# terran-project/terran

Measured on AMD Instinct MI355X. Metric: frames/sec 1080p detect+embed+pose, higher is better.
Workload: dtype f16x3: operands x = hi + lo (two IEEE halfs, 22 bits), 3 f16 MFMAs per product, f32 accumulate; float32-grade results; 1 GPU; BASELINE configs[4]: 1080p detect+embed+pose; Detection(short_side=416) + Recognition(top-2) + Estimation(short_side=184); 32 frames per GPU per step resident in HBM; random-init weights; precision=f16x3, frames_per_gpu_step=32, faces_per_frame=2, resident_batch_reused=True, batches_in_flight_per_gpu=2

## Files before the change

include/terran_amd.h:

```cpp
#ifndef TERRAN_AMD_H
#define TERRAN_AMD_H

#include <stddef.h>
#include <stdint.h>

#ifdef __cplusplus
extern "C" {
#endif

#define TA_OK 0
#define TA_E_INVALID (-1)
#define TA_E_DEVICE (-2)
#define TA_E_CAPACITY (-3)
#define TA_E_OVERFLOW (-4)
#define TA_E_RANGE (-5)

#define TA_MODEL_RETINAFACE 1
#define TA_MODEL_ARCFACE 2
#define TA_MODEL_OPENPOSE 3

typedef struct ta_ctx ta_ctx;
typedef struct ta_model ta_model;
typedef struct ta_frames ta_frames;

const char* ta_version(void);
int ta_device_count(void);
int ta_device_pci_bus_id(int device_id, char* out, int capacity);
int ta_ctx_create(int device_id, ta_ctx** out);
void ta_ctx_destroy(ta_ctx* ctx);
const char* ta_last_error(const ta_ctx* ctx);
int ta_ctx_sync(ta_ctx* ctx);
int ta_profile_enable(ta_ctx* ctx, int on);
int ta_profile_reset(ta_ctx* ctx);
int ta_profile_read(ta_ctx* ctx, int klass, double* ms, int64_t* launches, double* work);
int ta_timer_start(ta_ctx* ctx);
int ta_timer_stop(ta_ctx* ctx, double* ms);

int ta_host_alloc(ta_ctx* ctx, size_t bytes, void** out);
void ta_host_free(ta_ctx* ctx, void* ptr);

int ta_frames_upload(ta_ctx* ctx, const uint8_t* nhwc_rgb, int n, int h, int w, ta_frames** out);
int ta_frames_alloc(ta_ctx* ctx, int n, int h, int w, ta_frames** out);
int ta_frames_shape(const ta_frames* f, int* n, int* h, int* w);
int ta_frames_download(const ta_frames* f, uint8_t* nhwc_rgb);
void ta_frames_free(ta_frames* f);
int ta_frames_resize(ta_ctx* ctx, const ta_frames* src, int dst_h, int dst_w, ta_frames** out);
int ta_frames_resize_bicubic(ta_ctx* ctx, const ta_frames* src, int dst_h, int dst_w, ta_frames** out);
int ta_frames_paste(ta_ctx* ctx, const ta_frames* src, int src_index, ta_frames* dst, int dst_index,
                    int top, int left);

#define TA_DRAW_BAR 0
#define TA_DRAW_LINE 1
#define TA_DRAW_DISC 2
typedef struct ta_draw_prim {
  int32_t frame;
  int32_t kind;
  int32_t x0, y0, x1, y1;
  int32_t width;
  uint8_t rgba[4];
} ta_draw_prim;
int ta_frames_draw(ta_ctx* ctx, ta_frames* frames, const ta_draw_prim* prims, int n);

#define TA_JPEG_DEVICE 0
#define TA_JPEG_FALLBACK_PROCESS 1
#define TA_JPEG_FALLBACK_ARITHMETIC 2
#define TA_JPEG_FALLBACK_PRECISION 3
#define TA_JPEG_FALLBACK_COMPONENTS 4
#define TA_JPEG_FALLBACK_COLOR 5
#define TA_JPEG_FALLBACK_SCANS 6
#define TA_JPEG_FALLBACK_SAMPLING 7
#define TA_JPEG_INVALID (-1)
typedef struct ta_jpeg_header {
  int32_t width, height, components;
  int32_t path;
  int32_t h_samp[3], v_samp[3];
  int32_t quant_index[3];
  int32_t blocks_w[3], blocks_h[3];
  int32_t restart_interval;
  int32_t reserved[2];
  int64_t block_offset[3];
  int64_t blocks_total;
  uint16_t quant[4][64];
} ta_jpeg_header;
int ta_jpeg_coefficients(const uint8_t* data, size_t size, ta_jpeg_header* header, int16_t* coefs, int64_t capacity_blocks,
                         char* err, int err_capacity);
int ta_jpeg_decode(ta_ctx* ctx, const uint8_t* const* data, const size_t* sizes, int n, int threads, int capacity,
                   ta_frames** out, int32_t* paths, int32_t* required);
int ta_jpeg_last_stats(const ta_ctx* ctx, double* ms, int64_t* counts);

int ta_jpeg_encode_header(int h, int w, int quality, int subsampling, uint8_t* out, size_t capacity, size_t* size);
int ta_jpeg_encode(ta_ctx* ctx, const ta_frames* frames, int quality, int subsampling, const uint8_t** out,
                   size_t* sizes);
int ta_jpeg_encode_last_stats(const ta_ctx* ctx, double* ms, int64_t* counts);

int ta_model_load(ta_ctx* ctx, int kind, const void* blob, size_t bytes, ta_model** out);
void ta_model_free(ta_model* m);
int ta_model_kind(const ta_model* m);

int ta_model_forward_frames(ta_model* m, const ta_frames* frames);
int ta_model_forward_crops(ta_model* m, const uint8_t* crops_nchw_bgr, int n);
int ta_model_tensor_shape(ta_model* m, int tensor, int* n, int* c, int* h, int* w);
int ta_model_read_tensor(ta_model* m, int tensor, int ch_off, int ch, float* dst_nchw);

int ta_model_tensor_unscale(const ta_model* m, int tensor, float* out, int capacity);
int ta_model_debug_amax(ta_model* m, int enable, float* out, int capacity);
int ta_model_graph_probe(ta_model* m, int reps, double* out_ms);

int ta_retinaface_run(ta_model* m, const ta_frames* frames, float score_thr, float nms_thr,
                      int capacity, int32_t* counts, float* boxes, float* landmarks, float* scores,
                      int32_t* required);
int ta_retinaface_postprocess(ta_ctx* ctx, const float* const heads[9], int n, int h, int w,
                              float score_thr, float nms_thr, int capacity, int32_t* counts,
                              float* boxes, float* landmarks, float* scores, int32_t* required);

int ta_arcface_embed_crops(ta_model* m, const uint8_t* crops_nchw_bgr, int n, int normalize, float* out);
int ta_arcface_embed_faces(ta_model* m, const ta_frames* frames, const int32_t* frame_index,
                           const double* inv_affine, int n, int normalize, float* out,
                           uint8_t* crops_out);
int ta_arcface_embed_faces_multi(ta_model* m, const ta_frames* const* frames, int n_sources, const int32_t* source_index,
                                 const int32_t* frame_index, const double* inv_affine, int n, int normalize,
                                 float* out, uint8_t* crops_out);
int ta_cosine_distance(ta_ctx* ctx, const float* a, int na, const float* b, int nb, int dim, float* out);

int ta_openpose_run(ta_model* m, const ta_frames* frames, double scale, int capacity,
                    int32_t* counts, int32_t* keypoints, double* scores, int32_t* required);
int ta_openpose_group(ta_ctx* ctx, const float* pafs, const float* heatmaps, int n, int h, int w,
                      double scale, int capacity, int32_t* counts, int32_t* keypoints,
                      double* scores, int32_t* required);
int ta_openpose_last_stats(const ta_ctx* ctx, int64_t* peaks, int64_t* connections);

int ta_openpose_debug_read(ta_ctx* ctx, int n, int cap_peaks, int32_t* peak_counts, int32_t* peaks_yx,
                           float* peak_scores, int cap_conn, int32_t* conn_counts, int32_t* conn_ij,
                           float* conn_scores);

int ta_bicubic_x8(ta_ctx* ctx, const float* maps, int n, int c, int h, int w, float* out);

#define TA_CONV_AUTO 0
#define TA_CONV_GENERIC 1
#define TA_CONV_PIPE64 2
#define TA_CONV_PIPE128 3
#define TA_CONV_SPLIT_2x2 4
#define TA_CONV_SPLIT_2x2_P8 5
#define TA_CONV_SPLIT_2x4 6
#define TA_CONV_SPLIT_1x4 7
#define TA_CONV_WIN_2x2 8
#define TA_CONV_WIN_2x4 9
#define TA_CONV_WIN_1x4 10
#define TA_CONV_SPLIT_1x4_W2 11
#define TA_CONV_SPLIT_2x2_W2 12
int ta_debug_conv_variant(ta_ctx* ctx, int variant);
int ta_debug_range_check(ta_ctx* ctx);
int ta_debug_conv_counts(ta_ctx* ctx, int64_t* counts16, int reset);
int ta_debug_kernel_work(ta_ctx* ctx, char* csv, size_t capacity, int reset);

#ifdef __cplusplus
}
#endif
#endif
```

terran_amd/csrc/conv_split.hip:

```cpp
#include "conv_split_kernels.h"

TA_TRACE_READER(ta_debug_trace_read_split)

__global__ __launch_bounds__(256) void splitk_reduce_kernel(const ta_conv_launch p) {
  const int c4 = p.cout >> 2;
  const int total = p.M * c4;
  const int HoWo = p.Ho * p.Wo;
  for (int i = blockIdx.x * blockDim.x + threadIdx.x; i < total; i += gridDim.x * blockDim.x) {
    const int pix = i / c4, co = (i - pix * c4) * 4;
    const int img = pix / HoWo;
    const int rem = pix - img * HoWo;
    const int y = rem / p.Wo, x = rem - y * p.Wo;
    f32x4 v = *(const f32x4*)(p.bias + co);
    const f32x4 us = *(const f32x4*)((p.bias + p.coutp) + co);
    if (p.bias9) {
      const int cls = ta_border_class(y, x, p.Ho, p.Wo);
      if (cls != TA_INTERIOR) v = *(const f32x4*)(p.bias9 + (size_t)cls * p.coutp + co);
    }
    for (int k = 0; k < p.k_split; ++k) {
      const f32x4 t = *(const f32x4*)(p.partial + ((size_t)k * p.M + pix) * p.coutp + co);
#pragma unroll
      for (int e = 0; e < 4; ++e) v[e] = __builtin_fmaf(t[e], us[e], v[e]);
    }
    if (p.act == TA_ACT_RELU) {
#pragma unroll
      for (int e = 0; e < 4; ++e) v[e] = ta_relu(v[e]);
    } else if (p.act == TA_ACT_PRELU) {
      const f32x4 sl = *(const f32x4*)(p.prelu + co);
#pragma unroll
      for (int e = 0; e < 4; ++e) v[e] = v[e] > 0.f ? v[e] : v[e] * sl[e];
    }
    if (p.res) {
      const int ry = p.res_up2 ? (y >> 1) : y, rx = p.res_up2 ? (x >> 1) : x;
      const f32x4 r = ta_ld4(p.res + (size_t)img * p.res_img + (size_t)ry * p.res_row + (size_t)rx * p.res_pix + p.res_off0, p.res_ch + co, p.res_fmt);
#pragma unroll
      for (int e = 0; e < 4; ++e) v[e] += r[e];
    }
    ta_st4(p.out + (size_t)img * p.out_img + (size_t)y * p.out_row + (size_t)x * p.out_pix + p.out_off0, p.out_ch + co,
           p.out_fmt, v);
    unsigned amax = ta_amax4(0u, v);
    if (p.out2) {
      const f32x4 sc = *(const f32x4*)(p.scale2 + co), sh = *(const f32x4*)(p.shift2 + co);
      f32x4 z;
#pragma unroll
      for (int e = 0; e < 4; ++e) z[e] = v[e] * sc[e] + sh[e];
      ta_st4(p.out2 + (size_t)img * p.o2_img + (size_t)y * p.o2_row + (size_t)x * p.o2_pix + p.o2_off0, p.o2_ch + co, p.o2_fmt, z);
      amax = ta_amax4(amax, z);
    }
    if (p.range_check) ta_range_report(p, amax);
  }
}


int ta_win_patch_rows(const ta_conv_launch& p, int BM) {
  if (p.Wo <= 0 || p.Ho <= 0 || p.win_wp <= 0) return 1 << 30;
  const long long n = BM - 1, hp = p.win_img / p.win_wp;
  const long long rows = n + ((n + p.Wo - 1) / p.Wo) * (p.win_wp - p.Wo) + ((n + (long long)p.Ho * p.Wo - 1) / ((long long)p.Ho * p.Wo)) * (hp - p.Ho) * p.win_wp +
                         (long long)(p.k_h - 1) * p.win_wp + p.k_w;
  return rows > (1 << 30) ? (1 << 30) : (int)rows;
}


int ta_launch_conv_split(ta_ctx* ctx, int v, const ta_conv_launch& p) {
  int rc;
  switch (p.prec) {
    case PREC_F16X3: rc = launch_split_variant<PREC_F16X3>(ctx, v, p); break;
    case PREC_F16X2: rc = launch_split_variant<PREC_F16X2>(ctx, v, p); break;
    default: rc = ta_launch_conv_split_modes(ctx, v, p); break;
  }
  if (rc != TA_OK || p.k_split <= 1) return rc;
  const int total = p.M * (p.cout >> 2);
  hipLaunchKernelGGL(splitk_reduce_kernel, dim3((total + 255) / 256), dim3(256), 0, ctx->stream, p);
  TA_HIP(ctx, hipGetLastError());
  return TA_OK;
}
```

terran_amd/csrc/conv_split_kernels.h:

```cpp
#pragma once
#include "conv_common.h"

__device__ __forceinline__ void split_acc_clear(f32x16 (&acc)[2][2]) {
#pragma unroll
  for (int a = 0; a < 2; ++a)
#pragma unroll
    for (int b = 0; b < 2; ++b)
#pragma unroll
      for (int r = 0; r < 16; ++r) acc[a][b][r] = 0.f;
}

template <int PREC>
__device__ __forceinline__ void split_mma16(f32x16 (&acc)[2][2], const bf16x8 (&ah)[2], const bf16x8 (&al)[2], const bf16x8 (&bh)[2],
                                            const bf16x8 (&bl)[2]) {
  if constexpr (prec_x3(PREC) || prec_x2(PREC)) {
#pragma unroll
    for (int a = 0; a < 2; ++a)
#pragma unroll
      for (int b = 0; b < 2; ++b) acc[a][b] = ta_mfma16<PREC>(al[a], bh[b], acc[a][b]);
  }
  if constexpr (prec_x3(PREC)) {
#pragma unroll
    for (int a = 0; a < 2; ++a)
#pragma unroll
      for (int b = 0; b < 2; ++b) acc[a][b] = ta_mfma16<PREC>(ah[a], bl[b], acc[a][b]);
  }
  if constexpr (PREC == PREC_F16) {
#pragma unroll
    for (int a = 0; a < 2; ++a)
#pragma unroll
      for (int b = 0; b < 2; ++b) acc[a][b] = ta_mfma16<PREC>(al[a], bl[b], acc[a][b]);
  }
#pragma unroll
  for (int a = 0; a < 2; ++a)
#pragma unroll
    for (int b = 0; b < 2; ++b) acc[a][b] = ta_mfma16<PREC>(ah[a], bh[b], acc[a][b]);
}

template <int NREAD, int NMMA>
__device__ __forceinline__ void split_pin() {
#pragma unroll
  for (int i = 0; i < NREAD; ++i) {
    __builtin_amdgcn_sched_group_barrier(0x100, 1, 0);
    __builtin_amdgcn_sched_group_barrier(0x008, 1, 0);
  }
  __builtin_amdgcn_sched_group_barrier(0x008, NMMA - NREAD, 0);
}


template <int CM, int CN, int NP, int PREC, int STAGES>
__global__ __launch_bounds__(64 * (CM * CN + NP), STAGES == 2 ? 4 : (CM * CN + NP) / 4) void conv_igemm_split(const ta_conv_launch p) {
  static_assert(NP == 4 || NP == 8, "4 or 8 producer waves");
  static_assert(STAGES == 3 || (STAGES == 2 && CM * CN == 4 && NP == 4), "3-stage ring, or the 2-stage two-workgroups-per-CU variant of the 8-wave tiles");
  static_assert(CM * CN == 4 || CM * CN == 8, "consumer grid: 1x4 (64 cout x 256 px), 2x2 (128 x 128) or 2x4 (128 x 256)");
  constexpr int NC = CM * CN;
  constexpr int BN = CM * 64, BM = CN * 64;
  constexpr int NI = (BN + BM) / 8 / NP;
  constexpr int QA = BN / 8 / NP;
  constexpr int STAGE = (BN + BM) * 32;
  extern __shared__ __attribute__((aligned(16))) float lds[];

  const int tid = threadIdx.x;
  const int lane = tid & 63;
  const int wave = __builtin_amdgcn_readfirstlane(tid >> 6);
  if (wave == 0) TA_STAMP(0);
  if (wave == NC) TA_STAMP(8);

  const int n_ct = p.coutp / BN;
  const int n_pt = (p.M + BM - 1) / BM;
  const int tile_blocks = (((n_pt + 7) >> 3) * n_ct) << 3;
  const int ks = p.k_split > 1 ? ta_div_r(blockIdx.x, tile_blocks, p.r_tile_blocks, p.fast_div) : 0;
  const int bid = blockIdx.x - ks * tile_blocks;
  const int grp = bid >> 3, xcd = bid & 7;
  const int gq = ta_div_r(grp, n_ct, p.r_nct, p.fast_div);
  const int pt = ta_xcd_tile(n_pt, xcd, gq);
  if (pt < 0) return;
  const int ct0 = (grp - gq * n_ct) * BN;
  const int pt0 = pt * BM;
  const int HoWo = p.Ho * p.Wo;
  int s_begin = 0, S = p.n_slabs;
  if (p.k_split > 1) {
    s_begin = (int)(((long long)ks * p.n_slabs) / p.k_split);
    S = (int)(((long long)(ks + 1) * p.n_slabs) / p.k_split) - s_begin;
  }

  if (wave >= NC) {
    const int pw = wave - NC;
    const int pchunk = lane & 7;
    const int lchunk = pchunk ^ ((4 * (pw & 1) + (lane >> 4)) & 7);
    const char* a_base = (const char*)p.w;
    const size_t a_slab_bytes = (size_t)p.coutp * 128;
    unsigned a_off[QA];
    unsigned b_off[NI - QA];
#pragma unroll
    for (int q = 0; q < QA; ++q) a_off[q] = (unsigned)(((ct0 + (q * NP + pw) * 8 + (lane >> 3)) * 32 + lchunk * 4) * 4);
    ta_k_walk wa(p, s_begin);
    auto issue_a = [&](int, int stage) {
#pragma unroll
      for (int q = 0; q < QA; ++q) ta_dma16(a_base + (size_t)wa.a_slab * a_slab_bytes, a_off[q], lds + stage * STAGE + (q * NP + pw) * 256);
      wa.advance();
    };
    issue_a(0, 0);
    if (S > 1) issue_a(1, 1);
    const int pl = p.pool;
    const ta_pixel_walk walk(p, pl ? pt0 >> 2 : pt0, HoWo);
    const int in_ch = p.in_ch_off + (p.group_cout ? (ct0 / p.group_cout) * p.group_cin : 0);
    const size_t off0 = (size_t)walk.img0 * p.in_img + (size_t)((walk.y0 << pl) * p.stride) * p.in_row +
                        (size_t)((walk.x0 << pl) * p.stride) * p.in_pix + p.in_off0 + in_ch;
    const char* b_base = (const char*)(p.in + off0);
    ta_k_walk wb(p, s_begin);
#pragma unroll
    for (int q = QA; q < NI; ++q) {
      const int d = (q * NP + pw) * 8 + (lane >> 3) - BN;
      int img, y, x;
      const int dd = pt0 + d < p.M ? d : 0;
      walk.at(pl ? dd >> 2 : dd, img, y, x);
      if (pl) {
        y = 2 * y + ((dd >> 1) & 1);
        x = 2 * x + (dd & 1);
      }
      const size_t off = (size_t)img * p.in_img + (size_t)(y * p.stride) * p.in_row + (size_t)(x * p.stride) * p.in_pix +
                         p.in_off0 + in_ch;
      b_off[q - QA] = (unsigned)((off - off0) * 4 + lchunk * 16);
      ta_dma16(b_base + wb.b_off, b_off[q - QA], lds + (q * NP + pw) * 256);
    }
    wb.advance();
    auto issue_b = [&](int stage) {
#pragma unroll
      for (int q = QA; q < NI; ++q) ta_dma16(b_base + wb.b_off, b_off[q - QA], lds + stage * STAGE + (q * NP + pw) * 256);
      wb.advance();
    };
    if (wave == NC) TA_STAMP(9);
    if (S > 1) issue_b(1);
    if (wave == NC) TA_STAMP(10);
    int stage = STAGES == 2 ? 0 : 2;
    if constexpr (STAGES == 2) {
      for (int s = 0; s < S; ++s) {
        if (s == 0 && S > 1) asm volatile("s_waitcnt vmcnt(%0)" ::"n"(NI - QA) : "memory");
        else asm volatile("s_waitcnt vmcnt(0)" ::: "memory");
        __builtin_amdgcn_s_barrier();
        asm volatile("" ::: "memory");
        if (s >= 1 && s + 1 < S) {
          issue_a(s + 1, stage);
          issue_b(stage);
          stage ^= 1;
        }
      }
    } else
    for (int s = 0; s < S; ++s) {
      if (s == 0 && S > 1) asm volatile("s_waitcnt vmcnt(%0)" ::"n"(NI - QA) : "memory");
      else if (s + 1 < S) asm volatile("s_waitcnt vmcnt(%0)" ::"n"(NI) : "memory");
      else asm volatile("s_waitcnt vmcnt(0)" ::: "memory");
      __builtin_amdgcn_s_barrier();
      asm volatile("" ::: "memory");
      if (s + 2 < S) {
        issue_a(s + 2, stage);
        issue_b(stage);
        stage = stage == 2 ? 0 : stage + 1;
      }
    }
    {
      __builtin_amdgcn_s_barrier();
      __builtin_amdgcn_s_barrier();
      asm volatile("" ::: "memory");
      bool done = false;
      if constexpr (PREC != PREC_F32) done = conv_drain_dispatch<BN, BM, 64 * (NC + NP), (PREC == PREC_F16 ? 2 : (prec_half(PREC) ? 1 : 0))>(p, lds, ct0, pt0, tid, HoWo);
      if (!done) conv_epilogue_drain<BN, BM, 64 * (NC + NP)>(p, lds, ct0, pt0, tid, HoWo, ks);
    }
    return;
  }

  const int cm = wave / CN, cn = wave % CN;
  int stage = 0;
  f32x16 acc[2][2];
  split_acc_clear(acc);
  const int frow = lane & 31;
  const int fsw = (frow >> 1) & 7;
  const int kg = lane >> 5;
  const int a_row0 = cm * 64 + frow;
  const int b_row0 = BN + cn * 64 + frow;
  struct Frag {
    bf16x8 ah[2], al[2], bh[2], bl[2];
    f32x4 a32[2][2], b32[2][2];
  };
  const int fcb = kg * 4;
  auto load = [&](Frag& f, const float* st, int t) {
    if constexpr (PREC == PREC_F32) {
#pragma unroll
      for (int g = 0; g < 2; ++g) {
        const int pc = ((fcb + 2 * t + g) ^ fsw) * 4;
#pragma unroll
        for (int a = 0; a < 2; ++a) f.a32[a][g] = *(const f32x4*)(st + (a_row0 + a * 32) * 32 + pc);
#pragma unroll
        for (int b = 0; b < 2; ++b) f.b32[b][g] = *(const f32x4*)(st + (b_row0 + b * 32) * 32 + pc);
      }
      return;
    }
#pragma unroll
    for (int a = 0; a < 2; ++a) {
      f.ah[a] = *(const bf16x8*)(st + (a_row0 + a * 32) * 32 + ((2 * kg + t) ^ fsw) * 4);
      if constexpr (prec_x3(PREC) || prec_x2(PREC) || PREC == PREC_F16) f.al[a] = *(const bf16x8*)(st + (a_row0 + a * 32) * 32 + ((4 + 2 * kg + t) ^ fsw) * 4);
    }
#pragma unroll
    for (int b = 0; b < 2; ++b) {
      f.bh[b] = *(const bf16x8*)(st + (b_row0 + b * 32) * 32 + ((2 * kg + t) ^ fsw) * 4);
      if constexpr (prec_x3(PREC) || PREC == PREC_F16) f.bl[b] = *(const bf16x8*)(st + (b_row0 + b * 32) * 32 + ((4 + 2 * kg + t) ^ fsw) * 4);
    }
  };
  auto mma = [&](const Frag& f) {
    if constexpr (PREC == PREC_F32) {
#pragma unroll
      for (int g = 0; g < 2; ++g)
#pragma unroll
        for (int e = 0; e < 4; ++e)
#pragma unroll
          for (int a = 0; a < 2; ++a)
#pragma unroll
            for (int b = 0; b < 2; ++b)
              acc[a][b] = __builtin_amdgcn_mfma_f32_32x32x2f32(f.a32[a][g][e], f.b32[b][g][e], acc[a][b], 0, 0, 0);
      return;
    }
    split_mma16<PREC>(acc, f.ah, f.al, f.bh, f.bl);
  };
  constexpr int NREAD = PREC == PREC_BF16 ? 4 : (prec_x2(PREC) ? 6 : 8);
  constexpr int NMMA = PREC == PREC_F32 ? 32 : (prec_x3(PREC) ? 12 : ((PREC == PREC_F16 || prec_x2(PREC)) ? 8 : 4));
  Frag F0, F1;
  if (wave == 0) TA_STAMP(1);
  __builtin_amdgcn_s_barrier();
  asm volatile("" ::: "memory");
  if (wave == 0) TA_STAMP(2);
  if constexpr (STAGES == 2) {
    for (int s = 0; s < S; ++s) {
      const float* st = lds + (s & 1) * STAGE;
      load(F0, st, 0);
      mma(F0);
      load(F0, st, 1);
      mma(F0);
      if (s + 1 < S) {
        asm volatile("s_waitcnt lgkmcnt(0)" ::: "memory");
        __builtin_amdgcn_s_barrier();
        asm volatile("" ::: "memory");
      }
    }
  } else {
  load(F0, lds + stage * STAGE, 0);
  for (int s = 0; s + 1 < S; ++s) {
    const float* st = lds + stage * STAGE;
    stage = stage + 1 == STAGES ? 0 : stage + 1;
    __builtin_amdgcn_sched_barrier(0);
    load(F1, st, 1);
    mma(F0);
    split_pin<NREAD, NMMA>();
    __builtin_amdgcn_sched_barrier(0);
    asm volatile("s_waitcnt lgkmcnt(0)" ::: "memory");
    __builtin_amdgcn_s_barrier();
    asm volatile("" ::: "memory");
    load(F0, lds + stage * STAGE, 0);
    mma(F1);
    split_pin<NREAD, NMMA>();
    __builtin_amdgcn_sched_barrier(0);
  }
  load(F1, lds + stage * STAGE, 1);
  stage = stage + 1 == STAGES ? 0 : stage + 1;
  mma(F0);
  mma(F1);
  }
  if (wave == 0) TA_STAMP(3);
  {
    __builtin_amdgcn_s_barrier();
    asm volatile("" ::: "memory");
    if (wave == 0) TA_STAMP(5);
    conv_epilogue_park<BN>(acc, lds, cm, cn, lane);
    if (wave == 0) TA_STAMP(6);
    asm volatile("s_waitcnt lgkmcnt(0)" ::: "memory");
    __builtin_amdgcn_s_barrier();
    asm volatile("" ::: "memory");
    if (wave == 0) TA_STAMP(7);
    bool done = false;
    if constexpr (PREC != PREC_F32) done = conv_drain_dispatch<BN, BM, 64 * (NC + NP), (PREC == PREC_F16 ? 2 : (prec_half(PREC) ? 1 : 0))>(p, lds, ct0, pt0, tid, HoWo);
    if (!done) conv_epilogue_drain<BN, BM, 64 * (NC + NP)>(p, lds, ct0, pt0, tid, HoWo, ks);
  }
  if (wave == 0) TA_STAMP(4);
}

template <int CM, int CN, int PREC, int PR>
__global__ __launch_bounds__(64 * (CM * CN + 4), (CM * CN + 4) / 4) void conv_igemm_win(const ta_conv_launch p) {
  static_assert(prec_half(PREC) && PREC != PREC_F16, "pre-split half-float tensors (f16x3 / f16x2)");
  static_assert(CM * CN == 4 || CM * CN == 8, "consumer grid: 1x4 (64 cout x 256 px), 2x2 (128 x 128) or 2x4 (128 x 256)");
  static_assert(PR % 32 == 0, "whole DMA instructions per producer wave");
  constexpr int NC = CM * CN, NP = 4;
  constexpr int BN = CM * 64, BM = CN * 64;
  constexpr int QA = BN / 8 / NP;
  constexpr int NPW = PR / 8 / NP;
  constexpr int A_STAGE = BN * 32;
  constexpr int PATCH = PR * 32;
  static_assert(QA + NPW < 64, "s_waitcnt vmcnt is a 6-bit count");
  extern __shared__ __attribute__((aligned(16))) float lds[];
  float* const patch0 = lds + 3 * A_STAGE;

  const int tid = threadIdx.x;
  const int lane = tid & 63;
  const int wave = __builtin_amdgcn_readfirstlane(tid >> 6);
  const int n_ct = p.coutp / BN;
  const int n_pt = (p.M + BM - 1) / BM;
  const int bid = blockIdx.x;
  const int grp = bid >> 3, xcd = bid & 7;
  const int gq = ta_div_r(grp, n_ct, p.r_nct, p.fast_div);
  const int pt = ta_xcd_tile(n_pt, xcd, gq);
  if (pt < 0) return;
  const int ct0 = (grp - gq * n_ct) * BN;
  const int pt0 = pt * BM;
  const int HoWo = p.Ho * p.Wo;
  const int S = p.n_slabs;
  const int T = p.k_w * p.k_h;
  if (wave == 0) TA_STAMP(0);
  if (wave == NC) TA_STAMP(8);
  const ta_pixel_walk walk(p, pt0, HoWo);
  const int wp = p.win_wp, wimg = p.win_img;

  if (wave >= NC) {
    const int pw = wave - NC;
    const int pchunk = lane & 7;
    const int lchunk = pchunk ^ ((4 * (pw & 1) + (lane >> 4)) & 7);
    const char* a_base = (const char*)p.w;
    const size_t a_slab_bytes = (size_t)p.coutp * 128;
    unsigned a_off[QA];
#pragma unroll
    for (int q = 0; q < QA; ++q) a_off[q] = (unsigned)(((ct0 + (q * NP + pw) * 8 + (lane >> 3)) * 32 + lchunk * 4) * 4);
    ta_k_walk wa(p, 0);
    auto issue_a = [&](int stage) {
#pragma unroll
      for (int q = 0; q < QA; ++q) ta_dma16(a_base + (size_t)wa.a_slab * a_slab_bytes, a_off[q], lds + stage * A_STAGE + (q * NP + pw) * 256);
      wa.advance();
    };
    issue_a(0);
    const int last = (p.M - pt0 < BM ? p.M - pt0 : BM) - 1;
    int img1, y1, x1;
    walk.at(last, img1, y1, x1);
    const int n_patch = (img1 - walk.img0) * wimg + (y1 - walk.y0) * wp + (x1 - walk.x0) + (p.k_h - 1) * wp + p.k_w;
    const int in_ch = p.in_ch_off + (p.group_cout ? (ct0 / p.group_cout) * p.group_cin : 0);
    const size_t off0 = (size_t)walk.img0 * p.in_img + (size_t)walk.y0 * p.in_row + (size_t)walk.x0 * p.in_pix + p.in_off0 + in_ch;
    const char* b_base = (const char*)(p.in + off0);
    unsigned p_off[NPW];
#pragma unroll
    for (int i = 0; i < NPW; ++i) {
      const int r = (i * NP + pw) * 8 + (lane >> 3);
      const int rr = r < n_patch ? r : n_patch - 1;
      p_off[i] = (unsigned)rr * (unsigned)(p.in_pix * 4) + (unsigned)(lchunk * 16);
    }
    auto issue_patch = [&](int cb) {
      float* dst = patch0 + (cb & 1) * PATCH;
#pragma unroll
      for (int i = 0; i < NPW; ++i) ta_dma16(b_base + (size_t)cb * 128, p_off[i], dst + (i * NP + pw) * 256);
    };
    if (wave == NC) TA_STAMP(9);
    issue_patch(0);
    if (S > 1) issue_a(1);
    if (wave == NC) TA_STAMP(10);
    int stage = 2, t = 0, cb = 0;
    bool patch_behind = false;
    for (int g = 0; g < S; ++g) {
      const bool more = g + 1 < S;
      if (patch_behind) {
        if (more) asm volatile("s_waitcnt vmcnt(%0)" ::"n"(QA + NPW) : "memory");
        else asm volatile("s_waitcnt vmcnt(%0)" ::"n"(NPW) : "memory");
      } else {
        if (more) asm volatile("s_waitcnt vmcnt(%0)" ::"n"(QA) : "memory");
        else asm volatile("s_waitcnt vmcnt(0)" ::: "memory");
      }
      __builtin_amdgcn_s_barrier();
      asm volatile("" ::: "memory");
      patch_behind = false;
      if (t == 0 && cb + 1 < p.k_cblocks) {
        issue_patch(cb + 1);
        patch_behind = true;
      }
      if (g + 2 < S) {
        issue_a(stage);
        stage = stage == 2 ? 0 : stage + 1;
      }
      if (++t == T) {
        t = 0;
        ++cb;
      }
    }
    {
      __builtin_amdgcn_s_barrier();
      __builtin_amdgcn_s_barrier();
      asm volatile("" ::: "memory");
      if (!conv_drain_dispatch<BN, BM, 64 * (NC + NP), 1>(p, lds, ct0, pt0, tid, HoWo))
        conv_epilogue_drain<BN, BM, 64 * (NC + NP)>(p, lds, ct0, pt0, tid, HoWo, 0);
    }
    return;
  }

  const int cm = wave / CN, cn = wave % CN;
  f32x16 acc[2][2];
  split_acc_clear(acc);
  const int frow = lane & 31;
  const int fsw = (frow >> 1) & 7;
  const int kg = lane >> 5;
  const int a_row0 = cm * 64 + frow;
  int rB[2];
#pragma unroll
  for (int b = 0; b < 2; ++b) {
    const int d = cn * 64 + b * 32 + frow;
    int img, y, x;
    walk.at(pt0 + d < p.M ? d : 0, img, y, x);
    rB[b] = (img - walk.img0) * wimg + (y - walk.y0) * wp + (x - walk.x0);
  }
  struct Frag {
    bf16x8 ah[2], al[2], bh[2], bl[2];
  };
  unsigned pb[2];
  auto baddr = [&](int tap_off, int buf) {
#pragma unroll
    for (int b = 0; b < 2; ++b) {
      const unsigned row = (unsigned)(rB[b] + tap_off);
      pb[b] = (unsigned)buf * (unsigned)(PATCH * 4) + row * 128u + ((((unsigned)(2 * kg)) ^ ((row >> 1) & 7u)) << 4);
    }
  };
  auto load = [&](Frag& f, const float* st, int t) {
#pragma unroll
    for (int a = 0; a < 2; ++a) {
      f.ah[a] = *(const bf16x8*)(st + (a_row0 + a * 32) * 32 + ((2 * kg + t) ^ fsw) * 4);
      f.al[a] = *(const bf16x8*)(st + (a_row0 + a * 32) * 32 + ((4 + 2 * kg + t) ^ fsw) * 4);
    }
#pragma unroll
    for (int b = 0; b < 2; ++b) {
      const char* q = (const char*)patch0 + (pb[b] ^ (unsigned)(t << 4));
      f.bh[b] = *(const bf16x8*)q;
      if constexpr (prec_x3(PREC)) f.bl[b] = *(const bf16x8*)((const char*)patch0 + ((pb[b] ^ (unsigned)(t << 4)) ^ 64u));
    }
  };
  auto mma = [&](const Frag& f) { split_mma16<PREC>(acc, f.ah, f.al, f.bh, f.bl); };
  constexpr int NREAD = prec_x3(PREC) ? 8 : 6;
  constexpr int NMMA = prec_x3(PREC) ? 12 : 8;
  int kx = 0, ky = 0, cb = 0, tap_off = 0, stage = 0;
  Frag F0, F1;
  baddr(0, 0);
  if (wave == 0) TA_STAMP(1);
  __builtin_amdgcn_s_barrier();
  asm volatile("" ::: "memory");
  if (wave == 0) TA_STAMP(2);
  load(F0, lds, 0);
  for (int g = 0; g + 1 < S; ++g) {
    const float* st = lds + stage * A_STAGE;
    stage = stage == 2 ? 0 : stage + 1;
    __builtin_amdgcn_sched_barrier(0);
    load(F1, st, 1);
    mma(F0);
    split_pin<NREAD, NMMA>();
    __builtin_amdgcn_sched_barrier(0);
    if (++kx == p.k_w) {
      kx = 0;
      tap_off += wp - p.k_w;
      if (++ky == p.k_h) {
        ky = 0;
        ++cb;
        tap_off = -1;
      }
    }
    ++tap_off;
    asm volatile("s_waitcnt lgkmcnt(0)" ::: "memory");
    baddr(tap_off, cb & 1);
    __builtin_amdgcn_s_barrier();
    asm volatile("" ::: "memory");
    load(F0, lds + stage * A_STAGE, 0);
    mma(F1);
    split_pin<NREAD, NMMA>();
    __builtin_amdgcn_sched_barrier(0);
  }
  load(F1, lds + stage * A_STAGE, 1);
  mma(F0);
  mma(F1);
  if (wave == 0) TA_STAMP(3);
  {
    __builtin_amdgcn_s_barrier();
    asm volatile("" ::: "memory");
    if (wave == 0) TA_STAMP(5);
    conv_epilogue_park<BN>(acc, lds, cm, cn, lane);
    if (wave == 0) TA_STAMP(6);
    asm volatile("s_waitcnt lgkmcnt(0)" ::: "memory");
    __builtin_amdgcn_s_barrier();
    asm volatile("" ::: "memory");
    if (wave == 0) TA_STAMP(7);
    if (!conv_drain_dispatch<BN, BM, 64 * (NC + NP), 1>(p, lds, ct0, pt0, tid, HoWo))
      conv_epilogue_drain<BN, BM, 64 * (NC + NP)>(p, lds, ct0, pt0, tid, HoWo, 0);
  }
  if (wave == 0) TA_STAMP(4);
}

static void split_launch_facts(ta_ctx* ctx, ta_conv_launch& q, const ta_tile_grid& g, int BM, int split_fmt, bool lean_ok) {
  q.r_nct = 1.0f / (float)g.n_ct;
  q.r_tile_blocks = 1.0f / (float)(g.groups * 8);
  q.r_Wo = 1.0f / (float)q.Wo;
  q.r_Ho = 1.0f / (float)q.Ho;
  q.r_HoWo = 1.0f / (float)(q.Ho * q.Wo);
  const long long grid = (long long)g.groups * 8 * q.k_split;
  q.fast_div = (grid < (1 << 24) && (long long)q.M + BM < (1 << 24)) ? 1 : 0;
  const long long n_img = q.Ho * q.Wo > 0 ? ((long long)q.M + q.Ho * q.Wo - 1) / (q.Ho * q.Wo) : 0;
  auto fits = [&](long long img_stride, int off0) { return ((n_img + 1) * img_stride + off0) * 4 < (1LL << 32); };
  bool ok = lean_ok && q.out_fmt == split_fmt && (q.cout & 7) == 0 && ((q.out_ch | q.res_ch | q.o2_ch) & 7) == 0 && fits(q.out_img, q.out_off0);
  if (q.res) ok = ok && q.res_fmt == split_fmt && fits(q.res_img, q.res_off0);
  if (q.out2) ok = ok && q.o2_fmt == split_fmt && fits(q.o2_img, q.o2_off0);
  q.fast_drain = ok ? 1 : 0;
  if (ok) ctx->conv_counts[TA_CV_COUNT - 1] += 1;
}

template <int CM, int CN, int NP, int PREC, int STAGES>
static int launch_split(ta_ctx* ctx, const ta_conv_launch& p) {
  constexpr int BN = CM * 64, BM = CN * 64;
  const ta_tile_grid g(p, BN, BM);
  const size_t lds_bytes = (size_t)STAGES * (BN + BM) * 32 * sizeof(float);
  auto kern = conv_igemm_split<CM, CN, NP, PREC, STAGES>;
  TA_SET_LDS_ATTR(ctx, kern, lds_bytes);
  ta_conv_launch q = p;
  constexpr int SPLIT_FMT = PREC == PREC_F16 ? TA_FMT_F16 : (prec_half(PREC) ? TA_FMT_SPLIT16 : TA_FMT_SPLIT);
  split_launch_facts(ctx, q, g, BM, SPLIT_FMT, PREC != PREC_F32 && p.k_split == 1);
  TA_NOTE_KERNEL(ctx, "conv_igemm_split<%d,%d,%d,%d,%d>", CM, CN, NP, PREC, STAGES);
  hipLaunchKernelGGL(kern, dim3(g.groups * 8 * p.k_split), dim3(64 * (CM * CN + NP)), lds_bytes, ctx->stream, q);
  TA_HIP(ctx, hipGetLastError());
  return TA_OK;
}

template <int CM, int CN, int PREC, int PR>
static int launch_win(ta_ctx* ctx, const ta_conv_launch& p) {
  constexpr int BN = CM * 64, BM = CN * 64;
  const ta_tile_grid g(p, BN, BM);
  constexpr size_t ring = (size_t)(3 * BN + 2 * PR) * 128, park = (size_t)BM * BN * 4;
  constexpr size_t lds_bytes = ring > park ? ring : park;
  static_assert(lds_bytes <= 160 * 1024, "one workgroup's LDS");
  auto kern = conv_igemm_win<CM, CN, PREC, PR>;
  TA_SET_LDS_ATTR(ctx, kern, lds_bytes);
  ta_conv_launch q = p;
  q.k_split = 1;
  split_launch_facts(ctx, q, g, BM, TA_FMT_SPLIT16, true);
  TA_NOTE_KERNEL(ctx, "conv_igemm_win<%d,%d,%d,%d>", CM, CN, PREC, PR);
  hipLaunchKernelGGL(kern, dim3(g.groups * 8), dim3(64 * (CM * CN + 4)), lds_bytes, ctx->stream, q);
  TA_HIP(ctx, hipGetLastError());
  return TA_OK;
}

template <int PREC>
static int launch_split_variant(ta_ctx* ctx, int v, const ta_conv_launch& p) {
  switch (v) {
    case TA_CV_SPLIT_2x2: return launch_split<2, 2, 4, PREC, 3>(ctx, p);
    case TA_CV_SPLIT_2x2_P8: return launch_split<2, 2, 8, PREC, 3>(ctx, p);
    case TA_CV_SPLIT_2x4: return launch_split<2, 4, 4, PREC, 3>(ctx, p);
    case TA_CV_SPLIT_1x4: return launch_split<1, 4, 4, PREC, 3>(ctx, p);
    case TA_CV_SPLIT_1x4_W2: return launch_split<1, 4, 4, PREC, 2>(ctx, p);
    case TA_CV_SPLIT_2x2_W2: return launch_split<2, 2, 4, PREC, 2>(ctx, p);
    case TA_CV_WIN_2x2:
    case TA_CV_WIN_2x4:
    case TA_CV_WIN_1x4:
      if constexpr (PREC == PREC_F16X3 || PREC == PREC_F16X2) {
        if (v == TA_CV_WIN_2x2) return launch_win<2, 2, PREC, TA_WIN_PR_2x2>(ctx, p);
        if (v == TA_CV_WIN_2x4) return launch_win<2, 4, PREC, TA_WIN_PR_2x4>(ctx, p);
        return launch_win<1, 4, PREC, TA_WIN_PR_1x4>(ctx, p);
      }
      break;
  }
  return ta_fail(ctx, TA_E_INVALID, "conv: unknown kernel variant %d", v);
}
```

terran_amd/csrc/conv_split_modes.hip:

```cpp
#include "conv_split_kernels.h"

TA_TRACE_READER(ta_debug_trace_read_split_modes)

int ta_launch_conv_split_modes(ta_ctx* ctx, int v, const ta_conv_launch& p) {
  switch (p.prec) {
    case PREC_F32: return launch_split_variant<PREC_F32>(ctx, v, p);
    case PREC_BF16X3: return launch_split_variant<PREC_BF16X3>(ctx, v, p);
    case PREC_F16: return launch_split_variant<PREC_F16>(ctx, v, p);
    default: return launch_split_variant<PREC_BF16>(ctx, v, p);
  }
}
```

terran_amd/csrc/net.hip:

```cpp
#include <stdlib.h>
#include <string.h>

#include <algorithm>
#include <chrono>

#include "act_format.h"
#include "ta_internal.h"

static int conv_out(int in, int k, int stride, int pad) { return (in + 2 * pad - k) / stride + 1; }

static bool conv_ksplit_eligible(const ta_op_desc& op, int in_fmt) {
  const int kblk = in_fmt == TA_FMT_F16 ? 64 : 32;
  const bool uniform = (op.cin % kblk == 0) && (op.n_slabs == op.kh * op.kw * (op.cin / kblk));
  const bool kernel_ok = in_fmt == ta_split_fmt_of(op.prec);
  return uniform && kernel_ok && op.groups <= 1 && !op.pool;
}

#define TA_MAX_PLANS 4
#define TA_MAX_PLAN_BYTES ((size_t)96 << 30)

static void destroy_plan(ta_plan* pl) {
  if (!pl) return;
  if (pl->arena) (void)hipFree(pl->arena);
  if (pl->ktab_dev) (void)hipFree(pl->ktab_dev);
  delete pl;
}

static void activate(ta_model* m, ta_plan* pl) {
  m->active = pl;
  pl->last_use = ++m->use_counter;
  m->plan_n = pl->n;
  m->plan_h = pl->h;
  m->plan_w = pl->w;
  m->tensors = pl->tensors;
  m->ktab_dev = pl->ktab_dev;
  m->ktab_off = pl->ktab_off;
  m->splitk_ws = pl->splitk_ws;
}

static void free_plans(ta_model* m) {
  for (ta_plan* pl : m->plans) destroy_plan(pl);
  m->plans.clear();
  m->active = nullptr;
  m->plan_n = m->plan_h = m->plan_w = 0;
  m->tensors.clear();
  m->ktab_dev = nullptr;
}

static int plan_capacity(int kind, int n) {
  if (kind != TA_MODEL_ARCFACE) return n;
  if (n <= 8) return 8;
  if (n <= 32) return 32;
  return (n + 63) / 64 * 64;
}

int ta_model_plan(ta_model* m, int n_run, int h, int w) {
  ta_ctx* ctx = m->ctx;
  if (n_run <= 0 || h <= 0 || w <= 0) return ta_fail(ctx, TA_E_INVALID, "plan: bad input shape %dx%dx%d", n_run, h, w);
  const int n = plan_capacity(m->kind, n_run);
  m->run_n = n_run;
  if (m->active && m->plan_n == n && m->plan_h == h && m->plan_w == w) {
    m->active->last_use = ++m->use_counter;
    return TA_OK;
  }
  for (ta_plan* pl : m->plans)
    if (pl->n == n && pl->h == h && pl->w == w) {
      activate(m, pl);
      return TA_OK;
    }
  TA_HIP(ctx, hipStreamSynchronize(ctx->stream));
  for (;;) {
    size_t bytes = 0;
    for (ta_plan* pl : m->plans) bytes += pl->arena_bytes;
    if (m->plans.size() < TA_MAX_PLANS && bytes <= TA_MAX_PLAN_BYTES) break;
    if (m->plans.empty()) break;
    size_t lru = 0;
    for (size_t i = 1; i < m->plans.size(); ++i)
      if (m->plans[i]->last_use < m->plans[lru]->last_use) lru = i;
    if (m->plans[lru] == m->active) m->active = nullptr;
    destroy_plan(m->plans[lru]);
    m->plans.erase(m->plans.begin() + lru);
  }
  ta_plan* np = new ta_plan();
  np->n = n;
  np->h = h;
  np->w = w;
  struct guard_t {
    ta_plan*& p;
    ~guard_t() { if (p) destroy_plan(p); }
  } guard{np};

  const int T = m->hdr.n_tensors;
  std::vector<ta_tensor> ts(T);
  std::vector<bool> set(T, false);
  for (int i = 0; i < T; ++i) {
    ts[i].c = m->tdesc[i].channels;
    ts[i].halo = m->tdesc[i].halo;
    ts[i].fmt = m->tdesc[i].fmt;
    if (m->tdesc[i].unscale_off >= 0) {
      ts[i].unscale_dev = (const float*)(m->weights_dev + m->tdesc[i].unscale_off);
      ts[i].unscale_host = m->unscale_host[i].data();
    }
    ts[i].n = n;
  }
  const int in_id = m->hdr.input_tensor;
  ts[in_id].h = h;
  ts[in_id].w = w;
  set[in_id] = true;

  auto resolve_alias = [&](int id) -> int {
    const int src = m->tdesc[id].alias_of;
    if (src == -2) ts[id].owns = false;
    if (src < 0 || set[id]) return TA_OK;
    if (!set[src]) return ta_fail(ctx, TA_E_INVALID, "plan: alias tensor %d used before its source %d", id, src);
    if (ts[src].halo != 0 || (size_t)ts[src].h * ts[src].w * ts[src].c != (size_t)ts[id].c)
      return ta_fail(ctx, TA_E_INVALID, "plan: alias tensor %d does not match source %d", id, src);
    ts[id].h = ts[id].w = 1;
    ts[id].owns = false;
    set[id] = true;
    return TA_OK;
  };

  auto set_out = [&](int id, int oh, int ow) -> int {
    if (oh <= 0 || ow <= 0) return ta_fail(ctx, TA_E_INVALID, "plan: input %dx%d too small for the network", h, w);
    if (set[id]) {
      if (ts[id].h != oh || ts[id].w != ow)
        return ta_fail(ctx, TA_E_INVALID, "plan: tensor %d written with %dx%d and %dx%d", id, ts[id].h, ts[id].w, oh, ow);
      return TA_OK;
    }
    ts[id].h = oh;
    ts[id].w = ow;
    set[id] = true;
    return TA_OK;
  };

  for (size_t oi = 0; oi < m->ops.size(); ++oi) {
    const ta_op_desc& op = m->ops[oi];
    TA_TRY(resolve_alias(op.in));
    if (!set[op.in]) return ta_fail(ctx, TA_E_INVALID, "plan: op %zu reads unset tensor %d", oi, op.in);
    const ta_tensor& ti = ts[op.in];
    if (op.type != TA_OP_CONV && (ti.fmt == TA_FMT_F16 || ts[op.out].fmt == TA_FMT_F16))
      return ta_fail(ctx, TA_E_INVALID, "plan: op %zu: only convs read and write half-float tensors", oi);
    switch (op.type) {
      case TA_OP_CONV:
        if (op.groups > 1) {
          const bool ok = op.cin % 32 == 0 && op.n_slabs == op.kh * op.kw * (op.cin / 32) && op.n_slabs >= 2 &&
                          op.cout % op.groups == 0 && (op.cout / op.groups) % 128 == 0 && op.cout == op.coutp &&
                          op.in_ch_off % 32 == 0 && op.in_ch_off + op.groups * op.cin <= ti.c &&
                          ti.fmt == ta_split_fmt_of(op.prec);
          if (!ok) return ta_fail(ctx, TA_E_INVALID, "plan: op %zu: unsupported grouped convolution", oi);
        }
        [[fallthrough]];
      case TA_OP_DWCONV:
        if (ti.halo < op.pad) return ta_fail(ctx, TA_E_INVALID, "plan: op %zu needs halo %d, tensor has %d", oi, op.pad, ti.halo);
        if (op.type == TA_OP_CONV && op.pool) {
          if (op.out2 >= 0 || op.res >= 0 || op.groups > 1 || op.cin % 32 || op.coutp % 64)
            return ta_fail(ctx, TA_E_INVALID, "plan: op %zu: unsupported conv + max-pool fusion", oi);
          TA_TRY(set_out(op.out, conv_out(ti.h, op.kh, op.stride, op.pad) / 2, conv_out(ti.w, op.kw, op.stride, op.pad) / 2));
          break;
        }
        TA_TRY(set_out(op.out, conv_out(ti.h, op.kh, op.stride, op.pad), conv_out(ti.w, op.kw, op.stride, op.pad)));
        if (op.out2 >= 0) TA_TRY(set_out(op.out2, ts[op.out].h, ts[op.out].w));
        break;
      case TA_OP_MAXPOOL:
        TA_TRY(set_out(op.out, ti.h / 2, ti.w / 2));
        break;
      case TA_OP_RFSTEM:
        if (oi != 0 || op.in != in_id || m->tdesc[op.in].alias_of != -2 || op.w_off < 0)
          return ta_fail(ctx, TA_E_INVALID, "plan: the RetinaFace front op must be op 0 on a shape-only input tensor");
        if (op.cout == 32)
          TA_TRY(set_out(op.out, ((ti.h + 1) / 2 + 1) / 2, ((ti.w + 1) / 2 + 1) / 2));
        else
          TA_TRY(set_out(op.out, (ti.h + 1) / 2, (ti.w + 1) / 2));
        break;
      case TA_OP_DWPW:
        if (ti.halo < 1) return ta_fail(ctx, TA_E_INVALID, "plan: op %zu (dw+pw) needs an input halo", oi);
        if (ti.fmt != TA_FMT_F32 || op.in_ch_off || op.scale2_off < 0 || op.shift2_off < 0 || op.cin > ti.c)
          return ta_fail(ctx, TA_E_INVALID, "plan: op %zu: unsupported dw+pw block", oi);
        TA_TRY(set_out(op.out, conv_out(ti.h, 3, op.stride, 1), conv_out(ti.w, 3, op.stride, 1)));
        break;

      case TA_OP_COPYCH:
        TA_TRY(set_out(op.out, ti.h, ti.w));
        break;
      default:
        return ta_fail(ctx, TA_E_INVALID, "plan: unknown op type %d", op.type);
    }
  }
  for (int i = 0; i < T; ++i) TA_TRY(resolve_alias(i));
  for (int i = 0; i < T; ++i)
    if ((ts[i].fmt != TA_FMT_F32 && ts[i].c % 32) || (ts[i].fmt == TA_FMT_F16 && ts[i].c % 64) || ts[i].fmt < 0 || ts[i].fmt > TA_FMT_F16)
      return ta_fail(ctx, TA_E_INVALID, "plan: tensor %d: format %d with %d channels", i, ts[i].fmt, ts[i].c);

  size_t total = 0;
  std::vector<size_t> offs(T, 0);
  for (int i = 0; i < T; ++i) {
    if (!set[i] || !ts[i].owns) continue;
    const size_t bytes = ts[i].elems() * sizeof(float);
    if (bytes >= ((size_t)1 << 32)) return ta_fail(ctx, TA_E_INVALID, "plan: tensor %d exceeds 4 GiB; split the batch", i);
    offs[i] = total;
    total += (bytes + 255) & ~(size_t)255;
  }
  size_t ws_bytes = 0;
  for (size_t oi = 0; oi < m->ops.size(); ++oi) {
    const ta_op_desc& op = m->ops[oi];
    if (op.type != TA_OP_CONV) continue;
    const int M = ts[op.out].n * ts[op.out].h * ts[op.out].w;
    const int ks = ta_conv_ksplit(op.coutp, op.n_slabs, conv_ksplit_eligible(op, ts[op.in].fmt), (op.variant >> 8) & 255);
    if (ks > 1) ws_bytes = std::max(ws_bytes, (size_t)ks * M * op.coutp * sizeof(float));
  }
  const size_t ws_off = total;
  total += (ws_bytes + 255) & ~(size_t)255;
  hipError_t e = hipMalloc((void**)&np->arena, total ? total : 256);
  if (e != hipSuccess) return ta_fail(ctx, TA_E_DEVICE, "plan: hipMalloc(%zu) failed: %s", total, hipGetErrorString(e));
  np->arena_bytes = total;
  TA_HIP(ctx, hipMemsetAsync(np->arena, 0, total ? total : 256, ctx->stream));
  for (int i = 0; i < T; ++i)
    if (set[i] && ts[i].owns) ts[i].dev = (float*)(np->arena + offs[i]);
  for (int i = 0; i < T; ++i)
    if (set[i] && !ts[i].owns) ts[i].dev = m->tdesc[i].alias_of >= 0 ? ts[m->tdesc[i].alias_of].dev : nullptr;
  np->splitk_ws = ws_bytes ? (float*)(np->arena + ws_off) : nullptr;

  std::vector<int32_t> ktab;
  np->ktab_off.assign(m->ops.size(), 0);
  for (size_t oi = 0; oi < m->ops.size(); ++oi) {
    const ta_op_desc& op = m->ops[oi];
    if (op.type != TA_OP_CONV) continue;
    const ta_tensor& ti = ts[op.in];
    np->ktab_off[oi] = ktab.size();
    if (ti.fmt == TA_FMT_F16) continue;
    const int cpt = op.cin / 4;
    const int nq = op.kh * op.kw * cpt;
    if (nq > op.n_slabs * 8) return ta_fail(ctx, TA_E_INVALID, "plan: op %zu has too few K slabs", oi);
    for (int q = 0; q < op.n_slabs * 8; ++q) {
      int32_t off = 0;
      if (q < nq) {
        const int tap = q / cpt, ch = (q % cpt) * 4;
        const int ky = tap / op.kw, kx = tap % op.kw;
        off = (int32_t)((((size_t)ky * ti.wp() + kx) * ti.c + op.in_ch_off + ch) * sizeof(float));
      }
      ktab.push_back(off);
    }
  }
  if (!ktab.empty()) {
    TA_HIP(ctx, hipMalloc((void**)&np->ktab_dev, ktab.size() * sizeof(int32_t)));
    TA_HIP(ctx, hipMemcpy(np->ktab_dev, ktab.data(), ktab.size() * sizeof(int32_t), hipMemcpyHostToDevice));
  }
  TA_HIP(ctx, hipStreamSynchronize(ctx->stream));
  np->tensors.swap(ts);
  ta_plan* done = np;
  np = nullptr;
  m->plans.push_back(done);
  activate(m, done);
  return TA_OK;
}

static const float* wptr(const ta_model* m, int64_t off) { return off < 0 ? nullptr : (const float*)(m->weights_dev + off); }

static void print_op_profile(ta_model* m, std::vector<hipEvent_t>& ev) {
  (void)hipStreamSynchronize(m->ctx->stream);
  double tot_ms = 0, tot_fl = 0;
  for (size_t oi = 0; oi < m->ops.size(); ++oi) {
    const ta_op_desc& op = m->ops[oi];
    const ta_tensor& to = m->tensors[op.out];
    float ms = 0.f;
    (void)hipEventElapsedTime(&ms, ev[2 * oi], ev[2 * oi + 1]);
    const ta_tensor& ti = m->tensors[op.in];
    const double M = op.type == TA_OP_CONV && op.pool
                         ? (double)m->run_n * conv_out(ti.h, op.kh, op.stride, op.pad) * conv_out(ti.w, op.kw, op.stride, op.pad)
                         : (double)m->run_n * to.h * to.w;
    const double fl = (op.type == TA_OP_CONV || op.type == TA_OP_DWPW) ? 2.0 * op.macs_per_pixel * M : 0.0;
    tot_ms += ms;
    tot_fl += fl;
    fprintf(stderr, "op %3zu type %d k%dx%d s%d g%d cin %4d cout %4d  %3dx%-3d M %8.0f slabs %4d  %8.1f us %7.1f TF\n", oi, op.type, op.kh,
            op.kw, op.stride, op.groups, op.cin, op.cout, to.h, to.w, M, op.n_slabs, ms * 1e3, ms > 0 ? fl / (ms * 1e-3) / 1e12 : 0.0);
  }
  fprintf(stderr, "model kind %d n %d: %.3f ms in ops, %.1f GFLOP, %.1f TF\n", m->kind, m->run_n, tot_ms, tot_fl / 1e9, tot_fl / (tot_ms * 1e-3) / 1e12);
  for (auto e : ev) (void)hipEventDestroy(e);
}

int ta_model_run_ops(ta_model* m) {
  ta_ctx* ctx = m->ctx;
  static const bool prof_ops = getenv("TA_PROFILE_OPS") != nullptr;
  std::vector<hipEvent_t> ev;
  if (prof_ops) {
    ev.resize(2 * m->ops.size());
    for (auto& e : ev) (void)hipEventCreate(&e);
  }
  struct fin_t {
    ta_model* m;
    std::vector<hipEvent_t>& ev;
    bool on;
    ~fin_t() { if (on) print_op_profile(m, ev); }
  } fin{m, ev, prof_ops};
  static const bool no_lanes = getenv("TA_NO_LANES") != nullptr;
  const bool lanes_on = !prof_ops && !ctx->profiling && !no_lanes;
  struct lanes_t {
    ta_ctx* ctx;
    hipStream_t main;
    bool started[2] = {false, false};
    ~lanes_t() {
      ctx->stream = main;
      for (int i = 0; i < 2; ++i)
        if (started[i]) {
          (void)hipEventRecord(ctx->side_join[i], ctx->side_stream[i]);
          (void)hipStreamWaitEvent(main, ctx->side_join[i], 0);
        }
    }
  } lanes{ctx, ctx->stream};
  for (size_t oi = 0; oi < m->ops.size(); ++oi) {
    const ta_op_desc& op = m->ops[oi];
    const ta_tensor& ti = m->tensors[op.in];
    const ta_tensor& to = m->tensors[op.out];
    const int lane = lanes_on ? (op.variant >> 17) & 3 : 0;
    ctx->stream = lanes.main;
    if (lane) {
      const int li = lane - 1;
      if (!ctx->side_stream[li]) {
        TA_HIP(ctx, hipStreamCreateWithFlags(&ctx->side_stream[li], hipStreamNonBlocking));
        TA_HIP(ctx, hipEventCreateWithFlags(&ctx->side_fork[li], hipEventDisableTiming));
        TA_HIP(ctx, hipEventCreateWithFlags(&ctx->side_join[li], hipEventDisableTiming));
      }
      if (!lanes.started[li]) {
        TA_HIP(ctx, hipEventRecord(ctx->side_fork[li], lanes.main));
        TA_HIP(ctx, hipStreamWaitEvent(ctx->side_stream[li], ctx->side_fork[li], 0));
        lanes.started[li] = true;
      }
      ctx->stream = ctx->side_stream[li];
    }
    struct evp_t {
      hipEvent_t e;
      hipStream_t s;
      bool on;
      ~evp_t() { if (on) (void)hipEventRecord(e, s); }
    } evp{prof_ops ? ev[2 * oi + 1] : nullptr, ctx->stream, prof_ops};
    if (prof_ops) (void)hipEventRecord(ev[2 * oi], ctx->stream);
    switch (op.type) {
      case TA_OP_CONV: {
        ta_conv_launch p;
        memset(&p, 0, sizeof(p));
        p.in = ti.dev;
        p.w = wptr(m, op.w_off);
        p.ktab = m->ktab_dev + m->ktab_off[oi];
        p.bias = wptr(m, op.bias_off);
        p.prelu = wptr(m, op.prelu_off);
        p.out = to.dev;
        p.M = m->run_n * to.h * to.w;
        p.Ho = to.h;
        p.Wo = to.w;
        p.n_slabs = op.n_slabs;
        p.coutp = op.coutp;
        p.cout = op.cout;
        p.act = op.act;
        p.stride = op.stride;
        p.prec = op.prec;
        const int kblk = ti.fmt == TA_FMT_F16 ? 64 : 32;
        p.uniform_k = (op.cin % kblk == 0) && (op.n_slabs == op.kh * op.kw * (op.cin / kblk));
        p.k_cblocks = op.cin / kblk;
        if (ti.fmt == TA_FMT_F16 && (!p.uniform_k || op.in_ch_off || op.groups > 1 || op.prec != 4))
          return ta_fail(ctx, TA_E_INVALID, "op %zu: a half-float tensor feeds whole-tensor convs of the f16 mode only", oi);
        p.k_w = op.kw;
        p.k_h = op.kh;
        p.in_ch_off = op.in_ch_off;
        p.in_img = (int)((size_t)ti.hp() * ti.wp() * ti.cf());
        p.in_row = ti.wp() * ti.cf();
        p.in_pix = ti.cf();
        p.win_wp = ti.wp();
        p.win_img = ti.hp() * ti.wp();
        p.in_off0 = (int)(((size_t)(ti.halo - op.pad) * ti.wp() + (ti.halo - op.pad)) * ti.cf());
        p.out_img = (int)((size_t)to.hp() * to.wp() * to.cf());
        p.out_row = to.wp() * to.cf();
        p.out_pix = to.cf();
        p.out_off0 = (int)to.off(0, 0, 0);
        p.out_ch = op.out_ch_off;
        p.out_fmt = to.fmt;
        p.in_fmt = ti.fmt;
        if (op.res >= 0) {
          const ta_tensor& tr = m->tensors[op.res];
          p.res = tr.dev;
          p.res_img = (int)((size_t)tr.hp() * tr.wp() * tr.cf());
          p.res_row = tr.wp() * tr.cf();
          p.res_pix = tr.cf();
          p.res_off0 = (int)tr.off(0, 0, 0);
          p.res_ch = op.res_ch_off;
          p.res_fmt = tr.fmt;
          p.res_up2 = op.res_up2;
        }
        if (op.out2 >= 0) {
          const ta_tensor& t2 = m->tensors[op.out2];
          p.out2 = t2.dev;
          p.scale2 = wptr(m, op.scale2_off);
          p.shift2 = wptr(m, op.shift2_off);
          p.o2_img = (int)((size_t)t2.hp() * t2.wp() * t2.cf());
          p.o2_row = t2.wp() * t2.cf();
          p.o2_pix = t2.cf();
          p.o2_off0 = (int)t2.off(0, 0, 0);
          p.o2_ch = op.out2_ch_off;
          p.o2_fmt = t2.fmt;
        }
        if (op.groups > 1) {
          p.group_cout = op.cout / op.groups;
          p.group_cin = op.cin;
        }
        p.variant = op.variant & 255;
        if ((op.variant >> 16) & 1) p.bias9 = wptr(m, op.scale2_off);
        p.range_check = (m->has_half_ops && (m->tensor_read[op.out] || (op.out2 >= 0 && m->tensor_read[op.out2]))) ? 1 : 0;
        p.amax_index = (m->amax_on && oi < TA_AMAX_OPS) ? (int)oi : -1;
        double flops = 2.0 * op.macs_per_pixel * (double)p.M;
        if (op.pool) {
          p.pool = 1;
          p.M = m->run_n * to.h * to.w * 4;
          flops = 2.0 * op.macs_per_pixel * (double)m->run_n * conv_out(ti.h, op.kh, op.stride, op.pad) *
                  conv_out(ti.w, op.kw, op.stride, op.pad);
        }
        p.k_split = m->splitk_ws ? ta_conv_ksplit(p.coutp, p.n_slabs, conv_ksplit_eligible(op, ti.fmt), (op.variant >> 8) & 255) : 1;
        p.partial = m->splitk_ws;
        if (lane) p.k_split = 1;
        TA_TRY(ta_launch_conv(ctx, p, flops));
        break;
      }
      case TA_OP_RFSTEM:
        TA_TRY(ta_launch_rfstem(ctx, m->input_u8, m->run_n, ti.h, ti.w, (const float*)m->weights_host_small.data(),
                                op.cout == 32 ? wptr(m, op.w_off) + 448 : nullptr, to));
        break;
      case TA_OP_DWPW: {
        ta_conv_launch p;
        memset(&p, 0, sizeof(p));
        p.in = ti.dev;
        p.w = wptr(m, op.w_off);
        p.bias = wptr(m, op.bias_off);
        p.dw_w = wptr(m, op.scale2_off);
        p.dw_bias = wptr(m, op.shift2_off);
        p.dw_c = op.cin;
        p.dw_stride = op.stride;
        p.out = to.dev;
        p.M = m->run_n * to.h * to.w;
        p.Ho = to.h;
        p.Wo = to.w;
        p.n_slabs = op.n_slabs;
        p.coutp = op.coutp;
        p.cout = op.cout;
        p.act = op.act;
        p.stride = 1;
        p.prec = op.prec;
        p.range_check = (m->has_half_ops && m->tensor_read[op.out]) ? 1 : 0;
        p.amax_index = (m->amax_on && oi < TA_AMAX_OPS) ? (int)oi : -1;
        p.in_img = (int)((size_t)ti.hp() * ti.wp() * ti.c);
        p.in_row = ti.wp() * ti.c;
        p.in_pix = ti.c;
        p.in_off0 = (int)(((size_t)(ti.halo - 1) * ti.wp() + (ti.halo - 1)) * ti.c);
        p.in_fmt = ti.fmt;
        p.out_img = (int)((size_t)to.hp() * to.wp() * to.c);
        p.out_row = to.wp() * to.c;
        p.out_pix = to.c;
        p.out_off0 = (int)to.off(0, 0, 0);
        p.out_ch = op.out_ch_off;
        p.out_fmt = to.fmt;
        TA_TRY(ta_launch_dwpw(ctx, p, 2.0 * op.macs_per_pixel * (double)p.M));
        break;
      }
      case TA_OP_DWCONV: {
        ta_dw_launch p;
        memset(&p, 0, sizeof(p));
        p.in = ti.dev;
        p.w = wptr(m, op.w_off);
        p.bias = wptr(m, op.bias_off);
        p.out = to.dev;
        p.N = m->run_n;
        p.Ho = to.h;
        p.Wo = to.w;
        p.C = op.cin;
        p.stride = op.stride;
        p.relu = op.act == TA_ACT_RELU;
        p.in_img = (int)((size_t)ti.hp() * ti.wp() * ti.c);
        p.in_row = ti.wp() * ti.c;
        p.in_pix = ti.c;
        if (op.in_ch_off || op.out_ch_off) return ta_fail(ctx, TA_E_INVALID, "depthwise conv on a channel slice is not supported");
        p.in_off0 = (int)(((size_t)(ti.halo - op.pad) * ti.wp() + (ti.halo - op.pad)) * ti.c);
        p.in_fmt = ti.fmt;
        p.out_img = (int)((size_t)to.hp() * to.wp() * to.c);
        p.out_row = to.wp() * to.c;
        p.out_pix = to.c;
        p.out_off0 = (int)to.off(0, 0, 0);
        p.out_fmt = to.fmt;
        TA_TRY(ta_launch_dwconv(ctx, p));
        break;
      }
      case TA_OP_MAXPOOL:
        TA_TRY(ta_launch_maxpool(ctx, ti, to, m->run_n));
        break;
      case TA_OP_COPYCH:
        TA_TRY(ta_launch_copych(ctx, ti, op.in_ch_off, to, op.out_ch_off, op.cin, m->run_n));
        break;
    }
  }
  return TA_OK;
}

extern "C" {

int ta_model_load(ta_ctx* ctx, int kind, const void* blob, size_t bytes, ta_model** out) {
  ta_enter(ctx);
  if (!ctx || !blob || !out) return TA_E_INVALID;
  *out = nullptr;
  if (bytes < sizeof(ta_blob_header)) return ta_fail(ctx, TA_E_INVALID, "model blob too small");
  ta_blob_header h;
  memcpy(&h, blob, sizeof(h));
  if (h.magic != TA_BLOB_MAGIC || h.version != 9) return ta_fail(ctx, TA_E_INVALID, "model blob: bad magic/version (this library reads version 9)");
  if (h.kind != kind) return ta_fail(ctx, TA_E_INVALID, "model blob is kind %d, expected %d", h.kind, kind);
  if (h.n_tensors <= 0 || h.n_ops <= 0 || h.n_outputs < 0 || h.n_outputs > 16 || h.input_tensor < 0 ||
      h.input_tensor >= h.n_tensors)
    return ta_fail(ctx, TA_E_INVALID, "model blob: bad counts");
  const size_t t_end = (size_t)h.tensors_off + (size_t)h.n_tensors * sizeof(ta_tensor_desc);
  const size_t o_end = (size_t)h.ops_off + (size_t)h.n_ops * sizeof(ta_op_desc);
  const size_t w_end = (size_t)h.weights_off + (size_t)h.weights_bytes;
  if (t_end > bytes || o_end > bytes || w_end > bytes) return ta_fail(ctx, TA_E_INVALID, "model blob: truncated");
  ta_model* m = new ta_model();
  m->ctx = ctx;
  m->kind = kind;
  m->hdr = h;
  m->tdesc.resize(h.n_tensors);
  m->ops.resize(h.n_ops);
  memcpy(m->tdesc.data(), (const char*)blob + h.tensors_off, h.n_tensors * sizeof(ta_tensor_desc));
  memcpy(m->ops.data(), (const char*)blob + h.ops_off, h.n_ops * sizeof(ta_op_desc));
  for (auto& op : m->ops) {
    auto bad_t = [&](int t) { return t < 0 || t >= h.n_tensors; };
    auto bad_w = [&](int64_t off, size_t need) { return off >= 0 && (size_t)off + need > (size_t)h.weights_bytes; };
    bool bad = bad_t(op.in) || bad_t(op.out) || (op.res >= 0 && bad_t(op.res)) || (op.out2 >= 0 && bad_t(op.out2));
    if (op.type == TA_OP_CONV) {
      bad = bad || op.w_off < 0 || op.bias_off < 0 || op.cin % 4 || op.cout % 4 || op.coutp % 32 || op.n_slabs <= 0 ||
            op.stride <= 0 || op.wus_off != op.bias_off + 4 * (int64_t)op.coutp || bad_w(op.wus_off, (size_t)op.coutp * 4) || op.prec < 0 || op.prec > 5 || bad_w(op.w_off, (size_t)op.n_slabs * op.coutp * 128) ||
            bad_w(op.bias_off, (size_t)op.coutp * 4) || bad_w(op.prelu_off, (size_t)op.coutp * 4) ||
            bad_w(op.scale2_off, (size_t)op.coutp * 4) || bad_w(op.shift2_off, (size_t)op.coutp * 4) ||
            (op.act == TA_ACT_PRELU && op.prelu_off < 0) || (op.out2 >= 0 && (op.scale2_off < 0 || op.shift2_off < 0)) ||
            (((op.variant >> 16) & 1) && (op.out2 >= 0 || op.scale2_off < 0 || op.kh != 3 || op.kw != 3 || op.stride != 1 || op.pad != 1 ||
                                          op.pool || bad_w(op.scale2_off, (size_t)16 * op.coutp * 4)));
    } else if (op.type == TA_OP_RFSTEM) {
      bad = bad || op.w_off < 0 || (op.cout != 16 && op.cout != 32) || bad_w(op.w_off, (op.cout == 32 ? 448 + 704 : 448) * 4);
    } else if (op.type == TA_OP_DWPW) {
      bad = bad || op.w_off < 0 || op.bias_off < 0 || op.scale2_off < 0 || op.shift2_off < 0 || op.cin % 4 || op.cout % 4 ||
            (op.prec != 0 && op.prec != 3) || op.wus_off != op.bias_off + 4 * (int64_t)op.coutp || bad_w(op.wus_off, (size_t)op.coutp * 4) ||
            op.coutp % 32 || op.n_slabs <= 0 || op.n_slabs * 32 < op.cin || (op.stride != 1 && op.stride != 2) ||
            bad_w(op.w_off, (size_t)op.n_slabs * op.coutp * 128) || bad_w(op.bias_off, (size_t)op.coutp * 4) ||
            bad_w(op.scale2_off, (size_t)op.cin * 36) || bad_w(op.shift2_off, (size_t)op.cin * 4);
    } else if (op.type == TA_OP_DWCONV) {
      bad = bad || op.w_off < 0 || op.bias_off < 0 || op.cin % 4 || op.kh != 3 || op.kw != 3 ||
            bad_w(op.w_off, (size_t)op.cin * 36) || bad_w(op.bias_off, (size_t)op.cin * 4);
    }
    if (bad) {
      delete m;
      return ta_fail(ctx, TA_E_INVALID, "model blob: malformed op");
    }
  }
  {
    bool bad = m->tdesc[h.input_tensor].unscale_off >= 0;
    m->unscale_host.resize(h.n_tensors);
    for (int t = 0; t < h.n_tensors && !bad; ++t) {
      const int64_t off = m->tdesc[t].unscale_off;
      if (off < 0) continue;
      const size_t need = (size_t)m->tdesc[t].channels * sizeof(float);
      if ((off & 3) || (size_t)off + need > (size_t)h.weights_bytes) {
        bad = true;
        break;
      }
      m->unscale_host[t].resize(m->tdesc[t].channels);
      memcpy(m->unscale_host[t].data(), (const char*)blob + h.weights_off + off, need);
    }
    for (int i = 0; i < h.n_outputs; ++i)
      if (h.outputs[i] < 0 || h.outputs[i] >= h.n_tensors) bad = true;
    m->tensor_read.assign(h.n_tensors, 0);
    for (auto& op : m->ops) {
      m->tensor_read[op.in] = 1;
      if (op.res >= 0) m->tensor_read[op.res] = 1;
    }
    for (int t = 0; t < h.n_tensors; ++t)
      if (m->tdesc[t].alias_of >= 0 && m->tdesc[t].alias_of < h.n_tensors && (m->tensor_read[t] || m->tensor_read[m->tdesc[t].alias_of]))
        m->tensor_read[t] = m->tensor_read[m->tdesc[t].alias_of] = 1;
    for (auto& op : m->ops) {
      if (op.type == TA_OP_DWCONV && (m->tdesc[op.in].unscale_off >= 0 || m->tdesc[op.out].unscale_off >= 0)) bad = true;
      if ((op.type == TA_OP_CONV || op.type == TA_OP_DWPW) && (op.prec == 3 || op.prec == 4 || op.prec == 5)) m->has_half_ops = true;
    }
    if (bad) {
      delete m;
      return ta_fail(ctx, TA_E_INVALID, "model blob: inconsistent activation scales");
    }
  }
  {
    std::vector<int> writer_lane(h.n_tensors, 0), reader_lanes(h.n_tensors, 0);
    bool bad = false;
    for (auto& op : m->ops) {
      const int lane = (op.variant >> 17) & 3;
      if (lane == 3 || (lane && (op.type != TA_OP_CONV || ((op.variant >> 8) & 255) > 1 || op.pool))) bad = true;
      const int reads[3] = {op.in, op.res, -1};
      for (int t : reads) {
        if (t < 0) continue;
        if (writer_lane[t] && writer_lane[t] != lane) bad = true;
        reader_lanes[t] |= 1 << lane;
      }
      const int writes[2] = {op.out, op.out2};
      for (int t : writes) {
        if (t < 0) continue;
        if (reader_lanes[t] & ~(1 << lane)) bad = true;
        if (writer_lane[t] && writer_lane[t] != lane) bad = true;
        if (lane) writer_lane[t] = lane;
        else if (reader_lanes[t] >> 1) bad = true;
      }
    }
    if (bad) {
      delete m;
      return ta_fail(ctx, TA_E_INVALID, "model blob: an op lane (side stream) shares tensors with ops outside it");
    }
  }
  hipError_t e = hipMalloc((void**)&m->weights_dev, h.weights_bytes ? h.weights_bytes : 16);
  if (e != hipSuccess) {
    delete m;
    return ta_fail(ctx, TA_E_DEVICE, "hipMalloc(weights %lld) failed: %s", (long long)h.weights_bytes, hipGetErrorString(e));
  }
  e = hipMemcpy(m->weights_dev, (const char*)blob + h.weights_off, h.weights_bytes, hipMemcpyHostToDevice);
  if (e != hipSuccess) {
    (void)hipFree(m->weights_dev);
    delete m;
    return ta_fail(ctx, TA_E_DEVICE, "weights upload failed: %s", hipGetErrorString(e));
  }
  if (m->ops[0].type == TA_OP_RFSTEM)
    m->weights_host_small.assign((const char*)blob + h.weights_off + m->ops[0].w_off, (const char*)blob + h.weights_off + m->ops[0].w_off + 448 * 4);
  *out = m;
  return TA_OK;
}

int ta_model_graph_probe(ta_model* m, int reps, double* out_ms) {
  ta_enter(m ? m->ctx : nullptr);
  if (!m || !out_ms || reps < 1) return TA_E_INVALID;
  ta_ctx* ctx = m->ctx;
  if (m->run_n <= 0) return ta_fail(ctx, TA_E_INVALID, "graph_probe: run a forward first (it replays that plan)");
  struct res_t {
    hipEvent_t e0 = nullptr, e1 = nullptr;
    hipGraph_t graph = nullptr;
    hipGraphExec_t exec = nullptr;
    ~res_t() {
      if (exec) (void)hipGraphExecDestroy(exec);
      if (graph) (void)hipGraphDestroy(graph);
      if (e0) (void)hipEventDestroy(e0);
      if (e1) (void)hipEventDestroy(e1);
    }
  } r;
  hipEvent_t& e0 = r.e0;
  hipEvent_t& e1 = r.e1;
  hipGraph_t& graph = r.graph;
  hipGraphExec_t& exec = r.exec;
  TA_HIP(ctx, hipEventCreate(&e0));
  TA_HIP(ctx, hipEventCreate(&e1));
  auto now = [] { return std::chrono::duration<double, std::milli>(std::chrono::steady_clock::now().time_since_epoch()).count(); };
  for (int i = 0; i < 2; ++i) TA_TRY(ta_model_run_ops(m));
  TA_HIP(ctx, hipStreamSynchronize(ctx->stream));
  float ms = 0.f;
  double t0 = now();
  TA_HIP(ctx, hipEventRecord(e0, ctx->stream));
  for (int i = 0; i < reps; ++i) TA_TRY(ta_model_run_ops(m));
  TA_HIP(ctx, hipEventRecord(e1, ctx->stream));
  out_ms[2] = (now() - t0) / reps;
  TA_HIP(ctx, hipStreamSynchronize(ctx->stream));
  TA_HIP(ctx, hipEventElapsedTime(&ms, e0, e1));
  out_ms[0] = ms / reps;
  t0 = now();
  TA_HIP(ctx, hipStreamBeginCapture(ctx->stream, hipStreamCaptureModeRelaxed));
  const int rc = ta_model_run_ops(m);
  const hipError_t ce = hipStreamEndCapture(ctx->stream, &graph);
  if (rc != TA_OK) return rc;
  TA_HIP(ctx, ce);
  TA_HIP(ctx, hipGraphInstantiate(&exec, graph, nullptr, nullptr, 0));
  out_ms[4] = now() - t0;
  for (int i = 0; i < 2; ++i) TA_HIP(ctx, hipGraphLaunch(exec, ctx->stream));
  TA_HIP(ctx, hipStreamSynchronize(ctx->stream));
  t0 = now();
  TA_HIP(ctx, hipEventRecord(e0, ctx->stream));
  for (int i = 0; i < reps; ++i) TA_HIP(ctx, hipGraphLaunch(exec, ctx->stream));
  TA_HIP(ctx, hipEventRecord(e1, ctx->stream));
  out_ms[3] = (now() - t0) / reps;
  TA_HIP(ctx, hipStreamSynchronize(ctx->stream));
  TA_HIP(ctx, hipEventElapsedTime(&ms, e0, e1));
  out_ms[1] = ms / reps;
  return TA_OK;
}

int ta_model_debug_amax(ta_model* m, int enable, float* out, int capacity) {
  ta_enter(m ? m->ctx : nullptr);
  if (!m) return TA_E_INVALID;
  ta_ctx* ctx = m->ctx;
  const size_t n = 2 * std::min(m->ops.size(), (size_t)TA_AMAX_OPS);
  unsigned* slots = (unsigned*)ctx->range_flag + TA_AMAX_SLOT0;
  TA_HIP(ctx, hipStreamSynchronize(ctx->stream));
  if (out) {
    if (!m->amax_on) return ta_fail(ctx, TA_E_INVALID, "debug_amax: not enabled");
    if ((size_t)capacity < 2 * m->ops.size()) return ta_fail(ctx, TA_E_CAPACITY, "debug_amax: %zu floats needed", 2 * m->ops.size());
    memset(out, 0, 2 * m->ops.size() * sizeof(float));
    TA_HIP(ctx, hipMemcpy(out, slots, n * sizeof(float), hipMemcpyDeviceToHost));
  }
  if (enable == 2) return TA_OK;
  if (enable) {
    if (ctx->amax_owner && ctx->amax_owner != m)
      return ta_fail(ctx, TA_E_INVALID, "debug_amax: another model of this context is collecting (disable it first)");
    TA_HIP(ctx, hipMemset(slots, 0, 2 * TA_AMAX_OPS * sizeof(unsigned)));
    ctx->amax_owner = m;
  } else if (ctx->amax_owner == m) {
    ctx->amax_owner = nullptr;
  }
  m->amax_on = enable != 0;
  return TA_OK;
}

int ta_model_tensor_unscale(const ta_model* m, int tensor, float* out, int capacity) {
  if (!m || !out || tensor < 0 || tensor >= (int)m->tdesc.size()) return TA_E_INVALID;
  const int c = m->tdesc[tensor].channels;
  if (capacity < c) return TA_E_CAPACITY;
  for (int i = 0; i < c; ++i) out[i] = m->unscale_host[tensor].empty() ? 1.0f : m->unscale_host[tensor][i];
  return TA_OK;
}

void ta_model_free(ta_model* m) {
  ta_enter(m ? m->ctx : nullptr);
  if (!m) return;
  (void)hipStreamSynchronize(m->ctx->stream);
  if (m->ctx->amax_owner == m) m->ctx->amax_owner = nullptr;
  free_plans(m);
  if (m->weights_dev) (void)hipFree(m->weights_dev);
  delete m;
}

int ta_model_kind(const ta_model* m) { return m ? m->kind : TA_E_INVALID; }

int ta_model_forward_frames(ta_model* m, const ta_frames* f) {
  ta_enter(m ? m->ctx : nullptr);
  if (!m || !f) return TA_E_INVALID;
  ta_ctx* ctx = m->ctx;
  if (m->kind != TA_MODEL_RETINAFACE && m->kind != TA_MODEL_OPENPOSE)
    return ta_fail(ctx, TA_E_INVALID, "forward_frames: model kind %d takes crops", m->kind);
  if (f->n == 0) return TA_OK;
  TA_TRY(ta_model_plan(m, f->n, f->h, f->w));
  m->input_u8 = f->dev;
  if (m->ops[0].type != TA_OP_RFSTEM)
    TA_TRY(ta_launch_preprocess(ctx, m->kind == TA_MODEL_RETINAFACE ? TA_PRE_RETINAFACE : TA_PRE_OPENPOSE, f->dev, f->n,
                                f->h, f->w, m->tensors[m->hdr.input_tensor]));
  return ta_model_run_ops(m);
}

int ta_model_forward_crops(ta_model* m, const uint8_t* crops, int n) {
  ta_enter(m ? m->ctx : nullptr);
  if (!m || (!crops && n > 0)) return TA_E_INVALID;
  ta_ctx* ctx = m->ctx;
  if (m->kind != TA_MODEL_ARCFACE) return ta_fail(ctx, TA_E_INVALID, "forward_crops: not an ArcFace model");
  if (n == 0) return TA_OK;
  TA_TRY(ta_model_plan(m, n, 112, 112));
  void* scr = nullptr;
  const size_t bytes = (size_t)n * 3 * 112 * 112;
  TA_TRY(ta_scratch(ctx, bytes, &scr));
  TA_HIP(ctx, hipMemcpyAsync(scr, crops, bytes, hipMemcpyHostToDevice, ctx->stream));
  TA_HIP(ctx, hipStreamSynchronize(ctx->stream));
  TA_TRY(ta_launch_preprocess(ctx, TA_PRE_ARCFACE_CROPS, (const uint8_t*)scr, n, 112, 112,
                              m->tensors[m->hdr.input_tensor]));
  return ta_model_run_ops(m);
}

int ta_model_tensor_shape(ta_model* m, int tensor, int* n, int* c, int* h, int* w) {
  if (!m || tensor < 0 || tensor >= (int)m->tensors.size()) return TA_E_INVALID;
  const ta_tensor& t = m->tensors[tensor];
  if (n) *n = m->run_n;
  if (c) *c = t.c;
  if (h) *h = t.h;
  if (w) *w = t.w;
  return TA_OK;
}

int ta_model_read_tensor(ta_model* m, int tensor, int ch_off, int ch, float* dst) {
  ta_enter(m ? m->ctx : nullptr);
  if (!m || !dst || tensor < 0 || tensor >= (int)m->tensors.size()) return TA_E_INVALID;
  ta_ctx* ctx = m->ctx;
  const ta_tensor& t = m->tensors[tensor];
  if (!t.dev || ch_off < 0 || ch <= 0 || ch_off + ch > t.c) return ta_fail(ctx, TA_E_INVALID, "read_tensor: bad slice");
  std::vector<float> host((size_t)m->run_n * t.hp() * t.wp() * t.c);
  TA_HIP(ctx, hipStreamSynchronize(ctx->stream));
  TA_HIP(ctx, hipMemcpy(host.data(), t.dev, host.size() * sizeof(float), hipMemcpyDeviceToHost));
  for (int i = 0; i < m->run_n; ++i)
    for (int c = 0; c < ch; ++c)
      for (int y = 0; y < t.h; ++y)
        for (int x = 0; x < t.w; ++x)
        {
          const int cc = ch_off + c;
          float v;
          if (t.fmt == TA_FMT_F16) {
            _Float16 hh;
            memcpy(&hh, (const char*)&host[t.off(i, y, x)] + 2 * cc, 2);
            v = (float)hh;
          } else if (t.fmt != TA_FMT_F32) {
            const char* b = (const char*)&host[t.off(i, y, x)] + ((cc >> 5) << 7) + ((cc & 31) << 1);
            uint16_t h16, l16;
            memcpy(&h16, b, 2);
            memcpy(&l16, b + 64, 2);
            if (t.fmt == TA_FMT_SPLIT16) {
              _Float16 hh, ll;
              memcpy(&hh, &h16, 2);
              memcpy(&ll, &l16, 2);
              v = (float)hh + (float)ll;
            } else {
              const uint32_t hb = (uint32_t)h16 << 16, lb = (uint32_t)l16 << 16;
              float hf, lf;
              memcpy(&hf, &hb, 4);
              memcpy(&lf, &lb, 4);
              v = hf + lf;
            }
          } else {
            v = host[t.off(i, y, x) + cc];
          }
          dst[(((size_t)i * ch + c) * t.h + y) * t.w + x] = t.unscale_host ? v * t.unscale_host[cc] : v;
        }
  return TA_OK;
}

}
```

terran_amd/csrc/ta_internal.h:

```cpp
#pragma once
#include <hip/hip_runtime.h>
#include <stdint.h>
#include <stdio.h>
#include <atomic>
#include <map>
#include <mutex>
#include <string>
#include <vector>

#include "../../include/terran_amd.h"

#define TA_BLOB_MAGIC 0x314D4154u

enum {
  TA_OP_CONV = 1,
  TA_OP_DWCONV = 2,
  TA_OP_MAXPOOL = 3,
  TA_OP_COPYCH = 4,
  TA_OP_RFSTEM = 5,
  TA_OP_DWPW = 6
};
enum { TA_ACT_NONE = 0, TA_ACT_RELU = 1, TA_ACT_PRELU = 2 };

struct ta_blob_header {
  uint32_t magic;
  uint32_t version;
  int32_t kind;
  int32_t n_tensors;
  int32_t n_ops;
  int32_t input_tensor;
  int32_t n_outputs;
  int32_t outputs[16];
  int64_t tensors_off, ops_off, weights_off, weights_bytes;
};

struct ta_tensor_desc {
  int32_t channels;
  int32_t halo;
  int32_t alias_of;
  int32_t fmt;
  int32_t unscale_off;
};

struct ta_op_desc {
  int32_t type;
  int32_t in, out;
  int32_t in_ch_off, cin;
  int32_t out_ch_off, cout;
  int32_t coutp;
  int32_t kh, kw, stride, pad;
  int32_t act;
  int32_t res, res_ch_off, res_up2;
  int32_t out2, out2_ch_off;
  int32_t n_slabs;
  int32_t prec;
  int32_t groups;
  int32_t variant;
  int32_t pool;
  int32_t wscale_log2;
  int64_t w_off, bias_off, prelu_off, scale2_off, shift2_off;
  int64_t wus_off;
  double macs_per_pixel;
};

static_assert(sizeof(ta_blob_header) == 128 && sizeof(ta_tensor_desc) == 20 && sizeof(ta_op_desc) == 152,
              "blob layout is shared with terran_amd/pack.py (HEADER_DT / TENSOR_DT / OP_DT)");

struct ta_prof_class {
  double ms = 0;
  int64_t launches = 0;
  double work = 0;
};

struct ta_pending_event {
  hipEvent_t a, b;
  int klass;
  const std::string* kernel;
};

struct ta_ctx {
  int device = -1;
  hipStream_t stream = nullptr;
  std::string err;
  bool profiling = false;
  ta_prof_class prof[4];
  std::vector<ta_pending_event> pending;
  std::vector<hipEvent_t> event_pool;
  hipEvent_t t0 = nullptr, t1 = nullptr;
  void* scratch = nullptr;
  size_t scratch_bytes = 0;
  void* pinned = nullptr;
  size_t pinned_bytes = 0;
  std::mutex frame_cache_mu;
  std::vector<std::pair<size_t, void*>> frame_cache;
  size_t frame_cache_bytes = 0;
  int64_t pose_peaks = 0, pose_connections = 0;
  double jpeg_ms[4] = {0, 0, 0, 0};
  int64_t jpeg_counts[4] = {0, 0, 0, 0};
  double jpeg_enc_ms[8] = {0, 0, 0, 0, 0, 0, 0, 0};
  int64_t jpeg_enc_counts[4] = {0, 0, 0, 0};
  void* jpeg_enc_dev = nullptr;
  size_t jpeg_enc_dev_bytes = 0;
  uint8_t* jpeg_enc_out = nullptr;
  size_t jpeg_enc_out_bytes = 0;
  float* pose_wphase = nullptr;
  struct {
    int n = 0, maxp = 0;
    const int *peak_cnt = nullptr, *peak_yx = nullptr, *conn_cnt = nullptr, *conn_ij = nullptr;
    const float *peak_sc = nullptr, *conn_sc = nullptr;
    struct over_t {
      int img, maxp;
      void* mem;
      const int *peak_cnt, *peak_yx, *conn_cnt, *conn_ij;
      const float *peak_sc, *conn_sc;
    };
    std::vector<over_t> over;
  } pose_dbg;
  hipStream_t side_stream[2] = {nullptr, nullptr};
  hipEvent_t side_fork[2] = {nullptr, nullptr}, side_join[2] = {nullptr, nullptr};
  int conv_force = 0;
#ifdef TA_CONV_TRACE
  int conv_trace_block = 0;
#endif
  int64_t conv_counts[16] = {0};
  int* range_flag = nullptr;
  int* range_flag_host = nullptr;
  const void* amax_owner = nullptr;
  double cur_flops = 0;
  std::map<std::string, std::pair<int64_t, double>> kernel_work;
  std::map<std::string, double> kernel_ms;
  const std::string* cur_kernel = nullptr;
  void note_kernel(const char* name) {
    auto it = kernel_work.try_emplace(name, 0, 0.0).first;
    it->second.first += 1;
    it->second.second += cur_flops;
    cur_kernel = &it->first;
  }
};
void ta_pose_free_big(ta_ctx* ctx);
#define TA_AMAX_SLOT0 16
#define TA_AMAX_OPS 4096
int ta_range_enqueue(ta_ctx* ctx);
int ta_range_check(ta_ctx* ctx);
int ta_range_finish(ta_ctx* ctx, int rc);

enum {
  TA_CV_AUTO = 0,
  TA_CV_GENERIC = 1,
  TA_CV_PIPE64 = 2,
  TA_CV_PIPE128 = 3,
  TA_CV_SPLIT_2x2 = 4,
  TA_CV_SPLIT_2x2_P8 = 5,
  TA_CV_SPLIT_2x4 = 6,
  TA_CV_SPLIT_1x4 = 7,
  TA_CV_WIN_2x2 = 8,
  TA_CV_WIN_2x4 = 9,
  TA_CV_WIN_1x4 = 10,
  TA_CV_SPLIT_1x4_W2 = 11,
  TA_CV_SPLIT_2x2_W2 = 12,
  TA_CV_COUNT = 16
};

#define TA_SET_LDS_ATTR(ctx, kern, bytes)                                                                         \
  do {                                                                                                            \
    static std::atomic<unsigned long long> _done{0};                                                              \
    const unsigned long long _bit = 1ull << ((ctx)->device & 63);                                                 \
    if (!(_done.load(std::memory_order_acquire) & _bit)) {                                                        \
      TA_HIP(ctx, hipFuncSetAttribute((const void*)(kern), hipFuncAttributeMaxDynamicSharedMemorySize, (int)(bytes))); \
      _done.fetch_or(_bit, std::memory_order_release);                                                            \
    }                                                                                                             \
  } while (0)

int ta_fail(ta_ctx* ctx, int code, const char* fmt, ...);
static inline void ta_enter(const ta_ctx* ctx) {
  if (ctx) (void)hipSetDevice(ctx->device);
}
int ta_scratch(ta_ctx* ctx, size_t bytes, void** out);
int ta_pinned(ta_ctx* ctx, size_t bytes, void** out);

#define TA_HIP(ctx, expr)                                                                      \
  do {                                                                                         \
    hipError_t _e = (expr);                                                                    \
    if (_e != hipSuccess)                                                                      \
      return ta_fail((ctx), TA_E_DEVICE, "%s failed: %s (%s:%d)", #expr, hipGetErrorString(_e), \
                     __FILE__, __LINE__);                                                      \
  } while (0)

#define TA_TRY(expr)            \
  do {                          \
    int _r = (expr);            \
    if (_r != TA_OK) return _r; \
  } while (0)

struct ta_prof_scope {
  ta_ctx* ctx;
  int klass;
  double work;
  hipEvent_t a = nullptr, b = nullptr;
  ta_prof_scope(ta_ctx* c, int k, double w);
  ~ta_prof_scope();
};

void ta_drain_profile(ta_ctx* ctx);

struct ta_frames {
  ta_ctx* ctx;
  int n, h, w;
  uint8_t* dev;
  size_t cap = 0;
};
int ta_frames_alloc_uninit(ta_ctx* ctx, int n, int h, int w, ta_frames** out);

struct ta_tensor {
  float* dev = nullptr;
  int n = 0, h = 0, w = 0, c = 0, halo = 0, fmt = 0;
  const float* unscale_dev = nullptr;
  const float* unscale_host = nullptr;
  bool owns = true;
  int hp() const { return h + 2 * halo; }
  int wp() const { return w + 2 * halo; }
  size_t elems() const { return (size_t)n * hp() * wp() * c; }
  int cf() const { return fmt == 3  ? c / 2 : c; }
  size_t off(int img, int y, int x) const { return (((size_t)img * hp() + y + halo) * wp() + x + halo) * cf(); }
};

struct ta_conv_launch {
  const float* in;
  const float* w;
  const int32_t* ktab;
  const float* bias;
  const float* prelu;
  float* out;
  const float* res;
  float* out2;
  const float* scale2;
  const float* shift2;
  int M, Ho, Wo, n_slabs, coutp, cout, act, stride, prec;
  int uniform_k, k_cblocks, k_w, k_h, in_ch_off;
  int in_img, in_row, in_pix, in_off0;
  int out_img, out_row, out_pix, out_off0, out_ch, out_fmt;
  int res_img, res_row, res_pix, res_off0, res_up2, res_ch, res_fmt;
  int o2_img, o2_row, o2_pix, o2_off0, o2_ch, o2_fmt;
  int in_fmt;
  int win_wp, win_img;
  int group_cout, group_cin;
  int k_split;
  float* partial;
  int variant;
  const float* dw_w;
  const float* dw_bias;
  int dw_c, dw_stride;
  int pool;
  float r_nct, r_tile_blocks, r_Wo, r_Ho, r_HoWo;
  int fast_div;
  int fast_drain;
#ifdef TA_CONV_TRACE
  int trace_block;
#endif
  const float* bias9;
  int range_check;
  int amax_index;
  int* range_flag;
};

static inline int ta_split_fmt_of(int prec) { return prec == 0 ? 0  : (prec == 4 ? 3  : ((prec == 3 || prec == 5) ? 2  : 1 )); }

static inline int ta_conv_ksplit(int coutp, int n_slabs, bool eligible, int packed = 0) {
  if (!eligible || coutp % 128) return 1;
  if (packed > 1) return packed <= n_slabs ? packed : 1;
  if (n_slabs < 512) return 1;
  return 32;
}

int ta_launch_conv(ta_ctx* ctx, const ta_conv_launch& p, double flops);
int ta_launch_conv_sym(ta_ctx* ctx, int variant, const ta_conv_launch& p);
int ta_launch_conv_split(ta_ctx* ctx, int variant, const ta_conv_launch& p);
int ta_launch_conv_split_modes(ta_ctx* ctx, int variant, const ta_conv_launch& p);
int ta_launch_dwpw(ta_ctx* ctx, const ta_conv_launch& p, double flops);
int ta_win_patch_rows(const ta_conv_launch& p, int BM);
#define TA_WIN_PR_2x2 384
#define TA_WIN_PR_2x4 448
#define TA_WIN_PR_1x4 512
struct ta_frames;
int ta_launch_rfstem(ta_ctx* ctx, const uint8_t* frames_dev, int n, int h, int w, const float* weights_host, const float* w2_dev, const struct ta_tensor& out);

struct ta_dw_launch {
  const float* in;
  const float* w;
  const float* bias;
  float* out;
  int N, Ho, Wo, C, stride, relu;
  int in_img, in_row, in_pix, in_off0, in_fmt;
  int out_img, out_row, out_pix, out_off0, out_fmt;
};
int ta_launch_dwconv(ta_ctx* ctx, const ta_dw_launch& p);
int ta_launch_maxpool(ta_ctx* ctx, const ta_tensor& in, const ta_tensor& out, int n);
int ta_launch_copych(ta_ctx* ctx, const ta_tensor& in, int in_ch, const ta_tensor& out, int out_ch, int ch, int n);

enum { TA_PRE_RETINAFACE = 1, TA_PRE_OPENPOSE = 2, TA_PRE_ARCFACE_CROPS = 3 };
int ta_launch_preprocess(ta_ctx* ctx, int mode, const uint8_t* src_dev, int n, int h, int w, const ta_tensor& dst);

struct ta_plan {
  int n = 0, h = 0, w = 0;
  std::vector<ta_tensor> tensors;
  char* arena = nullptr;
  size_t arena_bytes = 0;
  int32_t* ktab_dev = nullptr;
  std::vector<size_t> ktab_off;
  float* splitk_ws = nullptr;
  uint64_t last_use = 0;
};

struct ta_model {
  ta_ctx* ctx = nullptr;
  int kind = 0;
  ta_blob_header hdr;
  std::vector<ta_tensor_desc> tdesc;
  std::vector<ta_op_desc> ops;
  char* weights_dev = nullptr;
  bool has_half_ops = false;
  bool amax_on = false;
  std::vector<char> tensor_read;
  std::vector<std::vector<float>> unscale_host;
  std::vector<char> weights_host_small;
  std::vector<ta_plan*> plans;
  ta_plan* active = nullptr;
  uint64_t use_counter = 0;
  int plan_n = 0, plan_h = 0, plan_w = 0;
  int run_n = 0;
  const uint8_t* input_u8 = nullptr;
  std::vector<ta_tensor> tensors;
  int32_t* ktab_dev = nullptr;
  std::vector<size_t> ktab_off;
  float* splitk_ws = nullptr;
};

int ta_model_plan(ta_model* m, int n, int h, int w);
int ta_model_run_ops(ta_model* m);
```

terran_amd/lib.py:

```python
import ctypes as C
import os

import numpy as np

HERE = os.path.dirname(os.path.abspath(__file__))
LIB_PATH = os.path.join(HERE, 'libterran_amd.so')

OK, E_INVALID, E_DEVICE, E_CAPACITY, E_OVERFLOW, E_RANGE = 0, -1, -2, -3, -4, -5
_CODES = {E_INVALID: 'TA_E_INVALID', E_DEVICE: 'TA_E_DEVICE', E_CAPACITY: 'TA_E_CAPACITY', E_OVERFLOW: 'TA_E_OVERFLOW',
          E_RANGE: 'TA_E_RANGE'}


class TerranAmdError(RuntimeError):
    def __init__(self, code, msg):
        super().__init__('%s: %s' % (_CODES.get(code, code), msg))
        self.code = code


c_int, c_float, c_double, c_void_p, c_size_t = C.c_int, C.c_float, C.c_double, C.c_void_p, C.c_size_t
P = C.POINTER
u8p, i32p, f32p, f64p = P(C.c_uint8), P(C.c_int32), P(C.c_float), P(C.c_double)

SIGNATURES = {
    'ta_version': (C.c_char_p, []),
    'ta_device_count': (c_int, []),
    'ta_device_pci_bus_id': (c_int, [c_int, C.c_char_p, c_int]),
    'ta_ctx_create': (c_int, [c_int, P(c_void_p)]),
    'ta_ctx_destroy': (None, [c_void_p]),
    'ta_last_error': (C.c_char_p, [c_void_p]),
    'ta_ctx_sync': (c_int, [c_void_p]),
    'ta_profile_enable': (c_int, [c_void_p, c_int]),
    'ta_profile_reset': (c_int, [c_void_p]),
    'ta_profile_read': (c_int, [c_void_p, c_int, f64p, P(C.c_int64), f64p]),
    'ta_timer_start': (c_int, [c_void_p]),
    'ta_timer_stop': (c_int, [c_void_p, f64p]),
    'ta_host_alloc': (c_int, [c_void_p, c_size_t, P(c_void_p)]),
    'ta_host_free': (None, [c_void_p, c_void_p]),
    'ta_frames_upload': (c_int, [c_void_p, c_void_p, c_int, c_int, c_int, P(c_void_p)]),
    'ta_frames_alloc': (c_int, [c_void_p, c_int, c_int, c_int, P(c_void_p)]),
    'ta_frames_shape': (c_int, [c_void_p, P(c_int), P(c_int), P(c_int)]),
    'ta_frames_download': (c_int, [c_void_p, c_void_p]),
    'ta_frames_free': (None, [c_void_p]),
    'ta_frames_resize': (c_int, [c_void_p, c_void_p, c_int, c_int, P(c_void_p)]),
    'ta_frames_resize_bicubic': (c_int, [c_void_p, c_void_p, c_int, c_int, P(c_void_p)]),
    'ta_frames_paste': (c_int, [c_void_p, c_void_p, c_int, c_void_p, c_int, c_int, c_int]),
    'ta_frames_draw': (c_int, [c_void_p, c_void_p, c_void_p, c_int]),
    'ta_jpeg_coefficients': (c_int, [c_void_p, c_size_t, c_void_p, c_void_p, C.c_int64, C.c_char_p, c_int]),
    'ta_jpeg_decode': (c_int, [c_void_p, P(c_void_p), P(c_size_t), c_int, c_int, c_int, P(c_void_p), P(C.c_int32),
                               P(C.c_int32)]),
    'ta_jpeg_last_stats': (c_int, [c_void_p, c_void_p, c_void_p]),
    'ta_jpeg_encode_header': (c_int, [c_int, c_int, c_int, c_int, c_void_p, c_size_t, P(c_size_t)]),
    'ta_jpeg_encode': (c_int, [c_void_p, c_void_p, c_int, c_int, P(c_void_p), P(c_size_t)]),
    'ta_jpeg_encode_last_stats': (c_int, [c_void_p, c_void_p, c_void_p]),
    'ta_model_load': (c_int, [c_void_p, c_int, c_void_p, c_size_t, P(c_void_p)]),
    'ta_model_free': (None, [c_void_p]),
    'ta_model_kind': (c_int, [c_void_p]),
    'ta_model_forward_frames': (c_int, [c_void_p, c_void_p]),
    'ta_model_forward_crops': (c_int, [c_void_p, c_void_p, c_int]),
    'ta_model_tensor_shape': (c_int, [c_void_p, c_int, P(c_int), P(c_int), P(c_int), P(c_int)]),
    'ta_model_tensor_unscale': (c_int, [c_void_p, c_int, c_void_p, c_int]),
    'ta_model_debug_amax': (c_int, [c_void_p, c_int, c_void_p, c_int]),
    'ta_model_graph_probe': (c_int, [c_void_p, c_int, c_void_p]),
    'ta_model_read_tensor': (c_int, [c_void_p, c_int, c_int, c_int, c_void_p]),
    'ta_retinaface_run': (c_int, [c_void_p, c_void_p, c_float, c_float, c_int, c_void_p, c_void_p, c_void_p,
                                  c_void_p, P(C.c_int32)]),
    'ta_retinaface_postprocess': (c_int, [c_void_p, P(c_void_p), c_int, c_int, c_int, c_float, c_float, c_int,
                                          c_void_p, c_void_p, c_void_p, c_void_p, P(C.c_int32)]),
    'ta_arcface_embed_crops': (c_int, [c_void_p, c_void_p, c_int, c_int, c_void_p]),
    'ta_arcface_embed_faces': (c_int, [c_void_p, c_void_p, c_void_p, c_void_p, c_int, c_int, c_void_p, c_void_p]),
    'ta_arcface_embed_faces_multi': (c_int, [c_void_p, P(c_void_p), c_int, c_void_p, c_void_p, c_void_p, c_int, c_int, c_void_p,
                                             c_void_p]),
    'ta_cosine_distance': (c_int, [c_void_p, c_void_p, c_int, c_void_p, c_int, c_int, c_void_p]),
    'ta_openpose_run': (c_int, [c_void_p, c_void_p, c_double, c_int, c_void_p, c_void_p, c_void_p, P(C.c_int32)]),
    'ta_openpose_group': (c_int, [c_void_p, c_void_p, c_void_p, c_int, c_int, c_int, c_double, c_int, c_void_p,
                                  c_void_p, c_void_p, P(C.c_int32)]),
    'ta_bicubic_x8': (c_int, [c_void_p, c_void_p, c_int, c_int, c_int, c_int, c_void_p]),
    'ta_openpose_last_stats': (c_int, [c_void_p, c_void_p, c_void_p]),
    'ta_openpose_debug_read': (c_int, [c_void_p, c_int, c_int, c_void_p, c_void_p, c_void_p, c_int, c_void_p, c_void_p,
                                       c_void_p]),
    'ta_debug_conv_variant': (c_int, [c_void_p, c_int]),
    'ta_debug_range_check': (c_int, [c_void_p]),
    'ta_debug_conv_counts': (c_int, [c_void_p, c_void_p, c_int]),
    'ta_debug_kernel_work': (c_int, [c_void_p, C.c_char_p, c_size_t, c_int]),
}

DRAW_BAR, DRAW_LINE, DRAW_DISC = 0, 1, 2
PRIM_DT = np.dtype([('frame', '<i4'), ('kind', '<i4'), ('x0', '<i4'), ('y0', '<i4'), ('x1', '<i4'), ('y1', '<i4'),
                    ('width', '<i4'), ('rgba', 'u1', (4,))])
assert PRIM_DT.itemsize == 32

JPEG_DEVICE = 0
JPEG_INVALID = -1
JPEG_PATHS = {-1: 'invalid', 0: 'device', 1: 'progressive/lossless/hierarchical', 2: 'arithmetic', 3: 'precision',
              4: 'components', 5: 'rgb', 6: 'scans', 7: 'sampling'}
JPEG_HEADER_DT = np.dtype([('width', '<i4'), ('height', '<i4'), ('components', '<i4'), ('path', '<i4'),
                           ('h_samp', '<i4', (3,)), ('v_samp', '<i4', (3,)), ('quant_index', '<i4', (3,)),
                           ('blocks_w', '<i4', (3,)), ('blocks_h', '<i4', (3,)), ('restart_interval', '<i4'),
                           ('reserved', '<i4', (2,)), ('block_offset', '<i8', (3,)), ('blocks_total', '<i8'),
                           ('quant', '<u2', (4, 64))])
assert JPEG_HEADER_DT.itemsize == 632


def jpeg_coefficients(data, header_only=False):
    lib = load()
    buf = np.frombuffer(bytes(data), np.uint8)
    hdr = np.zeros(1, JPEG_HEADER_DT)
    err = C.create_string_buffer(256)
    rc = lib.ta_jpeg_coefficients(ptr(buf), buf.size, ptr(hdr), None, 0, err, len(err))
    if rc != OK:
        raise TerranAmdError(rc, err.value.decode(errors='replace'))
    if header_only or hdr['path'][0] != JPEG_DEVICE:
        return hdr[0], None
    coefs = np.empty((int(hdr['blocks_total'][0]), 64), np.int16)
    rc = lib.ta_jpeg_coefficients(ptr(buf), buf.size, ptr(hdr), ptr(coefs), coefs.shape[0], err, len(err))
    if rc != OK:
        raise TerranAmdError(rc, err.value.decode(errors='replace'))
    return hdr[0], coefs


def jpeg_encode_header(h, w, quality=75, subsampling=2):
    lib = load()
    size = c_size_t()
    buf = np.zeros(1024, np.uint8)
    rc = lib.ta_jpeg_encode_header(int(h), int(w), int(quality), int(subsampling), ptr(buf), buf.size, C.byref(size))
    if rc != OK:
        raise TerranAmdError(rc, 'jpeg_encode_header(%r, %r, %r, %r)' % (h, w, quality, subsampling))
    return buf[:size.value].tobytes()


def check_jpeg_options(quality, subsampling):
    if isinstance(quality, bool) or not isinstance(quality, (int, np.integer)) or not 1 <= quality <= 100:
        raise ValueError('JPEG quality must be an int in 1..100, got %r' % (quality,))
    if isinstance(subsampling, bool) or not isinstance(subsampling, (int, np.integer)) or subsampling not in (0, 1, 2):
        raise ValueError('JPEG subsampling must be 0 (4:4:4), 1 (4:2:2) or 2 (4:2:0), got %r' % (subsampling,))
    return int(quality), int(subsampling)


CONV_VARIANTS = {'auto': 0, 'generic': 1, 'pipe64': 2, 'pipe128': 3, 'split_2x2': 4, 'split_2x2_p8': 5, 'split_2x4': 6,
                 'split_1x4': 7, 'win_2x2': 8, 'win_2x4': 9, 'win_1x4': 10, 'split_1x4_w2': 11, 'split_2x2_w2': 12}

_lib = None


def load():
    global _lib
    if _lib is None:
        if not os.path.exists(LIB_PATH):
            raise TerranAmdError(E_DEVICE, 'libterran_amd.so not built (run `python -m terran_amd.build`); '
                                           'there is no CPU fallback')
        from . import build as _build
        try:
            with open(_build.STAMP) as fh:
                stamp = fh.read().strip()
        except OSError:
            stamp = None
        try:
            current = _build.source_hash()
        except OSError:
            current = stamp
        if (stamp is None or stamp != current) and not os.environ.get('TA_ALLOW_STALE_LIB'):
            raise TerranAmdError(E_DEVICE, 'libterran_amd.so was not built from the sources in terran_amd/csrc '
                                           '(run `python -m terran_amd.build`)')
        os.environ.setdefault('GPU_MAX_HW_QUEUES', '12')
        os.environ.setdefault('HIP_FORCE_DEV_KERNARG', '1')
        lib = C.CDLL(LIB_PATH)
        missing = []
        for name, (res, args) in SIGNATURES.items():
            try:
                fn = getattr(lib, name)
            except AttributeError:
                missing.append(name)
                continue
            fn.restype = res
            fn.argtypes = args
        if missing and not os.environ.get('TA_BRINGUP_ALLOW_MISSING'):
            raise TerranAmdError(E_INVALID, 'libterran_amd.so lacks ABI symbols: %s' % ', '.join(missing))
        _lib = lib
    return _lib


def ptr(a):
    return a.ctypes.data_as(c_void_p) if a is not None else None


class Context:

    def __init__(self, device_id=0):
        self.lib = load()
        h = c_void_p()
        rc = self.lib.ta_ctx_create(int(device_id), C.byref(h))
        if rc != OK:
            raise TerranAmdError(rc, 'ta_ctx_create(%d) failed: no usable gfx950 device '
                                     '(ta_device_count=%d)' % (device_id, self.lib.ta_device_count()))
        self.h = h
        self.device_id = device_id

    def check(self, rc):
        if rc != OK:
            raise TerranAmdError(rc, self.lib.ta_last_error(self.h).decode(errors='replace'))

    def last_error(self):
        return self.lib.ta_last_error(self.h).decode(errors='replace')

    def sync(self):
        self.check(self.lib.ta_ctx_sync(self.h))

    def close(self):
        if getattr(self, 'h', None):
            self.lib.ta_ctx_destroy(self.h)
            self.h = None

    def __del__(self):
        try:
            self.close()
        except Exception:
            pass

    def profile(self, on):
        self.check(self.lib.ta_profile_enable(self.h, int(on)))

    def profile_reset(self):
        self.check(self.lib.ta_profile_reset(self.h))

    def profile_read(self, klass):
        ms, n, w = c_double(), C.c_int64(), c_double()
        self.check(self.lib.ta_profile_read(self.h, klass, C.byref(ms), C.byref(n), C.byref(w)))
        return ms.value, n.value, w.value

    def timer_start(self):
        self.check(self.lib.ta_timer_start(self.h))

    def timer_stop(self):
        ms = c_double()
        self.check(self.lib.ta_timer_stop(self.h, C.byref(ms)))
        return ms.value

    def upload(self, images):
        images = np.ascontiguousarray(images, dtype=np.uint8)
        assert images.ndim == 4 and images.shape[3] == 3
        return Frames(self, images)

    def pinned_array(self, shape):
        n = int(np.prod(shape))
        p = c_void_p()
        self.check(self.lib.ta_host_alloc(self.h, n, C.byref(p)))
        arr = np.ctypeslib.as_array((C.c_uint8 * n).from_address(p.value)).reshape(shape)
        arr_ptr = p.value
        return arr, arr_ptr

    def free_pinned(self, ptr):
        if getattr(self, 'h', None):
            self.lib.ta_host_free(self.h, c_void_p(ptr))

    def cosine_distance(self, a, b):
        a = np.ascontiguousarray(a, dtype=np.float32)
        b = np.ascontiguousarray(b, dtype=np.float32)
        out = np.empty((a.shape[0], b.shape[0]), np.float32)
        self.check(self.lib.ta_cosine_distance(self.h, ptr(a), a.shape[0], ptr(b), b.shape[0], a.shape[1], ptr(out)))
        return out

    def jpeg_decode(self, buffers, threads=0):
        bufs = [bytes(b) for b in buffers]
        n = len(bufs)
        arrs = [np.frombuffer(b, np.uint8) for b in bufs]
        data = (c_void_p * n)(*[a.ctypes.data for a in arrs])
        sizes = (c_size_t * n)(*[a.size for a in arrs])
        out = (c_void_p * n)()
        paths = np.zeros(n, np.int32)
        req = C.c_int32()
        rc = self.lib.ta_jpeg_decode(self.h, data, sizes, n, int(threads), n, out, paths.ctypes.data_as(P(C.c_int32)),
                                     C.byref(req))
        if rc != OK:
            e = TerranAmdError(rc, self.last_error())
            e.paths = paths
            raise e
        return [Frames(self, handle=c_void_p(out[k])) for k in range(req.value)], paths

    def jpeg_stats(self):
        ms, cnt = np.zeros(4, np.float64), np.zeros(4, np.int64)
        self.check(self.lib.ta_jpeg_last_stats(self.h, ptr(ms), ptr(cnt)))
        return (dict(zip(('host', 'h2d', 'idct', 'color'), ms.tolist())),
                dict(zip(('images', 'blocks', 'bytes', 'fallbacks'), cnt.tolist())))

    def jpeg_encode(self, frames, quality=75, subsampling=2):
        quality, subsampling = check_jpeg_options(quality, subsampling)
        n = frames.shape[0]
        out = c_void_p()
        sizes = (c_size_t * n)()
        self.check(self.lib.ta_jpeg_encode(self.h, frames.h, quality, subsampling, C.byref(out), sizes))
        files, at = [], out.value
        for k in range(n):
            files.append(C.string_at(at, sizes[k]))
            at += sizes[k]
        return files

    def jpeg_encode_stats(self):
        ms, cnt = np.zeros(8, np.float64), np.zeros(4, np.int64)
        self.check(self.lib.ta_jpeg_encode_last_stats(self.h, ptr(ms), ptr(cnt)))
        return (dict(zip(('h2d', 'coef', 'length', 'emit', 'ffcount', 'pack', 'd2h', 'host'), ms.tolist())),
                dict(zip(('images', 'blocks', 'bytes', 'entropy_bytes'), cnt.tolist())))

    def conv_variant(self, name):
        self.check(self.lib.ta_debug_conv_variant(self.h, CONV_VARIANTS[name]))

    def conv_counts(self, reset=False):
        c = np.zeros(16, np.int64)
        self.check(self.lib.ta_debug_conv_counts(self.h, ptr(c), int(reset)))
        out = {k: int(c[v]) for k, v in CONV_VARIANTS.items() if v and c[v]}
        if c[15]:
            out['lean_epilogue'] = int(c[15])
        return out

    def kernel_work(self, reset=False):
        buf = C.create_string_buffer(1 << 16)
        self.check(self.lib.ta_debug_kernel_work(self.h, buf, len(buf), int(reset)))
        out = {}
        for line in buf.value.decode().splitlines():
            f = line.split(';')
            out[f[0]] = (int(f[1]), float(f[2]), float(f[3]) if len(f) > 3 else 0.0)
        return out

    def pose_debug(self, n, cap_peaks=1024, cap_conn=1024):
        pc = np.zeros((n, 18), np.int32)
        pyx = np.zeros((n, 18, cap_peaks, 2), np.int32)
        psc = np.zeros((n, 18, cap_peaks), np.float32)
        cc = np.zeros((n, 19), np.int32)
        cij = np.zeros((n, 19, cap_conn, 2), np.int32)
        csc = np.zeros((n, 19, cap_conn), np.float32)
        self.check(self.lib.ta_openpose_debug_read(self.h, n, cap_peaks, ptr(pc), ptr(pyx), ptr(psc), cap_conn,
                                                   ptr(cc), ptr(cij), ptr(csc)))
        assert pc.max(initial=0) <= cap_peaks and cc.max(initial=0) <= cap_conn
        peaks = [[(pyx[i, p, :pc[i, p]].copy(), psc[i, p, :pc[i, p]].copy()) for p in range(18)] for i in range(n)]
        conns = [[None if cc[i, l] < 0 else (cij[i, l, :cc[i, l]].copy(), csc[i, l, :cc[i, l]].copy())
                  for l in range(19)] for i in range(n)]
        return peaks, conns

    def pose_stats(self):
        a, b = C.c_int64(), C.c_int64()
        self.check(self.lib.ta_openpose_last_stats(self.h, C.byref(a), C.byref(b)))
        return a.value, b.value

    def bicubic_x8(self, maps):
        maps = np.ascontiguousarray(maps, dtype=np.float32)
        n, c, h, w = maps.shape
        out = np.empty((n, c, 8 * h, 8 * w), np.float32)
        self.check(self.lib.ta_bicubic_x8(self.h, ptr(maps), n, c, h, w, ptr(out)))
        return out


class Frames:

    def __init__(self, ctx, images=None, handle=None):
        self.ctx = ctx
        if handle is not None:
            self.h = handle
        else:
            h = c_void_p()
            n, hh, ww = images.shape[:3]
            ctx.check(ctx.lib.ta_frames_upload(ctx.h, ptr(images), n, hh, ww, C.byref(h)))
            self.h = h
        n, hh, ww = c_int(), c_int(), c_int()
        ctx.lib.ta_frames_shape(self.h, C.byref(n), C.byref(hh), C.byref(ww))
        self.shape = (n.value, hh.value, ww.value, 3)

    def __len__(self):
        return self.shape[0]

    @classmethod
    def zeros(cls, ctx, n, h, w):
        hd = c_void_p()
        ctx.check(ctx.lib.ta_frames_alloc(ctx.h, n, h, w, C.byref(hd)))
        return cls(ctx, handle=hd)

    def resize(self, h, w, ctx=None):
        ctx = ctx or self.ctx
        hd = c_void_p()
        ctx.check(ctx.lib.ta_frames_resize(ctx.h, self.h, int(h), int(w), C.byref(hd)))
        return Frames(ctx, handle=hd)

    def resize_bicubic(self, h, w, ctx=None):
        ctx = ctx or self.ctx
        hd = c_void_p()
        ctx.check(ctx.lib.ta_frames_resize_bicubic(ctx.h, self.h, int(h), int(w), C.byref(hd)))
        return Frames(ctx, handle=hd)

    def paste(self, src, src_index, dst_index, top, left):
        self.ctx.check(self.ctx.lib.ta_frames_paste(self.ctx.h, src.h, src_index, self.h, dst_index, top, left))

    def draw(self, prims, ctx=None):
        ctx = ctx or self.ctx
        prims = np.ascontiguousarray(prims, dtype=PRIM_DT)
        ctx.check(ctx.lib.ta_frames_draw(ctx.h, self.h, ptr(prims) if len(prims) else None, len(prims)))

    def encode_jpeg(self, quality=75, subsampling=2, ctx=None):
        return (ctx or self.ctx).jpeg_encode(self, quality, subsampling)

    def download(self):
        out = np.empty(self.shape, np.uint8)
        self.ctx.check(self.ctx.lib.ta_frames_download(self.h, ptr(out)))
        return out

    def free(self):
        if getattr(self, 'h', None) and getattr(self.ctx, 'h', None):
            self.ctx.lib.ta_frames_free(self.h)
        self.h = None

    def __del__(self):
        try:
            self.free()
        except Exception:
            pass


class Model:

    def __init__(self, ctx, program):
        self.ctx = ctx
        self.kind = program.kind
        self.names = dict(program.names)
        blob = program.blob()
        buf = np.frombuffer(blob, dtype=np.uint8)
        h = c_void_p()
        ctx.check(ctx.lib.ta_model_load(ctx.h, program.kind, ptr(buf), len(blob), C.byref(h)))
        self.h = h

    def forward_frames(self, frames):
        self.ctx.check(self.ctx.lib.ta_model_forward_frames(self.h, frames.h))

    def forward_crops(self, crops):
        crops = np.ascontiguousarray(crops, dtype=np.uint8)
        self.ctx.check(self.ctx.lib.ta_model_forward_crops(self.h, ptr(crops), crops.shape[0]))

    def read(self, name):
        tid, off, ch = self.names[name]
        n, c, h, w = c_int(), c_int(), c_int(), c_int()
        self.ctx.check(self.ctx.lib.ta_model_tensor_shape(self.h, tid, C.byref(n), C.byref(c), C.byref(h), C.byref(w)))
        out = np.empty((n.value, ch, h.value, w.value), np.float32)
        self.ctx.check(self.ctx.lib.ta_model_read_tensor(self.h, tid, off, ch, ptr(out)))
        return out

    def read_tensor(self, tid, ch_off=0, ch=None):
        n, c, h, w = c_int(), c_int(), c_int(), c_int()
        self.ctx.check(self.ctx.lib.ta_model_tensor_shape(self.h, tid, C.byref(n), C.byref(c), C.byref(h), C.byref(w)))
        ch = c.value - ch_off if ch is None else ch
        out = np.empty((n.value, ch, h.value, w.value), np.float32)
        self.ctx.check(self.ctx.lib.ta_model_read_tensor(self.h, tid, ch_off, ch, ptr(out)))
        return out

    def tensor_unscale(self, tid, channels):
        out = np.empty(channels, np.float32)
        self.ctx.check(self.ctx.lib.ta_model_tensor_unscale(self.h, tid, ptr(out), channels))
        return out

    def amax_collect(self, on=True):
        self.ctx.check(self.ctx.lib.ta_model_debug_amax(self.h, int(bool(on)), None, 0))

    def graph_probe(self, reps=20):
        out = np.zeros(5, np.float64)
        self.ctx.check(self.ctx.lib.ta_model_graph_probe(self.h, int(reps), ptr(out)))
        return tuple(float(x) for x in out)

    def amax_read(self, n_ops):
        out = np.zeros(2 * n_ops, np.float32)
        n = c_int()
        self.ctx.check(self.ctx.lib.ta_model_debug_amax(self.h, 2, ptr(out), out.size))
        return out.reshape(n_ops, 2)

    def free(self):
        if getattr(self, 'h', None) and getattr(self.ctx, 'h', None):
            self.ctx.lib.ta_model_free(self.h)
        self.h = None

    def __del__(self):
        try:
            self.free()
        except Exception:
            pass
```

terran_amd/pack.py:

```python
import os

import numpy as np

from . import arch

MODEL_RETINAFACE, MODEL_ARCFACE, MODEL_OPENPOSE = 1, 2, 3
OP_CONV, OP_DWCONV, OP_MAXPOOL, OP_COPYCH, OP_RFSTEM, OP_DWPW = 1, 2, 3, 4, 5, 6
ACT_NONE, ACT_RELU, ACT_PRELU = 0, 1, 2
MAGIC = 0x314D4154

HEADER_DT = np.dtype({
    'names': ['magic', 'version', 'kind', 'n_tensors', 'n_ops', 'input_tensor', 'n_outputs', 'outputs',
              'tensors_off', 'ops_off', 'weights_off', 'weights_bytes'],
    'formats': ['<u4', '<u4', '<i4', '<i4', '<i4', '<i4', '<i4', ('<i4', 16), '<i8', '<i8', '<i8', '<i8'],
    'offsets': [0, 4, 8, 12, 16, 20, 24, 28, 96, 104, 112, 120],
    'itemsize': 128,
})
TENSOR_DT = np.dtype([('channels', '<i4'), ('halo', '<i4'), ('alias_of', '<i4'), ('fmt', '<i4'), ('unscale_off', '<i4')])
FMT_F32, FMT_SPLIT, FMT_SPLIT16, FMT_F16 = 0, 1, 2, 3
_OP_I32 = ['type', 'in', 'out', 'in_ch_off', 'cin', 'out_ch_off', 'cout', 'coutp', 'kh', 'kw', 'stride', 'pad',
           'act', 'res', 'res_ch_off', 'res_up2', 'out2', 'out2_ch_off', 'n_slabs', 'prec', 'groups', 'variant', 'pool', 'wscale_log2']
_OP_I64 = ['w_off', 'bias_off', 'prelu_off', 'scale2_off', 'shift2_off', 'wus_off']
OP_DT = np.dtype([(n, '<i4') for n in _OP_I32] + [(n, '<i8') for n in _OP_I64] + [('macs_per_pixel', '<f8')])
assert OP_DT.itemsize == 152 and TENSOR_DT.itemsize == 20
BLOB_VERSION = 9


PACK_SWITCHES = ('TERRAN_AMD_NO_FUSED_POOL', 'TERRAN_AMD_NO_GROUPED', 'TERRAN_AMD_NO_MERGED_OUTPUTS', 'TERRAN_AMD_ARCFACE_SECOND_OUTPUT',
                 'TERRAN_AMD_NO_STAGE4_KSPLIT', 'TERRAN_AMD_DETECTOR_F32', 'TERRAN_AMD_DETECTOR_BASE_F32', 'TERRAN_AMD_NO_FUSED_DETECTOR', 'TERRAN_AMD_NO_FUSED_FRONT',
                 'TERRAN_AMD_NO_DETECTOR_LANES', 'TERRAN_AMD_NO_ACT_SCALES')


def active_switches():
    return tuple((k, os.environ[k]) for k in PACK_SWITCHES if os.environ.get(k))


_SOURCE_TAG = []


def source_tag():
    if not _SOURCE_TAG:
        import hashlib
        h = hashlib.sha256()
        here = os.path.dirname(os.path.abspath(__file__))
        try:
            for f in ('pack.py', 'arch.py'):
                with open(os.path.join(here, f), 'rb') as fh:
                    h.update(fh.read())
            _SOURCE_TAG.append(h.hexdigest()[:10])
        except OSError:
            _SOURCE_TAG.append(None)
    return _SOURCE_TAG[0]


PRECISIONS = {'f32': 0, 'bf16x3': 1, 'bf16': 2, 'f16x3': 3, 'f16': 4, 'f16x2': 5}
SPLIT_FMT = {0: FMT_F32, 1: FMT_SPLIT, 2: FMT_SPLIT, 3: FMT_SPLIT16, 4: FMT_F16, 5: FMT_SPLIT16}


def _rup(x, m):
    return (x + m - 1) // m * m


def _bf16_bits(x):
    u = np.ascontiguousarray(x, dtype=np.float32).view(np.uint32)
    return ((u + np.uint32(0x7FFF) + ((u >> np.uint32(16)) & np.uint32(1))) >> np.uint32(16)).astype(np.uint16)


def _bf16_to_f32(b):
    return (b.astype(np.uint32) << np.uint32(16)).view(np.float32)


def split_bf16_rows(packed):
    hi = _bf16_bits(packed)
    lo = _bf16_bits(packed - _bf16_to_f32(hi))
    rows = np.concatenate([hi, lo], axis=-1)
    return np.ascontiguousarray(rows).view(np.float32)


def row_exponents(packed):
    m = np.abs(np.asarray(packed, np.float32)).max(axis=(0, 2)).astype(np.float64)
    ok = np.isfinite(m) & (m > 0)
    s = np.zeros(m.shape, np.int64)
    s[ok] = np.clip(13 - np.floor(np.log2(m[ok])), -60, 60).astype(np.int64)
    return s


def split_f16_rows(packed, exps=None):
    packed = np.ascontiguousarray(packed, dtype=np.float32)
    s = row_exponents(packed) if exps is None else np.asarray(exps, np.int64)
    scaled = np.ldexp(packed, s[None, :, None].astype(np.int32)).astype(np.float32)
    hi = scaled.astype(np.float16)
    lo = (scaled - hi.astype(np.float32)).astype(np.float16)
    rows = np.concatenate([hi.view(np.uint16), lo.view(np.uint16)], axis=-1)
    return np.ascontiguousarray(rows).view(np.float32), s


_SQRT2, _SQRT2PI = np.sqrt(2.0), np.sqrt(2.0 * np.pi)
_TAP_CORR = 0.5
_ACT_TARGET_LOG2 = 10
_ACT_SIGMAS = 6.0
_CH_SPREAD = 8


def _erf(x):
    from math import erf
    return np.vectorize(erf, otypes=[np.float64])(x)


def act_moments(mu, var, act, slope=None):
    if act == ACT_NONE:
        return mu, var
    mu, var = np.asarray(mu, np.float64), np.maximum(np.asarray(var, np.float64), 1e-60)
    sd = np.sqrt(var)
    t = mu / sd
    Phi = 0.5 * (1.0 + _erf(t / _SQRT2))
    phi = np.exp(-0.5 * t * t) / _SQRT2PI
    m_pos = mu * Phi + sd * phi
    s_pos = (mu * mu + var) * Phi + mu * sd * phi
    m_neg = -mu * (1.0 - Phi) + sd * phi
    s_neg = (mu * mu + var) * (1.0 - Phi) - mu * sd * phi
    a = np.zeros_like(mu) if (act == ACT_RELU or slope is None) else np.asarray(slope, np.float64)
    m = m_pos - a * m_neg
    s2 = s_pos + a * a * s_neg
    return m, np.maximum(s2 - m * m, 0.0)


def fold_input_affine(W, bias, scale, shift):
    W = np.asarray(W, np.float64)
    a_s, a_t = np.asarray(scale, np.float64), np.asarray(shift, np.float64)
    T = np.einsum('ocyx,c->oyx', W, a_t)
    b0 = np.zeros(W.shape[0]) if bias is None else np.asarray(bias, np.float64)
    valid = ([1, 2], [0, 1, 2], [0, 1], [1])
    bias16 = np.stack([b0 + T[:, valid[cy]][:, :, valid[cx]].sum((1, 2)) for cy in range(4) for cx in range(4)])
    return W * a_s[None, :, None, None], bias16


class Program:

    def __init__(self, kind, precision='f32'):
        self.kind = kind
        self.precision = precision
        self.prec = PRECISIONS[precision]
        self.tensors = []
        self.ops = []
        self.wchunks = []
        self.wbytes = 0
        self.names = {}
        self.extra = {}
        self.input_tensor = None
        self.outputs = []
        self.f32_only = set()
        self.allow_split = True
        self._raw = {}
        self._chunk_at = {}
        self.lane = 0
        self.stats = {}
        self._chunk_size = {}
        self._fold = {}
        self.input_stats = None
        self.forced_scale = {}
        self.scales_enabled = not os.environ.get('TERRAN_AMD_NO_ACT_SCALES')

    def tensor(self, channels, halo, alias_of=-1, name=None, f32=False):
        assert channels % 4 == 0
        self.tensors.append((channels, halo, alias_of))
        tid = len(self.tensors) - 1
        if f32:
            self.f32_only.add(tid)
        if name:
            self.names[name] = (tid, 0, channels)
        return tid

    def tap(self, name, tid, ch_off, ch):
        self.names[name] = (tid, ch_off, ch)

    def _w(self, arr):
        arr = np.ascontiguousarray(arr, dtype=np.float32)
        off = self.wbytes
        self._chunk_at[off] = len(self.wchunks)
        self.wchunks.append(arr.tobytes())
        pad = (-len(self.wchunks[-1])) % 256
        if pad:
            self.wchunks.append(b'\0' * pad)
        self.wbytes += arr.nbytes + pad
        return off

    def _w_reserve(self, nbytes):
        off = self.wbytes
        self._chunk_at[off] = len(self.wchunks)
        self._chunk_size[off] = int(nbytes)
        self.wchunks.append(None)
        pad = (-int(nbytes)) % 256
        if pad:
            self.wchunks.append(b'\0' * pad)
        self.wbytes += int(nbytes) + pad
        return off

    def _rewrite(self, off, arr, raw=False):
        k = self._chunk_at[off]
        data = arr if raw else np.ascontiguousarray(arr, dtype=np.float32).tobytes()
        size = self._chunk_size.get(off, None if self.wchunks[k] is None else len(self.wchunks[k]))
        assert len(data) == size, (len(data), size)
        self.wchunks[k] = data

    def _stats_of(self, tid):
        c = self.tensors[tid][0]
        a = self.tensors[tid][2]
        if a >= 0:
            mu, var, wr, am = self._stats_of(a)
            rep = c // len(mu)
            return [np.tile(mu, rep), np.tile(var, rep), np.tile(wr, rep), np.tile(am, rep)]
        if tid not in self.stats:
            mu, var = np.zeros(c), np.ones(c)
            if tid == self.input_tensor and self.input_stats is not None:
                m_, v_ = self.input_stats
                mu[:len(m_)], var[:len(v_)] = m_, v_
            self.stats[tid] = [mu, var, np.zeros(c, bool), np.abs(mu) + _ACT_SIGMAS * np.sqrt(var)]
            if tid == self.input_tensor:
                self.stats[tid][2][:] = True
        return self.stats[tid]

    def _write_stats(self, tid, ch_off, mu, var, amax=None):
        st = self._stats_of(tid)
        n = len(mu)
        if amax is None:
            amax = np.abs(mu) + _ACT_SIGMAS * np.sqrt(var)
        new = ~st[2][ch_off:ch_off + n]
        take = new | (amax > st[3][ch_off:ch_off + n])
        st[0][ch_off:ch_off + n][take] = mu[take]
        st[1][ch_off:ch_off + n][take] = var[take]
        st[3][ch_off:ch_off + n] = np.where(new, amax, np.maximum(amax, st[3][ch_off:ch_off + n]))
        st[2][ch_off:ch_off + n] = True

    @staticmethod
    def _act_bound(mu, var, act, slope=None):
        sd = np.sqrt(np.maximum(var, 0.0))
        hi, lo = mu + _ACT_SIGMAS * sd, _ACT_SIGMAS * sd - mu
        if act == ACT_NONE:
            return np.maximum(hi, lo)
        if act == ACT_RELU or slope is None:
            return np.maximum(hi, 4.0 * sd)
        a = np.abs(np.asarray(slope, np.float64))
        return np.maximum(np.maximum(hi, a * lo), 4.0 * sd * np.maximum(a, 1.0))

    @staticmethod
    def _conv_moments(full, bias, mu_in, var_in, groups, cout):
        taps, cin_p, coutp = full.shape
        f64 = full.astype(np.float64)
        wsum = f64.sum(0)
        wsq = (f64 * f64).sum(0)
        rho = _TAP_CORR if taps > 1 else 0.0
        wvar = (1.0 - rho) * wsq + rho * wsum * wsum
        mu = np.zeros(coutp)
        var = np.zeros(coutp)
        if groups > 1:
            cg = cout // groups
            for g in range(groups):
                sl = slice(g * cg, (g + 1) * cg)
                mu[sl] = mu_in[g * cin_p:(g + 1) * cin_p] @ wsum[:, sl]
                var[sl] = var_in[g * cin_p:(g + 1) * cin_p] @ wvar[:, sl]
        else:
            mu = mu_in[:cin_p] @ wsum
            var = var_in[:cin_p] @ wvar
        b = np.zeros(coutp)
        if bias is not None:
            b[:cout] = np.asarray(bias, np.float64)
        return (mu + b)[:cout], np.maximum(var[:cout], 0.0)

    def conv(self, tin, tout, W, bias, *, stride=1, pad=None, act=ACT_NONE, in_ch_off=0, ch_pos=None, cin_p=None,
             out_ch_off=0, cout_p=None, prelu=None, res=-1, res_ch_off=0, res_up2=0, out2=-1, out2_ch_off=0,
             scale2=None, shift2=None, groups=1, variant=0, pool=False, k_split=0, precision=None, in_affine=None):
        W = np.asarray(W, dtype=np.float64)
        cout, cin, kh, kw = W.shape
        bias9 = None
        if in_affine is not None:
            assert (kh, kw, stride) == (3, 3, 1) and pad in (None, 1) and groups == 1 and out2 < 0 and scale2 is None and not pool
            W, bias9 = fold_input_affine(W, bias, *in_affine)
            bias = bias9[5]
        if groups > 1:
            assert cout % groups == 0 and cin % 32 == 0 and (cout // groups) % 128 == 0 and ch_pos is None
        if pad is None:
            pad = kh // 2
        if pool:
            assert groups == 1 and res < 0 and out2 < 0 and stride == 1 and cin % 32 == 0 and cout % 64 == 0 and ch_pos is None
        if cin_p is None:
            cin_p = _rup(cin, 4)
        if ch_pos is None:
            ch_pos = np.arange(cin)
        if cout_p is None:
            cout_p = _rup(cout, 4)
        coutp = _rup(cout_p, 32)
        K = kh * kw * cin_p
        n_slabs = _rup(K, 32) // 32
        full = np.zeros((kh * kw, cin_p, coutp), np.float32)
        full[:, np.asarray(ch_pos), :cout] = W.transpose(2, 3, 1, 0).reshape(kh * kw, cin, cout)
        flat = np.zeros((n_slabs * 32, coutp), np.float32)
        flat[:K] = full.reshape(K, coutp)
        prec = self.prec if precision is None else PRECISIONS[precision]

        def vec(v, fill=0.0):
            if v is None:
                return -1, None
            out = np.full(coutp, fill, np.float64)
            out[:cout] = np.asarray(v, dtype=np.float64)
            return self._w(out), out
        fold = dict(flat=flat, taps=kh * kw, cin_p=cin_p, K=K)
        scale2_off = -1
        if bias9 is not None:
            t9 = np.zeros((16, coutp), np.float64)
            t9[:, :cout] = bias9
            scale2_off = self._w(t9)
            fold['bias9'] = t9
            variant |= 1 << 16
        else:
            scale2_off, fold['scale2'] = vec(scale2)
        bvec = np.zeros(coutp, np.float64)
        if bias is not None:
            bvec[:cout] = np.asarray(bias, np.float64)
        fold['bias'] = bvec
        bias_off = self._w(np.concatenate([bvec, np.ones(coutp)]))
        wus_off = bias_off + 4 * coutp
        prelu_off, _ = vec(prelu)
        shift2_off, fold['shift2'] = vec(shift2)
        op = dict(type=OP_CONV, out=tout, in_ch_off=in_ch_off, cin=cin_p, out_ch_off=out_ch_off, cout=cout_p,
                  coutp=coutp, kh=kh, kw=kw, stride=stride, pad=pad, act=act, res=res, res_ch_off=res_ch_off,
                  res_up2=res_up2, out2=out2, out2_ch_off=out2_ch_off, n_slabs=n_slabs, prec=prec,
                  groups=groups, variant=variant | (int(k_split) << 8) | (self.lane << 17), pool=int(bool(pool)), wscale_log2=0,
                  w_off=self._w_reserve(n_slabs * coutp * 128), bias_off=bias_off, prelu_off=prelu_off, scale2_off=scale2_off,
                  shift2_off=shift2_off, wus_off=wus_off, macs_per_pixel=float(cout * cin * kh * kw))
        op['in'] = tin
        self._fold[len(self.ops)] = fold
        self.ops.append(op)
        st_in = self._stats_of(tin)
        span = cin_p * max(groups, 1)
        mu, var = self._conv_moments(full, bias, st_in[0][in_ch_off:in_ch_off + span], st_in[1][in_ch_off:in_ch_off + span],
                                     groups, cout)
        slope = None if prelu is None else np.asarray(prelu, np.float64)
        bound = self._act_bound(mu, var, act, slope)
        mu, var = act_moments(mu, var, act, slope)
        if res >= 0:
            st_r = self._stats_of(res)
            mu = mu + st_r[0][res_ch_off:res_ch_off + cout]
            var = var + st_r[1][res_ch_off:res_ch_off + cout]
            bound = bound + st_r[3][res_ch_off:res_ch_off + cout]
        if pool:
            mu, var = mu + 1.03 * np.sqrt(var), 0.49 * var
        self._write_stats(tout, out_ch_off, mu, var, bound)
        if out2 >= 0:
            s2, h2 = np.asarray(scale2, np.float64), np.asarray(shift2, np.float64)
            self._write_stats(out2, out2_ch_off, mu * s2 + h2, var * s2 * s2, np.abs(s2) * bound + np.abs(h2))

    def dwconv(self, tin, tout, W, bias, *, stride=1, relu=True):
        C = W.shape[0]
        w9 = np.asarray(W, dtype=np.float64).reshape(C, 9).T
        op = dict(type=OP_DWCONV, out=tout, in_ch_off=0, cin=C, out_ch_off=0, cout=C, coutp=_rup(C, 32), kh=3,
                  kw=3, stride=stride, pad=1, act=ACT_RELU if relu else ACT_NONE, res=-1, res_ch_off=0, res_up2=0,
                  out2=-1, out2_ch_off=0, n_slabs=0, prec=0, groups=1, variant=0, pool=0, wscale_log2=0, w_off=self._w(w9), bias_off=self._w(bias),
                  prelu_off=-1, scale2_off=-1, shift2_off=-1, wus_off=-1, macs_per_pixel=float(C * 9))
        op['in'] = tin
        self.ops.append(op)
        st = self._stats_of(tin)
        mu, var = self._dw_moments(w9, bias, st[0][:C], st[1][:C])
        act = ACT_RELU if relu else ACT_NONE
        self._write_stats(tout, 0, *act_moments(mu, var, act), self._act_bound(mu, var, act))

    @staticmethod
    def _dw_moments(w9, bias, mu_in, var_in):
        w9 = np.asarray(w9, np.float64)
        wsum, wsq = w9.sum(0), (w9 * w9).sum(0)
        return (np.asarray(bias, np.float64) + mu_in * wsum,
                var_in * ((1.0 - _TAP_CORR) * wsq + _TAP_CORR * wsum * wsum))

    def rfstem(self, tin, tout, Ws, bs, Wd, bd, Wp, bp, Wd2=None, bd2=None, Wp2=None, bp2=None):
        parts = [np.asarray(Ws, np.float64).reshape(8, 27).ravel(), np.asarray(bs, np.float64),
                 np.asarray(Wd, np.float64).reshape(8, 9).T.ravel(), np.asarray(bd, np.float64),
                 np.asarray(Wp, np.float64).reshape(16, 8).ravel(), np.asarray(bp, np.float64)]
        fuse = Wd2 is not None
        if fuse:
            parts += [np.asarray(Wd2, np.float64).reshape(16, 9).T.ravel(), np.asarray(bd2, np.float64),
                      np.asarray(Wp2, np.float64).reshape(32, 16).T.ravel(), np.asarray(bp2, np.float64)]
        blob = np.concatenate(parts)
        assert blob.size == (448 + 704 if fuse else 448)
        op = dict(type=OP_RFSTEM, out=tout, in_ch_off=0, cin=4, out_ch_off=0, cout=32 if fuse else 16, coutp=32, kh=3, kw=3, stride=2,
                  pad=1, act=ACT_RELU, res=-1, res_ch_off=0, res_up2=0, out2=-1, out2_ch_off=0, n_slabs=0, prec=0, groups=1,
                  variant=0, pool=0, wscale_log2=0, w_off=self._w(blob), bias_off=-1, prelu_off=-1, scale2_off=-1, shift2_off=-1,
                  wus_off=-1, macs_per_pixel=float(8 * 27 + 16 * 8) + (32 * 16 / 4.0 if fuse else 0.0))
        op['in'] = tin
        self._fold[len(self.ops)] = dict(rfstem=parts)
        self.ops.append(op)
        st = self._stats_of(tin)
        ws = np.asarray(Ws, np.float64)
        wsum, wsq = ws.sum((2, 3)), (ws * ws).sum((2, 3))
        mu = np.asarray(bs, np.float64) + wsum @ st[0][:3]
        var = ((1.0 - _TAP_CORR) * wsq + _TAP_CORR * wsum * wsum) @ st[1][:3]
        mu, var = act_moments(mu, var, ACT_RELU)
        mu, var = self._dw_moments(np.asarray(Wd, np.float64).reshape(8, 9).T, bd, mu, var)
        mu, var = act_moments(mu, var, ACT_RELU)
        wp = np.asarray(Wp, np.float64).reshape(16, 8)
        mu, var = np.asarray(bp, np.float64) + wp @ mu, (wp * wp) @ var
        if fuse:
            mu, var = act_moments(mu, var, ACT_RELU)
            mu, var = self._dw_moments(np.asarray(Wd2, np.float64).reshape(16, 9).T, bd2, mu, var)
            mu, var = act_moments(mu, var, ACT_RELU)
            wp2 = np.asarray(Wp2, np.float64).reshape(32, 16)
            mu, var = np.asarray(bp2, np.float64) + wp2 @ mu, (wp2 * wp2) @ var
        self._write_stats(tout, 0, *act_moments(mu, var, ACT_RELU), self._act_bound(mu, var, ACT_RELU))

    def dwpw(self, tin, tout, Wd, bd, Wp, bp, *, stride=1, precision=None):
        prec = self.prec if precision is None else PRECISIONS[precision]
        assert prec in (0, 3), 'the fused depthwise + pointwise block exists in the f32 and f16x3 modes'
        C = Wd.shape[0]
        Wp = np.asarray(Wp, np.float64)
        cout = Wp.shape[0]
        assert Wp.shape[1] == C and C % 4 == 0 and cout % 4 == 0
        coutp = _rup(cout, 32)
        n_slabs = _rup(C, 32) // 32
        flat = np.zeros((n_slabs * 32, coutp), np.float32)
        flat[:C, :cout] = Wp.reshape(cout, C).T
        bias = np.zeros(coutp, np.float64)
        bias[:cout] = np.asarray(bp, np.float64)
        w9 = np.asarray(Wd, np.float64).reshape(C, 9).T
        bd = np.asarray(bd, np.float64)
        op = dict(type=OP_DWPW, out=tout, in_ch_off=0, cin=C, out_ch_off=0, cout=cout, coutp=coutp, kh=1, kw=1,
                  stride=stride, pad=0, act=ACT_RELU, res=-1, res_ch_off=0, res_up2=0, out2=-1, out2_ch_off=0,
                  n_slabs=n_slabs, prec=prec, groups=1, variant=0, pool=0, wscale_log2=0, w_off=self._w_reserve(n_slabs * coutp * 128),
                  bias_off=self._w(np.concatenate([bias, np.ones(coutp)])), prelu_off=-1,
                  scale2_off=self._w(w9), shift2_off=self._w(bd), wus_off=-1,
                  macs_per_pixel=float(cout * C))
        op['wus_off'] = op['bias_off'] + 4 * coutp
        op['in'] = tin
        st = self._stats_of(tin)
        mu0, var0 = self._dw_moments(w9, bd, st[0][:C], st[1][:C])
        mid_bound = self._act_bound(mu0, var0, ACT_RELU)
        mu, var = act_moments(mu0, var0, ACT_RELU)
        self._fold[len(self.ops)] = dict(flat=flat, bias=bias, dw_w=w9, dw_b=bd, mid_bound=mid_bound)
        self.ops.append(op)
        wp = Wp.reshape(cout, C)
        mu2, var2 = bias[:cout] + wp @ mu, (wp * wp) @ var
        self._write_stats(tout, 0, *act_moments(mu2, var2, ACT_RELU), self._act_bound(mu2, var2, ACT_RELU))

    def simple(self, typ, tin, tout, in_ch_off=0, out_ch_off=0, ch=0):
        op = dict(type=typ, out=tout, in_ch_off=in_ch_off, cin=ch, out_ch_off=out_ch_off, cout=ch, coutp=0, kh=2,
                  kw=2, stride=2, pad=0, act=0, res=-1, res_ch_off=0, res_up2=0, out2=-1, out2_ch_off=0, n_slabs=0,
                  prec=0, groups=1, variant=0, pool=0, wscale_log2=0, w_off=-1, bias_off=-1, prelu_off=-1, scale2_off=-1, shift2_off=-1,
                  wus_off=-1, macs_per_pixel=0.0)
        op['in'] = tin
        self.ops.append(op)
        st = self._stats_of(tin)
        if typ == OP_MAXPOOL:
            self._write_stats(tout, 0, st[0] + 1.03 * np.sqrt(st[1]), 0.49 * st[1], st[3].copy())
        else:
            self._write_stats(tout, out_ch_off, st[0][in_ch_off:in_ch_off + ch].copy(), st[1][in_ch_off:in_ch_off + ch].copy(),
                              st[3][in_ch_off:in_ch_off + ch].copy())

    @classmethod
    def from_cache(cls, path):
        import json
        with open(path, 'rb') as f:
            head = f.read(16)
            if head[:8] != b'TAMCACHE':
                raise ValueError('not a pack cache file')
            n = int.from_bytes(head[8:16], 'little')
            meta = json.loads(f.read(n).decode())
            blob = f.read()
        self = cls(meta['kind'], meta['precision'])
        self.names = {k: tuple(v) for k, v in meta['names'].items()}
        self.outputs = meta['outputs']
        self.extra = dict(meta.get('extra') or {})
        self._blob = blob
        return self

    def save_cache(self, path):
        import json
        import os
        meta = json.dumps({'kind': self.kind, 'precision': self.precision, 'names': self.names,
                           'outputs': [int(o) for o in self.outputs], 'extra': getattr(self, 'extra', {})}).encode()
        tmp = path + '.tmp.%d' % os.getpid()
        with open(tmp, 'wb') as f:
            f.write(b'TAMCACHE' + len(meta).to_bytes(8, 'little') + meta + self.blob())
        os.replace(tmp, path)

    def tensor_formats(self):
        n = len(self.tensors)
        cprec = {}
        for op in self.ops:
            if op['type'] == OP_CONV:
                cprec.setdefault(op['in'], set()).add(op['prec'])
        fmt = []
        for t, (c, _, _) in enumerate(self.tensors):
            precs = cprec.get(t, {self.prec})
            p = next(iter(precs)) if len(precs) == 1 else 0
            fmt.append(SPLIT_FMT[p] if (self.allow_split and c % (64 if p == 4 else 32) == 0) else FMT_F32)
        for t in self.f32_only | {self.input_tensor}:
            fmt[t] = FMT_F32
        for op in self.ops:
            if op['type'] == OP_CONV:
                taps = op['kh'] * op['kw']
                pipe = (op['cin'] % 32 == 0 and op['in_ch_off'] % 32 == 0 and op['coutp'] % 64 == 0
                        and op['n_slabs'] >= 2 and op['n_slabs'] == taps * (op['cin'] // 32))
                if op['prec'] == 4:
                    k64 = op['cin'] % 64 == 0 and op['n_slabs'] == taps * (op['cin'] // 64)
                    pipe = (pipe or (k64 and op['coutp'] % 64 == 0)) and \
                        op['cin'] % 64 == 0 and op['in_ch_off'] == 0 and op['groups'] == 1
                if op['out_ch_off'] % 8 or op['res_ch_off'] % 8 or op['out2_ch_off'] % 8:
                    pipe = False
                if not pipe:
                    fmt[op['in']] = FMT_F32
            elif op['type'] in (OP_DWPW, OP_RFSTEM):
                fmt[op['in']] = FMT_F32
                if op['type'] == OP_RFSTEM:
                    fmt[op['out']] = FMT_F32
            elif op['type'] == OP_COPYCH:
                if op['cin'] % 32 or op['in_ch_off'] % 32 or op['out_ch_off'] % 32:
                    fmt[op['in']] = fmt[op['out']] = FMT_F32
            if op['type'] != OP_CONV:
                for t in (op['in'], op['out']):
                    if fmt[t] == FMT_F16:
                        fmt[t] = FMT_F32
        changed = True
        while changed:
            changed = False
            for t, (_, _, a) in enumerate(self.tensors):
                if a >= 0 and fmt[t] != fmt[a]:
                    fmt[t] = fmt[a] = FMT_F32
                    changed = True
            for op in self.ops:
                if op['type'] == OP_COPYCH and fmt[op['in']] != fmt[op['out']]:
                    fmt[op['in']] = fmt[op['out']] = FMT_F32
                    changed = True
        return fmt

    def expected_amax(self, tid, per_channel=False):
        st = self._stats_of(tid)
        am = np.where(st[2], st[3], 0.0)
        return am if per_channel else float(am.max()) if len(am) else 0.0

    def tensor_scales(self):
        n = len(self.tensors)
        sizes = [t[0] for t in self.tensors]
        scales = [np.zeros(c, np.int64) for c in sizes]
        if not self.scales_enabled or not any(op['type'] in (OP_CONV, OP_DWPW) and op['prec'] in (3, 4, 5) for op in self.ops):
            return scales
        base = np.concatenate([[0], np.cumsum(sizes)]).astype(np.int64)
        parent = np.arange(base[-1], dtype=np.int64)

        def find(x):
            r = x
            while parent[r] != r:
                r = parent[r]
            while parent[x] != r:
                parent[x], x = r, parent[x]
            return r

        def union_run(ta, ca, tb, cb, cnt):
            for i in range(cnt):
                ra, rb = find(base[ta] + ca + i), find(base[tb] + cb + i)
                if ra != rb:
                    parent[ra] = rb
        for t, (c, _, a) in enumerate(self.tensors):
            if a >= 0:
                ca = sizes[a]
                for p in range(c):
                    ra, rb = find(base[t] + p), find(base[a] + p % ca)
                    if ra != rb:
                        parent[ra] = rb
        fixed_t = set(self.f32_only) | {self.input_tensor}
        for op in self.ops:
            if op['type'] == OP_MAXPOOL:
                union_run(op['in'], 0, op['out'], 0, sizes[op['in']])
            elif op['type'] == OP_COPYCH:
                union_run(op['in'], op['in_ch_off'], op['out'], op['out_ch_off'], op['cin'])
            elif op['type'] == OP_DWCONV:
                fixed_t |= {op['in'], op['out']}
            elif op['type'] == OP_CONV and op['res'] >= 0:
                union_run(op['res'], op['res_ch_off'], op['out'], op['out_ch_off'], op['cout'])
        amax = np.concatenate([self.expected_amax(t, per_channel=True) for t in range(n)])
        for t in range(n):
            seg = amax[base[t]:base[t + 1]]
            if len(seg) and seg.max() > 0:
                np.maximum(seg, np.where(seg > 0, seg.max() * 2.0 ** -_CH_SPREAD, 0.0), out=seg)
        roots = np.array([find(i) for i in range(base[-1])], np.int64)
        gmax = np.zeros(base[-1])
        np.maximum.at(gmax, roots, amax)
        fixed = np.zeros(base[-1], bool)
        for t in fixed_t:
            fixed[roots[base[t]:base[t + 1]]] = True
        forced = {}
        for t, e in self.forced_scale.items():
            if isinstance(t, (int, np.integer)):
                for r in roots[base[t]:base[t + 1]]:
                    forced[int(r)] = int(e)
        g = gmax[roots]
        ok = np.isfinite(g) & (g > 0) & ~fixed[roots]
        expo = np.zeros(base[-1], np.int64)
        expo[ok] = np.clip(_ACT_TARGET_LOG2 - np.ceil(np.log2(g[ok])), -40, 40).astype(np.int64)
        for r, e in forced.items():
            if not fixed[r]:
                expo[roots == r] = e
        return [expo[base[t]:base[t + 1]].copy() for t in range(n)]

    def _pack_conv_weights(self, op, f, a_in):
        flat, taps, cin_p, K = f['flat'], f['taps'], f['cin_p'], f['K']
        coutp, groups = op['coutp'], max(op['groups'], 1)
        cols = a_in[op['in_ch_off']:op['in_ch_off'] + cin_p * groups]
        fs = flat
        if np.any(cols != 0):
            fs = flat.copy()
            if groups > 1:
                cg = op['cout'] // groups
                for g_ in range(groups):
                    e = -np.tile(cols[g_ * cin_p:(g_ + 1) * cin_p], taps).astype(np.int32)
                    fs[:K, g_ * cg:(g_ + 1) * cg] = np.ldexp(flat[:K, g_ * cg:(g_ + 1) * cg], e[:, None])
            else:
                fs[:K] = np.ldexp(flat[:K], -np.tile(cols[:cin_p], taps).astype(np.int32)[:, None])
        n_slabs = flat.shape[0] // 32
        packed = fs.reshape(n_slabs, 32, coutp).transpose(0, 2, 1)
        wexp = np.zeros(coutp, np.int64)
        if op['prec'] in (3, 4, 5):
            packed, wexp = split_f16_rows(packed)
        elif op['prec'] != 0:
            packed = split_bf16_rows(np.ascontiguousarray(packed))
        return np.ascontiguousarray(packed, dtype=np.float32).tobytes(), wexp, fs

    def blob(self):
        if getattr(self, '_blob', None) is not None:
            return self._blob
        hdr = np.zeros(1, HEADER_DT)
        tens = np.zeros(len(self.tensors), TENSOR_DT)
        fmts = self.tensor_formats()
        scales = self.tensor_scales()
        self.scales = scales
        unscale_off = []
        for i, (c, h, a) in enumerate(self.tensors):
            unscale_off.append(self._w(np.ldexp(np.ones(c), -scales[i].astype(np.int32))) if np.any(scales[i] != 0) else -1)
            assert unscale_off[-1] < 2 ** 31
            tens[i] = (c, h, a, fmts[i], unscale_off[-1])
        self.mid_scales = {}
        for i, f in self._fold.items():
            op = self.ops[i]
            a_in = scales[op['in']]
            a_out = np.zeros(op['coutp'], np.int64)
            if op['type'] in (OP_CONV, OP_DWPW, OP_RFSTEM):
                seg = scales[op['out']][op['out_ch_off']:op['out_ch_off'] + op['cout']]
                a_out[:len(seg)] = seg
            up = np.ldexp(1.0, a_out.astype(np.int32))
            if op['type'] == OP_CONV:
                data, wexp, fs = self._pack_conv_weights(op, f, a_in)
                if op['prec'] == 4 and fmts[op['in']] == FMT_F16:
                    cin_p, K, coutp = f['cin_p'], f['K'], op['coutp']
                    assert cin_p % 64 == 0 and op['in_ch_off'] == 0 and op['groups'] == 1
                    rows = np.ldexp(fs[:K].reshape(K // 64, 64, coutp).transpose(0, 2, 1), wexp[None, :, None].astype(np.int32)).astype(np.float16)
                    assert rows.nbytes * 2 == len(data)
                    data = rows.tobytes() + b'\0' * rows.nbytes
                    op['n_slabs'] = K // 64
                    f['rows64'] = rows
                f['wexp'] = wexp
                self._rewrite(op['w_off'], data, raw=True)
                self._rewrite(op['bias_off'], np.concatenate([f['bias'] * up, np.ldexp(np.ones(op['coutp']), (a_out - wexp).astype(np.int32))]))
                if 'bias9' in f:
                    self._rewrite(op['scale2_off'], f['bias9'] * up[None, :])
                elif op['out2'] >= 0:
                    a2 = np.zeros(op['coutp'], np.int64)
                    seg = scales[op['out2']][op['out2_ch_off']:op['out2_ch_off'] + op['cout']]
                    a2[:len(seg)] = seg
                    self._rewrite(op['scale2_off'], f['scale2'] * np.ldexp(1.0, (a2 - a_out).astype(np.int32)))
                    self._rewrite(op['shift2_off'], f['shift2'] * np.ldexp(1.0, a2.astype(np.int32)))
            elif op['type'] == OP_DWPW:
                C = op['cin']
                a_mid = np.zeros(C, np.int64)
                if op['prec'] == 3 and self.scales_enabled:
                    mb = f['mid_bound']
                    okc = np.isfinite(mb) & (mb > 0)
                    mbf = np.maximum(mb, mb[okc].max() * 2.0 ** -_CH_SPREAD) if okc.any() else mb
                    a_mid[okc] = np.clip(_ACT_TARGET_LOG2 - np.ceil(np.log2(mbf[okc])), -40, 40).astype(np.int64)
                elif op['prec'] == 0:
                    a_mid = a_in[:C].copy()
                if ('mid', i) in self.forced_scale:
                    a_mid[:] = int(self.forced_scale[('mid', i)])
                self.mid_scales[i] = a_mid
                self._rewrite(op['scale2_off'], f['dw_w'] * np.ldexp(1.0, (a_mid - a_in[:C]).astype(np.int32))[None, :])
                self._rewrite(op['shift2_off'], f['dw_b'] * np.ldexp(1.0, a_mid.astype(np.int32)))
                fl = f['flat'].copy()
                fl[:C] = np.ldexp(fl[:C], -a_mid.astype(np.int32)[:, None])
                n_slabs = fl.shape[0] // 32
                packed = np.ascontiguousarray(fl.reshape(n_slabs, 32, op['coutp']).transpose(0, 2, 1))
                wexp = np.zeros(op['coutp'], np.int64)
                if op['prec'] == 3:
                    packed, wexp = split_f16_rows(packed)
                self._rewrite(op['w_off'], np.ascontiguousarray(packed, dtype=np.float32).tobytes(), raw=True)
                self._rewrite(op['bias_off'], np.concatenate([f['bias'] * up, np.ldexp(np.ones(op['coutp']), (a_out - wexp).astype(np.int32))]))
            elif op['type'] == OP_RFSTEM:
                parts = list(f['rfstem'])
                if len(parts) == 10:
                    parts[8] = (parts[8].reshape(16, 32) * up[None, :32]).ravel()
                    parts[9] = parts[9] * up[:32]
                else:
                    parts[4] = (parts[4].reshape(16, 8) * up[:16, None]).ravel()
                    parts[5] = parts[5] * up[:16]
                self._rewrite(op['w_off'], np.concatenate(parts))
        ops = np.zeros(len(self.ops), OP_DT)
        for i, op in enumerate(self.ops):
            for k, v in op.items():
                ops[i][k] = v
        t_off = HEADER_DT.itemsize
        o_off = t_off + tens.nbytes
        w_off = _rup(o_off + ops.nbytes, 256)
        outs = np.full(16, -1, np.int32)
        outs[:len(self.outputs)] = self.outputs
        hdr[0] = (MAGIC, BLOB_VERSION, self.kind, len(self.tensors), len(self.ops), self.input_tensor, len(self.outputs), outs,
                  t_off, o_off, w_off, self.wbytes)
        head = hdr.tobytes() + tens.tobytes() + ops.tobytes()
        for f in self._fold.values():
            f.pop('flat', None)
        self._blob = head + b'\0' * (w_off - len(head)) + b''.join(self.wchunks)
        return self._blob


def _bn_affine(sd, key, eps):
    g = np.asarray(sd[key + '.weight'], np.float64)
    b = np.asarray(sd[key + '.bias'], np.float64)
    m = np.asarray(sd[key + '.running_mean'], np.float64)
    v = np.asarray(sd[key + '.running_var'], np.float64)
    s = g / np.sqrt(v + eps)
    return s, b - m * s


def _fold(W, bias, scale, shift):
    W = np.asarray(W, np.float64) * scale[:, None, None, None]
    b0 = np.zeros(W.shape[0]) if bias is None else np.asarray(bias, np.float64)
    return W, b0 * scale + shift


OP_FEAT, OP_PAF, OP_HM, OP_XCH = 0, 128, 168, 192


def pack_openpose(sd, precision='f32'):
    if precision in ('f16', 'f16x2'):
        precision = 'f16x3'
    P = Program(MODEL_OPENPOSE, precision)
    t = P.tensor(4, 1, name='input')
    P.input_tensor = t
    P.input_stats = (np.array([-0.05, -0.05, -0.05, 0.0]), np.array([0.08, 0.08, 0.08, 0.0]))
    X0 = P.tensor(OP_XCH, 3, name='X0')
    X1 = P.tensor(OP_XCH, 3, name='X1')
    items = arch.OPENPOSE_MODEL0
    fuse_pool = not os.environ.get('TERRAN_AMD_NO_FUSED_POOL')
    skip_pool = False
    for i, item in enumerate(items):
        nxt = items[i + 1] if i + 1 < len(items) else None
        if item[0] == 'pool':
            if skip_pool:
                skip_pool = False
                continue
            o = P.tensor(P.tensors[t][0], 1)
            P.simple(OP_MAXPOOL, t, o)
            t = o
            continue
        name, cin, cout, k = item
        W, b = sd['model0.%s.weight' % name], sd['model0.%s.bias' % name]
        if nxt is None:
            P.conv(t, X0, W, b, act=ACT_RELU, out_ch_off=OP_FEAT)
            P.tap('feat', X0, OP_FEAT, 128)
        elif nxt[0] == 'pool' and fuse_pool and cin % 32 == 0 and cout % 64 == 0:
            o = P.tensor(cout, 1, name=name + '_pooled')
            P.conv(t, o, W, b, act=ACT_RELU, pool=True)
            t = o
            skip_pool = True
        else:
            o = P.tensor(cout, 0 if nxt[0] == 'pool' else 1, name=name)
            P.conv(t, o, W, b, act=ACT_RELU)
            t = o
    P.simple(OP_COPYCH, X0, X1, OP_FEAT, OP_FEAT, 128)

    cat_pos = np.concatenate([OP_PAF + np.arange(38), OP_HM + np.arange(19), OP_FEAT + np.arange(128)])
    for st in range(1, 7):
        xin, xout = (X0, X1) if st % 2 == 1 else (X1, X0)
        l1, l2 = arch.openpose_stage_layers(st, 1), arch.openpose_stage_layers(st, 2)
        (n1, cin, c1, k, r1), (n2, cin2, c2, k2, r2) = l1[0], l2[0]
        assert (cin, k, r1) == (cin2, k2, r2) and c1 == c2 == 128
        W = np.concatenate([np.asarray(sd['model%d_%d.%s.weight' % (st, br, n)]) for br, n in ((1, n1), (2, n2))])
        b = np.concatenate([np.asarray(sd['model%d_%d.%s.bias' % (st, br, n)]) for br, n in ((1, n1), (2, n2))])
        kw = dict(ch_pos=cat_pos, cin_p=OP_XCH) if cin == 185 else dict(in_ch_off=OP_FEAT)
        cur = P.tensor(c1 + c2, l1[1][3] // 2)
        P.conv(xin, cur, W, b, act=ACT_RELU if r1 else ACT_NONE, **kw)
        grouped = not os.environ.get('TERRAN_AMD_NO_GROUPED')
        for li in range(1, len(l1) - 1):
            (na, cin, cout, k, relu), (nb, cin2, cout2, k2, relu2) = l1[li], l2[li]
            if not grouped:
                o = P.tensor(2 * cout, l1[li + 1][3] // 2)
                for br, n in ((1, na), (2, nb)):
                    key = 'model%d_%d.%s' % (st, br, n)
                    P.conv(cur, o, sd[key + '.weight'], sd[key + '.bias'], act=ACT_RELU if relu else ACT_NONE,
                           in_ch_off=(br - 1) * cin, out_ch_off=(br - 1) * cout)
                cur = o
                continue
            assert (cin, cout, k, relu) == (cin2, cout2, k2, relu2) and cin % 32 == 0 and cout % 128 == 0
            W = np.concatenate([np.asarray(sd['model%d_%d.%s.weight' % (st, br, n)]) for br, n in ((1, na), (2, nb))])
            b = np.concatenate([np.asarray(sd['model%d_%d.%s.bias' % (st, br, n)]) for br, n in ((1, na), (2, nb))])
            o = P.tensor(2 * cout, l1[li + 1][3] // 2)
            P.conv(cur, o, W, b, act=ACT_RELU if relu else ACT_NONE, groups=2)
            cur = o
        (np_, cin, co1, k, r1), (nh, cin2, co2, k2, r2) = l1[-1], l2[-1]
        if r1 == r2 and cin == cin2 <= 128 and not os.environ.get('TERRAN_AMD_NO_MERGED_OUTPUTS'):
            Wp, bp = np.asarray(sd['model%d_1.%s.weight' % (st, np_)]), np.asarray(sd['model%d_1.%s.bias' % (st, np_)])
            Wh, bh = np.asarray(sd['model%d_2.%s.weight' % (st, nh)]), np.asarray(sd['model%d_2.%s.bias' % (st, nh)])
            Wm = np.zeros((60, 2 * cin, 1, 1), np.float32)
            bm = np.zeros(60, np.float32)
            Wm[0:co1, :cin], bm[0:co1] = Wp, bp
            Wm[40:40 + co2, cin:], bm[40:40 + co2] = Wh, bh
            P.conv(cur, xout, Wm, bm, act=ACT_RELU if r1 else ACT_NONE, out_ch_off=OP_PAF, cout_p=60)
            P.ops[-1]['macs_per_pixel'] = float((co1 + co2) * cin)
        else:
            for br, layers in ((1, l1), (2, l2)):
                name, cin, cout, k, relu = layers[-1]
                key = 'model%d_%d.%s' % (st, br, name)
                off, cp = (OP_PAF, 40) if br == 1 else (OP_HM, 20)
                P.conv(cur, xout, sd[key + '.weight'], sd[key + '.bias'], act=ACT_RELU if relu else ACT_NONE,
                       in_ch_off=(br - 1) * cin, out_ch_off=off, cout_p=cp)
        P.tap('stage%d_paf' % st, xout, OP_PAF, 38)
        P.tap('stage%d_hm' % st, xout, OP_HM, 19)
    P.outputs = [X0]
    P.tap('pafs', X0, OP_PAF, 38)
    P.tap('heatmaps', X0, OP_HM, 19)
    return P


def pack_arcface(sd, precision='f32'):
    eps = arch.ARC_BN_EPS
    P = Program(MODEL_ARCFACE, precision)
    tin = P.tensor(4, 1, name='input')
    P.input_tensor = tin
    P.input_stats = (np.array([-0.1, -0.1, -0.1, 0.0]), np.array([0.25, 0.25, 0.25, 0.0]))
    units = list(arch.arcface_units())
    second = bool(os.environ.get('TERRAN_AMD_ARCFACE_SECOND_OUTPUT'))

    def next_bn(i):
        if i < len(units):
            st, u = units[i][0], units[i][1]
            return _bn_affine(sd, 'stages.%d.%d.body.0' % (st, u), eps)
        return _bn_affine(sd, 'final_layer.0', eps)

    s, sh = _bn_affine(sd, 'initial_layer.1', eps)
    W, b = _fold(sd['initial_layer.0.weight'], None, s, sh)
    R = P.tensor(64, 0 if second else 1, name='stem')
    Z = None
    if second:
        s2, sh2 = next_bn(0)
        Z = P.tensor(64, 1)
        P.conv(tin, R, W, b, act=ACT_PRELU, prelu=sd['initial_layer.2.weight'], out2=Z, scale2=s2, shift2=sh2)
    else:
        P.conv(tin, R, W, b, act=ACT_PRELU, prelu=sd['initial_layer.2.weight'])
    for i, (st, u, cin, cout, stride, sc) in enumerate(units):
        p = 'stages.%d.%d' % (st, u)
        s, sh = _bn_affine(sd, p + '.body.2', eps)
        W1, b1 = _fold(sd[p + '.body.1.weight'], None, s, sh)
        Y = P.tensor(cout, 1)
        ks = 2 if (cout == 512 and not os.environ.get('TERRAN_AMD_NO_STAGE4_KSPLIT')) else 0
        if second:
            P.conv(Z, Y, W1, b1, act=ACT_PRELU, prelu=sd[p + '.body.3.weight'], k_split=ks if cin == 512 else 0)
        else:
            P.conv(R, Y, W1, b1, act=ACT_PRELU, prelu=sd[p + '.body.3.weight'], k_split=ks if cin == 512 else 0,
                   in_affine=next_bn(i))
        if sc:
            s, sh = _bn_affine(sd, p + '.shortcut.1', eps)
            Ws, bs = _fold(sd[p + '.shortcut.0.weight'], None, s, sh)
            S = P.tensor(cout, 0)
            P.conv(R, S, Ws, bs, stride=stride, pad=0)
            res = S
        else:
            res = R
        s, sh = _bn_affine(sd, p + '.body.5', eps)
        W2, b2 = _fold(sd[p + '.body.4.weight'], None, s, sh)
        last = i == len(units) - 1
        Rn = P.tensor(cout, 0 if (second or last) else 1)
        if second:
            Zn = P.tensor(cout, 0 if last else 1)
            s2, sh2 = next_bn(i + 1)
            P.conv(Y, Rn, W2, b2, stride=stride, res=res, out2=Zn, scale2=s2, shift2=sh2, k_split=ks)
            Z = Zn
        else:
            P.conv(Y, Rn, W2, b2, stride=stride, res=res, k_split=ks)
        if u == arch.ARC_UNITS[st] - 1:
            P.tap('stage%d' % (st + 1), Rn, 0, cout)
        R = Rn
    s, sh = _bn_affine(sd, 'final_layer.4', eps)
    Wl = np.asarray(sd['final_layer.3.weight'], np.float64) * s[:, None]
    bl = np.asarray(sd['final_layer.3.bias'], np.float64) * s + sh
    f = np.arange(7 * 7 * 512)
    ch_pos = (f % 49) * 512 + f // 49
    if second:
        A = P.tensor(7 * 7 * 512, 0, alias_of=Z)
    else:
        s0, t0 = next_bn(len(units))
        chan = f // 49
        bl = bl + Wl @ t0[chan]
        Wl = Wl * s0[chan][None, :]
        A = P.tensor(7 * 7 * 512, 0, alias_of=R)
    E = P.tensor(512, 0, name='embedding', f32=True)
    P.conv(A, E, Wl.reshape(512, 7 * 7 * 512, 1, 1), bl, ch_pos=ch_pos, pad=0, k_split=32 if P.prec == 4 else 0)
    P.outputs = [E]
    return P


def pack_retinaface(sd, precision='f32', fused=None):
    if precision in ('f16', 'f16x2'):
        precision = 'f16x3'
    det_prec = 'f32' if precision in ('bf16x3', 'f16x3') else precision
    P = Program(MODEL_RETINAFACE, det_prec)
    refiner_prec = 'f16x3' if (precision == 'f16x3' and not os.environ.get('TERRAN_AMD_DETECTOR_F32')) else None
    P.allow_split = refiner_prec is not None
    if fused is None:
        fused = P.prec == 0 and not os.environ.get('TERRAN_AMD_NO_FUSED_DETECTOR')
    tin = P.tensor(4, 1, alias_of=-2 if fused else -1, name='input')
    P.input_tensor = tin
    P.input_stats = (np.array([110.0, 110.0, 110.0, 0.0]), np.array([4900.0, 4900.0, 4900.0, 0.0]))
    eps = arch.RETINA_BASE_BN_EPS

    def cbr(key_conv, key_bn, e=eps, bias=False):
        s, sh = _bn_affine(sd, key_bn, e)
        return _fold(sd[key_conv + '.weight'], sd[key_conv + '.bias'] if bias else None, s, sh)

    pw_keys = [('base.scales.%d.%d.conv_block.0' % (si, bi), 'base.scales.%d.%d.conv_block.1' % (si, bi), cout, both)
               for si, scale in enumerate(arch.RETINA_SCALES) for bi, (cin, cout, stride, both) in enumerate(scale)]
    pw_keys += [('base.final_conv.0.conv_block.0', 'base.final_conv.0.conv_block.1', 256, False),
                ('base.final_conv.1', 'base.final_conv.2', 256, True)]
    dw_keys = [('base.first_conv_block.3', 'base.first_conv_block.4', 1)]
    dw_keys += [('base.scales.%d.%d.sep_block.0' % (si, bi), 'base.scales.%d.%d.sep_block.1' % (si, bi), stride)
                for si, scale in enumerate(arch.RETINA_SCALES) for bi, (cin, cout, stride, both) in enumerate(scale)]
    dw_keys += [('base.final_conv.0.sep_block.0', 'base.final_conv.0.sep_block.1', 1)]
    assert len(pw_keys) == len(dw_keys) == 13
    feats = []
    if fused:
        Ws, bs = cbr('base.first_conv_block.0', 'base.first_conv_block.1')
        t = None
        fuse_front = not os.environ.get('TERRAN_AMD_NO_FUSED_FRONT')
        front = None
        for i, ((dk, dbn, stride), (pk, pbn, cout, both)) in enumerate(zip(dw_keys, pw_keys)):
            Wd, bd = cbr(dk, dbn)
            Wp, bp = cbr(pk, pbn)
            if i == 0 and fuse_front:
                front = (Wd, bd, Wp, bp)
                continue
            c = P.tensor(cout, 1 if i < 12 else 0)
            if i == 0:
                P.rfstem(tin, c, Ws, bs, Wd, bd, Wp, bp)
            elif i == 1 and front is not None:
                assert stride == 2 and cout == 32 and Wd.shape[0] == 16 and not both
                P.rfstem(tin, c, Ws, bs, *front, Wd, bd, Wp, bp)
            else:
                P.dwpw(t, c, Wd, bd, Wp, bp, stride=stride,
                       precision=refiner_prec if (Wd.shape[0] >= 64 and not os.environ.get('TERRAN_AMD_DETECTOR_BASE_F32')) else None)
            if both:
                feats.append(c)
            t = c
    else:
        W, b = cbr('base.first_conv_block.0', 'base.first_conv_block.1')
        a0 = P.tensor(8, 1)
        P.conv(tin, a0, W, b, stride=2, act=ACT_RELU)
        t = a0
        for i, ((dk, dbn, stride), (pk, pbn, cout, both)) in enumerate(zip(dw_keys, pw_keys)):
            W, b = cbr(dk, dbn)
            d = P.tensor(P.tensors[t][0], 0, name='stem' if i == 0 else None)
            P.dwconv(t, d, W, b, stride=stride)
            W, b = cbr(pk, pbn)
            c = P.tensor(cout, 1 if i < 12 else 0)
            P.conv(d, c, W, b, act=ACT_RELU)
            if both:
                feats.append(c)
            t = c
    f8, f16, f32 = feats
    P.tap('feat8', f8, 0, 64)
    P.tap('feat16', f16, 0, 128)
    P.tap('feat32', f32, 0, 256)

    e2 = arch.RETINA_REFINER_BN_EPS
    rp = refiner_prec

    def rcbr(p):
        return cbr(p + '.0', p + '.1', e2, bias=True)

    A = arch.RETINA_NUM_ANCHORS
    heads = {}
    use_lanes = not os.environ.get('TERRAN_AMD_NO_DETECTOR_LANES')

    def context_and_heads(s, x, lane):
        P.lane = lane if use_lanes else 0
        p = 'refiner.context_stride%d' % s
        ctx = P.tensor(96, 1)
        W3, b3 = rcbr(p + '.context_3x3')
        Wr, br_ = rcbr(p + '.dimension_reducer')
        P.conv(x, ctx, np.concatenate([W3, Wr]), np.concatenate([b3, br_]), act=ACT_RELU, out_ch_off=0, precision=rp)
        W5, b5 = rcbr(p + '.context_5x5')
        W7, b7 = cbr(p + '.context_7x7.0', p + '.context_7x7.1', e2, bias=True)
        P.conv(ctx, ctx, np.concatenate([W5, W7]), np.concatenate([b5, b7]), act=ACT_RELU, in_ch_off=32,
               out_ch_off=48, precision=rp)
        W7b, b7b = cbr(p + '.context_7x7.3', p + '.context_7x7.4', e2, bias=True)
        P.conv(ctx, ctx, W7b, b7b, act=ACT_RELU, in_ch_off=64, out_ch_off=80, precision=rp)
        P.tap('ctx%d_3x3' % s, ctx, 0, 32)
        P.tap('ctx%d_5x5' % s, ctx, 48, 16)
        P.tap('ctx%d_7x7' % s, ctx, 80, 16)
        Wh = np.concatenate([sd['outputs.%s_stride%d.weight' % (h, s)] for h in ('cls', 'bbox', 'landmark')])
        bh = np.concatenate([sd['outputs.%s_stride%d.bias' % (h, s)] for h in ('cls', 'bbox', 'landmark')])
        pos = np.concatenate([np.arange(32), 48 + np.arange(16), 80 + np.arange(16)])
        hd = P.tensor(16 * A, 0, name='head%d' % s, f32=True)
        P.conv(ctx, hd, Wh, bh, ch_pos=pos, cin_p=96, precision=rp)
        heads[s] = hd
        P.lane = 0

    W, b = rcbr('refiner.conv_stride32')
    p32 = P.tensor(64, 1, name='p32')
    P.conv(f32, p32, W, b, act=ACT_RELU, precision=rp)
    context_and_heads(32, p32, 1)
    W, b = rcbr('refiner.conv_stride16')
    s16 = P.tensor(64, 1)
    P.conv(f16, s16, W, b, act=ACT_RELU, res=p32, res_up2=1, precision=rp)
    W, b = rcbr('refiner.aggr_stride16')
    p16 = P.tensor(64, 1, name='p16')
    P.conv(s16, p16, W, b, act=ACT_RELU, precision=rp)
    context_and_heads(16, p16, 2)
    W, b = rcbr('refiner.conv_stride8')
    s8 = P.tensor(64, 1)
    P.conv(f8, s8, W, b, act=ACT_RELU, res=p16, res_up2=1, precision=rp)
    W, b = rcbr('refiner.aggr_stride8')
    p8 = P.tensor(64, 1, name='p8')
    P.conv(s8, p8, W, b, act=ACT_RELU, precision=rp)
    context_and_heads(8, p8, 0)
    P.outputs = [heads[32], heads[16], heads[8]]
    return P


PACKERS = {MODEL_RETINAFACE: pack_retinaface, MODEL_ARCFACE: pack_arcface, MODEL_OPENPOSE: pack_openpose}
```

Baseline: 2190 frames/s.

## Fuse OpenPose stage tail 1x1 convs into a chained kernel through LDS

Adds a conv_tail_chain kernel that computes a 1x1 head conv, keeps its output tile in LDS in split hi/lo form, and immediately runs up to two following 1x1 output convs on it. The planner marks eligible OpenPose stage tails in the packer, skips the follower ops, and no longer allocates the intermediate tensor. The aim is to drop the intermediate tensor's HBM write and read-back and the extra kernel launches. In exchange the fused kernel uses 128KB of LDS per block, which limits occupancy, and the blob version is bumped.

Measured after the change: 2174 frames/s. No clear change (-0.7%).

```diff
diff --git a/include/terran_amd.h b/include/terran_amd.h
--- a/include/terran_amd.h
+++ b/include/terran_amd.h
@@ -104,6 +104,7 @@
 
 int ta_model_tensor_unscale(const ta_model* m, int tensor, float* out, int capacity);
 int ta_model_debug_amax(ta_model* m, int enable, float* out, int capacity);
+int ta_model_plan_bytes(const ta_model* m, int64_t* bytes);
 int ta_model_graph_probe(ta_model* m, int reps, double* out_ms);
 
 int ta_retinaface_run(ta_model* m, const ta_frames* frames, float score_thr, float nms_thr,
diff --git a/terran_amd/csrc/conv_split.hip b/terran_amd/csrc/conv_split.hip
--- a/terran_amd/csrc/conv_split.hip
+++ b/terran_amd/csrc/conv_split.hip
@@ -74,3 +74,32 @@
   TA_HIP(ctx, hipGetLastError());
   return TA_OK;
 }
+
+int ta_launch_conv_chain(ta_ctx* ctx, const ta_chain_launch& c_in, double flops) {
+  if (c_in.head.M <= 0) return TA_OK;
+  ta_chain_launch c = c_in;
+  if (c.n_fin < 1 || c.n_fin > TA_CHAIN_MAX_FIN || c.head.coutp % 256 || c.head.n_slabs < 1)
+    return ta_fail(ctx, TA_E_INVALID, "conv chain: bad shape");
+  ta_conv_launch* all[1 + TA_CHAIN_MAX_FIN] = {&c.head, &c.fin[0], &c.fin[1]};
+  for (int i = 0; i <= c.n_fin; ++i) {
+    ta_conv_launch& q = *all[i];
+    q.range_flag = ctx->range_flag;
+    q.k_split = 1;
+    q.r_Wo = 1.0f / (float)q.Wo;
+    q.r_Ho = 1.0f / (float)q.Ho;
+    q.r_HoWo = 1.0f / (float)(q.Ho * q.Wo);
+    q.fast_div = (long long)q.M + 128 < (1 << 24) ? 1 : 0;
+#ifdef TA_CONV_TRACE
+    q.trace_block = ctx->conv_trace_block;
+#endif
+  }
+  if (!c.head.group_cout) {
+    c.head.group_cout = c.head.coutp;
+    c.head.group_cin = c.head.n_slabs * 32;
+  }
+  ctx->conv_counts[TA_CV_TAIL_CHAIN] += 1;
+  ctx->cur_flops = flops;
+  ta_prof_scope scope(ctx, 0, flops);
+  if (c.head.prec == PREC_F16X3) return launch_chain<PREC_F16X3>(ctx, c);
+  return ta_launch_conv_chain_modes(ctx, c);
+}
diff --git a/terran_amd/csrc/conv_split_kernels.h b/terran_amd/csrc/conv_split_kernels.h
--- a/terran_amd/csrc/conv_split_kernels.h
+++ b/terran_amd/csrc/conv_split_kernels.h
@@ -543,6 +543,178 @@
 }
 
 template <int PREC>
+__global__ __launch_bounds__(512) void conv_tail_chain(const ta_chain_launch c) {
+  static_assert(prec_x3(PREC), "three-product modes on pre-split tensors");
+  constexpr bool HALF = prec_half(PREC);
+  extern __shared__ __attribute__((aligned(16))) float lds[];
+  const ta_conv_launch& p = c.head;
+  const int tid = threadIdx.x;
+  const int lane = tid & 63;
+  const int wave = __builtin_amdgcn_readfirstlane(tid >> 6);
+  const int pt0 = blockIdx.x * 128;
+  const int HoWo = p.Ho * p.Wo;
+  const int frow = lane & 31, kg = lane >> 5;
+  const int cm = wave >> 1, cn = wave & 1;
+  const ta_pixel_walk walk(p, pt0, HoWo);
+  const char* bptr[2];
+#pragma unroll
+  for (int b = 0; b < 2; ++b) {
+    const int d = cn * 64 + b * 32 + frow;
+    int img, y, x;
+    walk.at(pt0 + d < p.M ? d : 0, img, y, x);
+    bptr[b] = (const char*)(p.in + ((size_t)img * p.in_img + (size_t)y * p.in_row + (size_t)x * p.in_pix + p.in_off0 + p.in_ch_off));
+  }
+  const int KS = p.n_slabs;
+  int uf[2], uct[2], upt[2];
+#pragma unroll
+  for (int i = 0; i < 2; ++i) {
+    int u = wave + 8 * i, f = 0;
+    while (f < c.n_fin && u >= (c.fin[f].coutp >> 5) * 4) u -= (c.fin[f++].coutp >> 5) * 4;
+    uf[i] = f < c.n_fin ? f : -1;
+    uct[i] = u >> 2;
+    upt[i] = u & 3;
+  }
+  f32x16 acc2[2];
+#pragma unroll
+  for (int i = 0; i < 2; ++i)
+#pragma unroll
+    for (int r = 0; r < 16; ++r) acc2[i][r] = 0.f;
+  unsigned amax = 0;
+  const float* hus = p.bias + p.coutp;
+  const int rounds = p.coutp >> 8;
+  for (int rd = 0; rd < rounds; ++rd) {
+    const int c0 = rd * 256 + cm * 64;
+    const int grp = p.group_cout ? c0 / p.group_cout : 0;
+    const char* arow = (const char*)p.w + ((size_t)(c0 + frow)) * 128 + kg * 32;
+    const size_t a_slab = (size_t)p.coutp * 128;
+    const int boff = grp * p.group_cin * 4 + kg * 32;
+    f32x16 acc[2][2];
+    split_acc_clear(acc);
+    struct Frag {
+      bf16x8 ah[2], al[2], bh[2], bl[2];
+    };
+    auto load = [&](Frag& f, int q) {
+      const int s = q >> 1, t = q & 1;
+#pragma unroll
+      for (int a = 0; a < 2; ++a) {
+        const char* w = arow + s * a_slab + a * 32 * 128 + t * 16;
+        f.ah[a] = *(const bf16x8*)w;
+        f.al[a] = *(const bf16x8*)(w + 64);
+      }
+#pragma unroll
+      for (int b = 0; b < 2; ++b) {
+        const char* x = bptr[b] + boff + s * 128 + t * 16;
+        f.bh[b] = *(const bf16x8*)x;
+        f.bl[b] = *(const bf16x8*)(x + 64);
+      }
+    };
+    Frag F0, F1;
+    load(F0, 0);
+    for (int q = 0; q < 2 * KS; q += 2) {
+      load(F1, q + 1);
+      split_mma16<PREC>(acc, F0.ah, F0.al, F0.bh, F0.bl);
+      if (q + 2 < 2 * KS) load(F0, q + 2);
+      split_mma16<PREC>(acc, F1.ah, F1.al, F1.bh, F1.bl);
+    }
+    if (rd) __syncthreads();
+#pragma unroll
+    for (int b = 0; b < 2; ++b) {
+      const int row = cn * 64 + b * 32 + frow;
+      const bool real = pt0 + row < p.M;
+      const unsigned sw = (unsigned)(row >> 1) & 7u;
+#pragma unroll
+      for (int a = 0; a < 2; ++a)
+#pragma unroll
+        for (int j = 0; j < 4; ++j) {
+          const int lc = cm * 64 + a * 32 + 8 * j + 4 * kg;
+          const int co = rd * 256 + lc;
+          const f32x4 bi = *(const f32x4*)(p.bias + co), us = *(const f32x4*)(hus + co);
+          f32x4 v;
+#pragma unroll
+          for (int e = 0; e < 4; ++e) {
+            v[e] = __builtin_fmaf(acc[a][b][4 * j + e], us[e], bi[e]);
+            if (p.act == TA_ACT_RELU) v[e] = ta_relu(v[e]);
+          }
+          if (real && (HALF || p.range_check)) amax = ta_amax4(amax, v);
+          unsigned h0, h1, l0, l1;
+          ta_pack2<HALF>(v[0], v[1], h0, l0);
+          ta_pack2<HALF>(v[2], v[3], h1, l1);
+          const unsigned chunk = (unsigned)(lc & 31) >> 3;
+          char* base = (char*)lds + (lc >> 5) * 16384 + row * 128 + ((lc >> 2) & 1) * 8;
+          *(uint2*)(base + ((chunk ^ sw) << 4)) = make_uint2(h0, h1);
+          *(uint2*)(base + (((chunk + 4) ^ sw) << 4)) = make_uint2(l0, l1);
+        }
+    }
+    __syncthreads();
+#pragma unroll
+    for (int i = 0; i < 2; ++i) {
+      if (uf[i] < 0) continue;
+      const ta_conv_launch& q = c.fin[uf[i]];
+      const int row = upt[i] * 32 + frow;
+      const unsigned sw = (unsigned)(row >> 1) & 7u;
+      const char* brow = (const char*)lds + row * 128;
+      const char* wrow = (const char*)q.w + ((size_t)(uct[i] * 32 + frow)) * 128 + kg * 32;
+      const size_t w_slab = (size_t)q.coutp * 128;
+      const int ws0 = (rd * 256 - q.in_ch_off) >> 5;
+      for (int sl = 0; sl < 8; ++sl) {
+        const int ws = ws0 + sl;
+        if (ws < 0 || ws >= q.n_slabs) continue;
+#pragma unroll
+        for (int t = 0; t < 2; ++t) {
+          const char* w = wrow + ws * w_slab + t * 16;
+          const bf16x8 ah = *(const bf16x8*)w, al = *(const bf16x8*)(w + 64);
+          const unsigned ch = (unsigned)(2 * kg + t);
+          const bf16x8 bh = *(const bf16x8*)(brow + sl * 16384 + ((ch ^ sw) << 4));
+          const bf16x8 bl = *(const bf16x8*)(brow + sl * 16384 + (((ch + 4) ^ sw) << 4));
+          acc2[i] = ta_mfma16<PREC>(al, bh, acc2[i]);
+          acc2[i] = ta_mfma16<PREC>(ah, bl, acc2[i]);
+          acc2[i] = ta_mfma16<PREC>(ah, bh, acc2[i]);
+        }
+      }
+    }
+  }
+  ta_range_report(p, amax);
+#pragma unroll
+  for (int i = 0; i < 2; ++i) {
+    if (uf[i] < 0) continue;
+    const ta_conv_launch& q = c.fin[uf[i]];
+    const int row = upt[i] * 32 + frow;
+    unsigned am = 0;
+    if (pt0 + row < q.M) {
+      int img, y, x;
+      walk.at(row, img, y, x);
+      float* o = q.out + (size_t)img * q.out_img + (size_t)y * q.out_row + (size_t)x * q.out_pix + q.out_off0;
+#pragma unroll
+      for (int j = 0; j < 4; ++j) {
+        const int co = uct[i] * 32 + 8 * j + 4 * kg;
+        if (co >= q.cout) continue;
+        const f32x4 bi = *(const f32x4*)(q.bias + co), us = *(const f32x4*)(q.bias + q.coutp + co);
+        f32x4 v;
+#pragma unroll
+        for (int e = 0; e < 4; ++e) {
+          v[e] = __builtin_fmaf(acc2[i][4 * j + e], us[e], bi[e]);
+          if (q.act == TA_ACT_RELU) v[e] = ta_relu(v[e]);
+        }
+        ta_st4(o, q.out_ch + co, q.out_fmt, v);
+        if (q.range_check) am = ta_amax4(am, v);
+      }
+    }
+    ta_range_report(q, am);
+  }
+}
+
+template <int PREC>
+static int launch_chain(ta_ctx* ctx, const ta_chain_launch& c) {
+  constexpr size_t lds_bytes = 8 * 128 * 128;
+  auto kern = conv_tail_chain<PREC>;
+  TA_SET_LDS_ATTR(ctx, kern, lds_bytes);
+  TA_NOTE_KERNEL(ctx, "conv_tail_chain<%d>", PREC);
+  hipLaunchKernelGGL(kern, dim3((c.head.M + 127) / 128), dim3(512), lds_bytes, ctx->stream, c);
+  TA_HIP(ctx, hipGetLastError());
+  return TA_OK;
+}
+
+template <int PREC>
 static int launch_split_variant(ta_ctx* ctx, int v, const ta_conv_launch& p) {
   switch (v) {
     case TA_CV_SPLIT_2x2: return launch_split<2, 2, 4, PREC, 3>(ctx, p);
diff --git a/terran_amd/csrc/conv_split_modes.hip b/terran_amd/csrc/conv_split_modes.hip
--- a/terran_amd/csrc/conv_split_modes.hip
+++ b/terran_amd/csrc/conv_split_modes.hip
@@ -10,3 +10,8 @@
     default: return launch_split_variant<PREC_BF16>(ctx, v, p);
   }
 }
+
+int ta_launch_conv_chain_modes(ta_ctx* ctx, const ta_chain_launch& c) {
+  if (c.head.prec != PREC_BF16X3) return ta_fail(ctx, TA_E_INVALID, "conv chain: arithmetic mode %d has no chained kernel", c.head.prec);
+  return launch_chain<PREC_BF16X3>(ctx, c);
+}
diff --git a/terran_amd/csrc/net.hip b/terran_amd/csrc/net.hip
--- a/terran_amd/csrc/net.hip
+++ b/terran_amd/csrc/net.hip
@@ -14,6 +14,43 @@
   const bool uniform = (op.cin % kblk == 0) && (op.n_slabs == op.kh * op.kw * (op.cin / kblk));
   const bool kernel_ok = in_fmt == ta_split_fmt_of(op.prec);
   return uniform && kernel_ok && op.groups <= 1 && !op.pool;
+}
+
+template <class F>
+static int chain_followers(const ta_model* m, size_t oi, F fmt) {
+  const std::vector<ta_op_desc>& ops = m->ops;
+  const ta_op_desc& h = ops[oi];
+  if ((h.variant >> 19) & 1) return 0;
+  size_t n = 0;
+  while (oi + 1 + n < ops.size() && ((ops[oi + 1 + n].variant >> 19) & 1)) ++n;
+  if (n < 1 || n > TA_CHAIN_MAX_FIN) return 0;
+  auto plain_1x1 = [&](const ta_op_desc& op) {
+    return op.type == TA_OP_CONV && (op.prec == 1 || op.prec == 3) && op.prec == h.prec && op.kh == 1 && op.kw == 1 && op.stride == 1 &&
+           op.pad == 0 && op.res < 0 && op.out2 < 0 && !op.pool && (op.variant & 0x7FFFF) == 0 && op.cin % 32 == 0 &&
+           op.n_slabs == op.cin / 32 && op.in_ch_off % 32 == 0 && (op.act == TA_ACT_NONE || op.act == TA_ACT_RELU) &&
+           fmt(op.in) == ta_split_fmt_of(op.prec) && fmt(op.out) == ta_split_fmt_of(op.prec);
+  };
+  const int groups = h.groups > 1 ? h.groups : 1;
+  if (!plain_1x1(h) || h.cout != h.coutp || h.coutp % 256 || (h.coutp / groups) % 64) return 0;
+  const ta_tensor_desc& mid = m->tdesc[h.out];
+  if (mid.alias_of != -1 || mid.channels != h.coutp || h.out_ch_off != 0 || h.out == h.in) return 0;
+  for (int i = 0; i < m->hdr.n_outputs; ++i)
+    if (m->hdr.outputs[i] == h.out) return 0;
+  for (const ta_tensor_desc& t : m->tdesc)
+    if (t.alias_of == h.out) return 0;
+  int tiles = 0;
+  for (size_t k = 0; k < ops.size(); ++k) {
+    const ta_op_desc& op = ops[k];
+    const bool member = k > oi && k <= oi + n;
+    if (member) {
+      if (!plain_1x1(op) || op.groups > 1 || op.in != h.out || op.in_ch_off + op.cin > h.coutp || op.out == h.out || op.cout % 4) return 0;
+      tiles += op.coutp / 32;
+    } else if (k != oi && (op.in == h.out || op.out == h.out || op.res == h.out || op.out2 == h.out)) {
+      return 0;
+    }
+  }
+  if (tiles > 4) return 0;
+  return (int)n;
 }
 
 #define TA_MAX_PLANS 4
@@ -192,6 +229,16 @@
     if ((ts[i].fmt != TA_FMT_F32 && ts[i].c % 32) || (ts[i].fmt == TA_FMT_F16 && ts[i].c % 64) || ts[i].fmt < 0 || ts[i].fmt > TA_FMT_F16)
       return ta_fail(ctx, TA_E_INVALID, "plan: tensor %d: format %d with %d channels", i, ts[i].fmt, ts[i].c);
 
+  np->chain.assign(m->ops.size(), 0);
+  if (!ctx->conv_force)
+    for (size_t oi = 0; oi < m->ops.size(); ++oi) {
+      const int nf = chain_followers(m, oi, [&](int t) { return ts[t].fmt; });
+      if (!nf) continue;
+      np->chain[oi] = nf;
+      for (int k = 1; k <= nf; ++k) np->chain[oi + k] = -1;
+      ts[m->ops[oi].out].owns = false;
+    }
+
   size_t total = 0;
   std::vector<size_t> offs(T, 0);
   for (int i = 0; i < T; ++i) {
@@ -269,7 +316,10 @@
     const double M = op.type == TA_OP_CONV && op.pool
                          ? (double)m->run_n * conv_out(ti.h, op.kh, op.stride, op.pad) * conv_out(ti.w, op.kw, op.stride, op.pad)
                          : (double)m->run_n * to.h * to.w;
-    const double fl = (op.type == TA_OP_CONV || op.type == TA_OP_DWPW) ? 2.0 * op.macs_per_pixel * M : 0.0;
+    double fl = (op.type == TA_OP_CONV || op.type == TA_OP_DWPW) ? 2.0 * op.macs_per_pixel * M : 0.0;
+    const int chained = m->active ? m->active->chain[oi] : 0;
+    if (chained < 0) fl = 0.0;
+    for (int k = 1; k <= chained; ++k) fl += 2.0 * m->ops[oi + k].macs_per_pixel * M;
     tot_ms += ms;
     tot_fl += fl;
     fprintf(stderr, "op %3zu type %d k%dx%d s%d g%d cin %4d cout %4d  %3dx%-3d M %8.0f slabs %4d  %8.1f us %7.1f TF\n", oi, op.type, op.kh,
@@ -308,6 +358,90 @@
         }
     }
   } lanes{ctx, ctx->stream};
+  auto conv_launch_of = [&](size_t oi, int lane, ta_conv_launch& p, double& flops) -> int {
+    const ta_op_desc& op = m->ops[oi];
+    const ta_tensor& ti = m->tensors[op.in];
+    const ta_tensor& to = m->tensors[op.out];
+    memset(&p, 0, sizeof(p));
+    p.in = ti.dev;
+    p.w = wptr(m, op.w_off);
+    p.ktab = m->ktab_dev + m->ktab_off[oi];
+    p.bias = wptr(m, op.bias_off);
+    p.prelu = wptr(m, op.prelu_off);
+    p.out = to.dev;
+    p.M = m->run_n * to.h * to.w;
+    p.Ho = to.h;
+    p.Wo = to.w;
+    p.n_slabs = op.n_slabs;
+    p.coutp = op.coutp;
+    p.cout = op.cout;
+    p.act = op.act;
+    p.stride = op.stride;
+    p.prec = op.prec;
+    const int kblk = ti.fmt == TA_FMT_F16 ? 64 : 32;
+    p.uniform_k = (op.cin % kblk == 0) && (op.n_slabs == op.kh * op.kw * (op.cin / kblk));
+    p.k_cblocks = op.cin / kblk;
+    if (ti.fmt == TA_FMT_F16 && (!p.uniform_k || op.in_ch_off || op.groups > 1 || op.prec != 4))
+      return ta_fail(ctx, TA_E_INVALID, "op %zu: a half-float tensor feeds whole-tensor convs of the f16 mode only", oi);
+    p.k_w = op.kw;
+    p.k_h = op.kh;
+    p.in_ch_off = op.in_ch_off;
+    p.in_img = (int)((size_t)ti.hp() * ti.wp() * ti.cf());
+    p.in_row = ti.wp() * ti.cf();
+    p.in_pix = ti.cf();
+    p.win_wp = ti.wp();
+    p.win_img = ti.hp() * ti.wp();
+    p.in_off0 = (int)(((size_t)(ti.halo - op.pad) * ti.wp() + (ti.halo - op.pad)) * ti.cf());
+    p.out_img = (int)((size_t)to.hp() * to.wp() * to.cf());
+    p.out_row = to.wp() * to.cf();
+    p.out_pix = to.cf();
+    p.out_off0 = (int)to.off(0, 0, 0);
+    p.out_ch = op.out_ch_off;
+    p.out_fmt = to.fmt;
+    p.in_fmt = ti.fmt;
+    if (op.res >= 0) {
+      const ta_tensor& tr = m->tensors[op.res];
+      p.res = tr.dev;
+      p.res_img = (int)((size_t)tr.hp() * tr.wp() * tr.cf());
+      p.res_row = tr.wp() * tr.cf();
+      p.res_pix = tr.cf();
+      p.res_off0 = (int)tr.off(0, 0, 0);
+      p.res_ch = op.res_ch_off;
+      p.res_fmt = tr.fmt;
+      p.res_up2 = op.res_up2;
+    }
+    if (op.out2 >= 0) {
+      const ta_tensor& t2 = m->tensors[op.out2];
+      p.out2 = t2.dev;
+      p.scale2 = wptr(m, op.scale2_off);
+      p.shift2 = wptr(m, op.shift2_off);
+      p.o2_img = (int)((size_t)t2.hp() * t2.wp() * t2.cf());
+      p.o2_row = t2.wp() * t2.cf();
+      p.o2_pix = t2.cf();
+      p.o2_off0 = (int)t2.off(0, 0, 0);
+      p.o2_ch = op.out2_ch_off;
+      p.o2_fmt = t2.fmt;
+    }
+    if (op.groups > 1) {
+      p.group_cout = op.cout / op.groups;
+      p.group_cin = op.cin;
+    }
+    p.variant = op.variant & 255;
+    if ((op.variant >> 16) & 1) p.bias9 = wptr(m, op.scale2_off);
+    p.range_check = (m->has_half_ops && (m->tensor_read[op.out] || (op.out2 >= 0 && m->tensor_read[op.out2]))) ? 1 : 0;
+    p.amax_index = (m->amax_on && oi < TA_AMAX_OPS) ? (int)oi : -1;
+    flops = 2.0 * op.macs_per_pixel * (double)p.M;
+    if (op.pool) {
+      p.pool = 1;
+      p.M = m->run_n * to.h * to.w * 4;
+      flops = 2.0 * op.macs_per_pixel * (double)m->run_n * conv_out(ti.h, op.kh, op.stride, op.pad) *
+              conv_out(ti.w, op.kw, op.stride, op.pad);
+    }
+    p.k_split = m->splitk_ws ? ta_conv_ksplit(p.coutp, p.n_slabs, conv_ksplit_eligible(op, ti.fmt), (op.variant >> 8) & 255) : 1;
+    p.partial = m->splitk_ws;
+    if (lane) p.k_split = 1;
+    return TA_OK;
+  };
   for (size_t oi = 0; oi < m->ops.size(); ++oi) {
     const ta_op_desc& op = m->ops[oi];
     const ta_tensor& ti = m->tensors[op.in];
@@ -337,85 +471,24 @@
     if (prof_ops) (void)hipEventRecord(ev[2 * oi], ctx->stream);
     switch (op.type) {
       case TA_OP_CONV: {
+        const int chained = m->active ? m->active->chain[oi] : 0;
+        if (chained < 0) break;
         ta_conv_launch p;
-        memset(&p, 0, sizeof(p));
-        p.in = ti.dev;
-        p.w = wptr(m, op.w_off);
-        p.ktab = m->ktab_dev + m->ktab_off[oi];
-        p.bias = wptr(m, op.bias_off);
-        p.prelu = wptr(m, op.prelu_off);
-        p.out = to.dev;
-        p.M = m->run_n * to.h * to.w;
-        p.Ho = to.h;
-        p.Wo = to.w;
-        p.n_slabs = op.n_slabs;
-        p.coutp = op.coutp;
-        p.cout = op.cout;
-        p.act = op.act;
-        p.stride = op.stride;
-        p.prec = op.prec;
-        const int kblk = ti.fmt == TA_FMT_F16 ? 64 : 32;
-        p.uniform_k = (op.cin % kblk == 0) && (op.n_slabs == op.kh * op.kw * (op.cin / kblk));
-        p.k_cblocks = op.cin / kblk;
-        if (ti.fmt == TA_FMT_F16 && (!p.uniform_k || op.in_ch_off || op.groups > 1 || op.prec != 4))
-          return ta_fail(ctx, TA_E_INVALID, "op %zu: a half-float tensor feeds whole-tensor convs of the f16 mode only", oi);
-        p.k_w = op.kw;
-        p.k_h = op.kh;
-        p.in_ch_off = op.in_ch_off;
-        p.in_img = (int)((size_t)ti.hp() * ti.wp() * ti.cf());
-        p.in_row = ti.wp() * ti.cf();
-        p.in_pix = ti.cf();
-        p.win_wp = ti.wp();
-        p.win_img = ti.hp() * ti.wp();
-        p.in_off0 = (int)(((size_t)(ti.halo - op.pad) * ti.wp() + (ti.halo - op.pad)) * ti.cf());
-        p.out_img = (int)((size_t)to.hp() * to.wp() * to.cf());
-        p.out_row = to.wp() * to.cf();
-        p.out_pix = to.cf();
-        p.out_off0 = (int)to.off(0, 0, 0);
-        p.out_ch = op.out_ch_off;
-        p.out_fmt = to.fmt;
-        p.in_fmt = ti.fmt;
-        if (op.res >= 0) {
-          const ta_tensor& tr = m->tensors[op.res];
-          p.res = tr.dev;
-          p.res_img = (int)((size_t)tr.hp() * tr.wp() * tr.cf());
-          p.res_row = tr.wp() * tr.cf();
-          p.res_pix = tr.cf();
-          p.res_off0 = (int)tr.off(0, 0, 0);
-          p.res_ch = op.res_ch_off;
-          p.res_fmt = tr.fmt;
-          p.res_up2 = op.res_up2;
+        double flops = 0;
+        TA_TRY(conv_launch_of(oi, lane, p, flops));
+        if (chained > 0) {
+          ta_chain_launch c;
+          memset(&c, 0, sizeof(c));
+          c.head = p;
+          c.n_fin = chained;
+          for (int k = 0; k < chained; ++k) {
+            double fl = 0;
+            TA_TRY(conv_launch_of(oi + 1 + k, lane, c.fin[k], fl));
+            flops += fl;
+          }
+          TA_TRY(ta_launch_conv_chain(ctx, c, flops));
+          break;
         }
-        if (op.out2 >= 0) {
-          const ta_tensor& t2 = m->tensors[op.out2];
-          p.out2 = t2.dev;
-          p.scale2 = wptr(m, op.scale2_off);
-          p.shift2 = wptr(m, op.shift2_off);
-          p.o2_img = (int)((size_t)t2.hp() * t2.wp() * t2.cf());
-          p.o2_row = t2.wp() * t2.cf();
-          p.o2_pix = t2.cf();
-          p.o2_off0 = (int)t2.off(0, 0, 0);
-          p.o2_ch = op.out2_ch_off;
-          p.o2_fmt = t2.fmt;
-        }
-        if (op.groups > 1) {
-          p.group_cout = op.cout / op.groups;
-          p.group_cin = op.cin;
-        }
-        p.variant = op.variant & 255;
-        if ((op.variant >> 16) & 1) p.bias9 = wptr(m, op.scale2_off);
-        p.range_check = (m->has_half_ops && (m->tensor_read[op.out] || (op.out2 >= 0 && m->tensor_read[op.out2]))) ? 1 : 0;
-        p.amax_index = (m->amax_on && oi < TA_AMAX_OPS) ? (int)oi : -1;
-        double flops = 2.0 * op.macs_per_pixel * (double)p.M;
-        if (op.pool) {
-          p.pool = 1;
-          p.M = m->run_n * to.h * to.w * 4;
-          flops = 2.0 * op.macs_per_pixel * (double)m->run_n * conv_out(ti.h, op.kh, op.stride, op.pad) *
-                  conv_out(ti.w, op.kw, op.stride, op.pad);
-        }
-        p.k_split = m->splitk_ws ? ta_conv_ksplit(p.coutp, p.n_slabs, conv_ksplit_eligible(op, ti.fmt), (op.variant >> 8) & 255) : 1;
-        p.partial = m->splitk_ws;
-        if (lane) p.k_split = 1;
         TA_TRY(ta_launch_conv(ctx, p, flops));
         break;
       }
@@ -506,7 +579,7 @@
   if (bytes < sizeof(ta_blob_header)) return ta_fail(ctx, TA_E_INVALID, "model blob too small");
   ta_blob_header h;
   memcpy(&h, blob, sizeof(h));
-  if (h.magic != TA_BLOB_MAGIC || h.version != 9) return ta_fail(ctx, TA_E_INVALID, "model blob: bad magic/version (this library reads version 9)");
+  if (h.magic != TA_BLOB_MAGIC || h.version != 10) return ta_fail(ctx, TA_E_INVALID, "model blob: bad magic/version (this library reads version 10)");
   if (h.kind != kind) return ta_fail(ctx, TA_E_INVALID, "model blob is kind %d, expected %d", h.kind, kind);
   if (h.n_tensors <= 0 || h.n_ops <= 0 || h.n_outputs < 0 || h.n_outputs > 16 || h.input_tensor < 0 ||
       h.input_tensor >= h.n_tensors)
@@ -680,6 +753,12 @@
   TA_HIP(ctx, hipStreamSynchronize(ctx->stream));
   TA_HIP(ctx, hipEventElapsedTime(&ms, e0, e1));
   out_ms[1] = ms / reps;
+  return TA_OK;
+}
+
+int ta_model_plan_bytes(const ta_model* m, int64_t* bytes) {
+  if (!m || !bytes) return TA_E_INVALID;
+  *bytes = m->active ? (int64_t)m->active->arena_bytes : 0;
   return TA_OK;
 }
 
diff --git a/terran_amd/csrc/ta_internal.h b/terran_amd/csrc/ta_internal.h
--- a/terran_amd/csrc/ta_internal.h
+++ b/terran_amd/csrc/ta_internal.h
@@ -158,6 +158,7 @@
   TA_CV_WIN_1x4 = 10,
   TA_CV_SPLIT_1x4_W2 = 11,
   TA_CV_SPLIT_2x2_W2 = 12,
+  TA_CV_TAIL_CHAIN = 13,
   TA_CV_COUNT = 16
 };
 
@@ -281,6 +282,14 @@
 #define TA_WIN_PR_2x2 384
 #define TA_WIN_PR_2x4 448
 #define TA_WIN_PR_1x4 512
+#define TA_CHAIN_MAX_FIN 2
+struct ta_chain_launch {
+  ta_conv_launch head;
+  ta_conv_launch fin[TA_CHAIN_MAX_FIN];
+  int n_fin;
+};
+int ta_launch_conv_chain(ta_ctx* ctx, const ta_chain_launch& c, double flops);
+int ta_launch_conv_chain_modes(ta_ctx* ctx, const ta_chain_launch& c);
 struct ta_frames;
 int ta_launch_rfstem(ta_ctx* ctx, const uint8_t* frames_dev, int n, int h, int w, const float* weights_host, const float* w2_dev, const struct ta_tensor& out);
 
@@ -308,6 +317,7 @@
   int32_t* ktab_dev = nullptr;
   std::vector<size_t> ktab_off;
   float* splitk_ws = nullptr;
+  std::vector<int> chain;
   uint64_t last_use = 0;
 };
 
diff --git a/terran_amd/lib.py b/terran_amd/lib.py
--- a/terran_amd/lib.py
+++ b/terran_amd/lib.py
@@ -60,6 +60,7 @@
     'ta_model_tensor_shape': (c_int, [c_void_p, c_int, P(c_int), P(c_int), P(c_int), P(c_int)]),
     'ta_model_tensor_unscale': (c_int, [c_void_p, c_int, c_void_p, c_int]),
     'ta_model_debug_amax': (c_int, [c_void_p, c_int, c_void_p, c_int]),
+    'ta_model_plan_bytes': (c_int, [c_void_p, c_void_p]),
     'ta_model_graph_probe': (c_int, [c_void_p, c_int, c_void_p]),
     'ta_model_read_tensor': (c_int, [c_void_p, c_int, c_int, c_int, c_void_p]),
     'ta_retinaface_run': (c_int, [c_void_p, c_void_p, c_float, c_float, c_int, c_void_p, c_void_p, c_void_p,
@@ -309,6 +310,8 @@
         out = {k: int(c[v]) for k, v in CONV_VARIANTS.items() if v and c[v]}
         if c[15]:
             out['lean_epilogue'] = int(c[15])
+        if c[13]:
+            out['tail_chain'] = int(c[13])
         return out
 
     def kernel_work(self, reset=False):
@@ -455,6 +458,11 @@
     def amax_collect(self, on=True):
         self.ctx.check(self.ctx.lib.ta_model_debug_amax(self.h, int(bool(on)), None, 0))
 
+    def plan_bytes(self):
+        out = np.zeros(1, np.int64)
+        self.ctx.check(self.ctx.lib.ta_model_plan_bytes(self.h, ptr(out)))
+        return int(out[0])
+
     def graph_probe(self, reps=20):
         out = np.zeros(5, np.float64)
         self.ctx.check(self.ctx.lib.ta_model_graph_probe(self.h, int(reps), ptr(out)))
diff --git a/terran_amd/pack.py b/terran_amd/pack.py
--- a/terran_amd/pack.py
+++ b/terran_amd/pack.py
@@ -23,11 +23,11 @@
 _OP_I64 = ['w_off', 'bias_off', 'prelu_off', 'scale2_off', 'shift2_off', 'wus_off']
 OP_DT = np.dtype([(n, '<i4') for n in _OP_I32] + [(n, '<i8') for n in _OP_I64] + [('macs_per_pixel', '<f8')])
 assert OP_DT.itemsize == 152 and TENSOR_DT.itemsize == 20
-BLOB_VERSION = 9
+BLOB_VERSION = 10
 
 
 PACK_SWITCHES = ('TERRAN_AMD_NO_FUSED_POOL', 'TERRAN_AMD_NO_GROUPED', 'TERRAN_AMD_NO_MERGED_OUTPUTS', 'TERRAN_AMD_ARCFACE_SECOND_OUTPUT',
-                 'TERRAN_AMD_NO_STAGE4_KSPLIT', 'TERRAN_AMD_DETECTOR_F32', 'TERRAN_AMD_DETECTOR_BASE_F32', 'TERRAN_AMD_NO_FUSED_DETECTOR', 'TERRAN_AMD_NO_FUSED_FRONT',
+                 'TERRAN_AMD_NO_STAGE4_KSPLIT', 'TERRAN_AMD_DETECTOR_F32', 'TERRAN_AMD_DETECTOR_BASE_F32', 'TERRAN_AMD_NO_FUSED_DETECTOR', 'TERRAN_AMD_NO_FUSED_FRONT', 'TERRAN_AMD_NO_FUSED_TAILS',
                  'TERRAN_AMD_NO_DETECTOR_LANES', 'TERRAN_AMD_NO_ACT_SCALES')
 
 
@@ -801,6 +801,7 @@
             P.conv(cur, o, W, b, act=ACT_RELU if relu else ACT_NONE, groups=2)
             cur = o
         (np_, cin, co1, k, r1), (nh, cin2, co2, k2, r2) = l1[-1], l2[-1]
+        n_before = len(P.ops)
         if r1 == r2 and cin == cin2 <= 128 and not os.environ.get('TERRAN_AMD_NO_MERGED_OUTPUTS'):
             Wp, bp = np.asarray(sd['model%d_1.%s.weight' % (st, np_)]), np.asarray(sd['model%d_1.%s.bias' % (st, np_)])
             Wh, bh = np.asarray(sd['model%d_2.%s.weight' % (st, nh)]), np.asarray(sd['model%d_2.%s.bias' % (st, nh)])
@@ -817,6 +818,9 @@
                 off, cp = (OP_PAF, 40) if br == 1 else (OP_HM, 20)
                 P.conv(cur, xout, sd[key + '.weight'], sd[key + '.bias'], act=ACT_RELU if relu else ACT_NONE,
                        in_ch_off=(br - 1) * cin, out_ch_off=off, cout_p=cp)
+        if grouped and l1[-2][3] == 1 and not os.environ.get('TERRAN_AMD_NO_FUSED_TAILS'):
+            for op in P.ops[n_before:]:
+                op['variant'] |= 1 << 19
         P.tap('stage%d_paf' % st, xout, OP_PAF, 38)
         P.tap('stage%d_hm' % st, xout, OP_HM, 19)
     P.outputs = [X0]
```
